# OpenStitching/stitching

Hardware: AMD Instinct MI355X
Metric: warped+blended Mpix/s (higher is better)
Workload: dtype u8/int16 (fixed-point remap, int32 pyramid sums, fp32 weights); 1 GPU; BASELINE config 2: 8 synthetic 4000x3000 frames, one ring; yaw step 38.9 deg = 0.58 hfov (42 % overlap; SURVEY 8(d) names 0.70 hfov); spherical warp + 5-band multiband blend, inputs resident in HBM; frames_per_gpu=8, panoramas_in_flight=2

## Files before the change

include/stitching_amd.h:

```cpp
#ifndef STITCHING_AMD_H
#define STITCHING_AMD_H

#include <stddef.h>
#include <stdint.h>

#ifdef __cplusplus
extern "C" {
#endif

#define STX_VERSION 100

#define STX_OK 0
#define STX_ERR_INVALID (-1)
#define STX_ERR_HIP (-2)
#define STX_ERR_OOM (-3)
#define STX_ERR_STATE (-4)
#define STX_ERR_UNSUPPORTED (-5)

#define STX_TRIG_EXACT 0
#define STX_TRIG_GLIBC 1
#define STX_TRIG_GLIBC_NOFMA 2
int stx_set_trig_mode(int mode);
int stx_get_trig_mode(void);

// ... 15 lines not shown
#define STX_WARP_CYLINDRICAL 2
#define STX_WARP_SPHERICAL 3
#define STX_WARP_FISHEYE 4
#define STX_WARP_STEREOGRAPHIC 5
#define STX_WARP_COMPRESSED_PLANE_A2B1 6
#define STX_WARP_COMPRESSED_PLANE_A15B1 7
#define STX_WARP_COMPRESSED_PLANE_PORTRAIT_A2B1 8
#define STX_WARP_COMPRESSED_PLANE_PORTRAIT_A15B1 9
#define STX_WARP_PANINI_A2B1 10
#define STX_WARP_PANINI_A15B1 11
#define STX_WARP_PANINI_PORTRAIT_A2B1 12
#define STX_WARP_PANINI_PORTRAIT_A15B1 13
#define STX_WARP_MERCATOR 14
#define STX_WARP_TRANSVERSE_MERCATOR 15
#define STX_WARP_TYPE_COUNT 16

#define STX_INTER_NEAREST 0
#define STX_INTER_LINEAR 1
#define STX_BORDER_CONSTANT 0
#define STX_BORDER_REFLECT 2

#define STX_BLEND_NO 0
#define STX_BLEND_FEATHER 1
#define STX_BLEND_MULTIBAND 2

#define STX_U8 0
#define STX_S16 1
#define STX_F32 2

typedef struct stx_ctx stx_ctx;
typedef struct stx_buf stx_buf;
typedef struct stx_blender stx_blender;
typedef struct stx_mb_weights stx_mb_weights;

int stx_version(void);
const char* stx_last_error(void);
int stx_device_count(int* out_n);
int stx_ctx_create(int device, stx_ctx** out);
int stx_ctx_destroy(stx_ctx* ctx);
int stx_ctx_sync(stx_ctx* ctx);

int stx_buf_from_host(stx_ctx* ctx, const void* host, size_t host_stride_bytes, int w, int h, int channels, int elem,
                      stx_buf** out);
int stx_buf_alloc(stx_ctx* ctx, int w, int h, int channels, int elem, stx_buf** out);
int stx_host_alloc(size_t bytes, void** out);
int stx_host_free(void* p);
int stx_buf_to_host(const stx_buf* buf, void* host, size_t host_stride_bytes);
int stx_buf_from_host_async(stx_ctx* ctx, const void* host, size_t host_stride_bytes, int w, int h, int channels, int elem,
                            stx_buf** out);
int stx_buf_to_host_async(const stx_buf* buf, void* host, size_t host_stride_bytes);
int stx_buf_view(const stx_buf* buf, int x, int y, int w, int h, stx_buf** out);
int stx_buf_info(const stx_buf* buf, int64_t info[6]);
int stx_buf_device_ptr(const stx_buf* buf, void** out);
int stx_buf_free(stx_buf* buf);

int stx_warp_roi(stx_ctx* ctx, int type, float scale, const float K[9], const float R[9], int w, int h,
                 int out_xywh[4]);
int stx_warp_rois(stx_ctx* ctx, int type, float scale, int n, const float* K9s, const float* R9s, const int* sizes_wh,
                  int* out_xywh);
int stx_warp(stx_ctx* ctx, int type, float scale, const float K[9], const float R[9], const stx_buf* src, int interp,
             int border, stx_buf** out, int out_tl[2]);
int stx_warp_image_and_mask(stx_ctx* ctx, int type, float scale, const float K[9], const float R[9],
                            const stx_buf* src, stx_buf** out_img, stx_buf** out_mask, int out_xywh[4]);
int stx_warp_batch(stx_ctx* ctx, int type, float scale, int n, const float* K9s, const float* R9s,
                   const stx_buf* const* srcs, stx_buf** out_imgs, stx_buf** out_masks, int* out_xywh);
int stx_warp_batch_rects(stx_ctx* ctx, int type, float scale, int n, const float* K9s, const float* R9s,
                         const stx_buf* const* srcs, const int* rects_xywh, stx_buf** out_imgs, stx_buf** out_masks);
int stx_warp_batch_gain(stx_ctx* ctx, int type, float scale, int n, const float* K9s, const float* R9s, const stx_buf* const* srcs,
                        const int* rects_xywh, const stx_buf* const* gain_maps_f32, const int* gain_flags, stx_buf** out_imgs,
                        stx_buf** out_masks, int* out_xywh);
int stx_warp_batch_with_rois(stx_ctx* ctx, int type, float scale, int n, const float* K9s, const float* R9s, const stx_buf* const* srcs,
                             const stx_buf* const* gain_maps_f32_or_null, const int* gain_flags_or_null, stx_buf** out_imgs,
                             stx_buf** out_masks, int* out_xywh);
int stx_warp_mask(stx_ctx* ctx, int type, float scale, const float K[9], const float R[9], int w, int h,
                  stx_buf** out_mask, int out_xywh[4]);

int stx_result_roi(int n, const int* corners_xy, const int* sizes_wh, int out_xywh[4]);
int stx_blend_create(stx_ctx* ctx, int kind, int num_bands, float sharpness, const int roi_xywh[4],
                     stx_blender** out);
int stx_blend_num_bands(const stx_blender* b, int* out_num_bands);
int stx_blend_feed(stx_blender* b, const stx_buf* img, const stx_buf* mask, int tlx, int tly);
int stx_blend_finish(stx_blender* b, stx_buf** out_pano_u8, stx_buf** out_mask_u8);
int stx_blend_finish_ex(stx_blender* b, stx_buf** out_pano_u8, stx_buf** out_mask_u8, stx_buf** out_pano_s16);
int stx_blend_destroy(stx_blender* b);
int stx_blend_keep_weights(stx_blender* b, stx_mb_weights** out);
int stx_blend_use_weights(stx_blender* b, stx_mb_weights* w, int* out_adopted);
int stx_mb_weights_free(stx_mb_weights* w);

int stx_gain_apply(stx_ctx* ctx, stx_buf* img_u8x3, const float gains_bgr[3]);
int stx_block_gain_apply(stx_ctx* ctx, stx_buf* img_u8x3, const stx_buf* gain_map_f32);
#define STX_GAIN_MAP_BOUNDED 1
int stx_block_gain_apply_batch(stx_ctx* ctx, int n, stx_buf* const* imgs_u8x3, const stx_buf* const* gain_maps_f32,
                               const int* full_wh_xy0, const int* flags);
#define STX_EXPOSURE_GAIN 1
#define STX_EXPOSURE_GAIN_BLOCKS 2
#define STX_EXPOSURE_CHANNELS 3
#define STX_EXPOSURE_CHANNELS_BLOCKS 4
int stx_exposure_feed(stx_ctx* ctx, int kind, int n, const stx_buf* const* imgs_u8x3, const stx_buf* const* masks_u8,
                      const int* corners_xy, int block_size, int nr_feeds, double* out_gains, long long* inout_count,
                      double out_info[4]);
int stx_exposure_stats(stx_ctx* ctx, int kind, int n, const stx_buf* const* imgs_u8x3, const stx_buf* const* masks_u8,
                       const int* corners_xy, int block_size, long long* inout_jobs, int* out_ab, long long* out_c,
                       double* out_sums);
// ... 108 lines not shown
```

include/stitching_amd_debug.h:

```cpp
#ifndef STITCHING_AMD_DEBUG_H
#define STITCHING_AMD_DEBUG_H

#include "stitching_amd.h"

#ifdef __cplusplus
extern "C" {
#endif

int stx_debug_warp_maps(stx_ctx* ctx, int type, float scale, const float K[9], const float R[9], int w, int h, int which,
                        const int rect_xywh[4], stx_buf** out_xmap_f32, stx_buf** out_ymap_f32, int out_xywh[4]);

int stx_debug_feather_dist_cap(void);

int stx_debug_blend_replayed(stx_ctx* ctx, int* out_launches);

#ifdef __cplusplus
}
#endif
#endif
```

stitching_amd/_lib.py:

```python
import ctypes as C
import os

from .stitching_error import StitchingError

_HERE = os.path.dirname(os.path.abspath(__file__))
LIB_PATH = os.environ.get("STITCHING_AMD_LIB") or os.path.join(_HERE, "libstitching_amd.so")

STX_OK = 0
WARP_PLANE, WARP_AFFINE, WARP_CYLINDRICAL, WARP_SPHERICAL = 0, 1, 2, 3
WARP_TYPE_IDS = {"plane": 0, "affine": 1, "cylindrical": 2, "spherical": 3, "fisheye": 4, "stereographic": 5,
                 "compressedPlaneA2B1": 6, "compressedPlaneA1.5B1": 7, "compressedPlanePortraitA2B1": 8,
                 "compressedPlanePortraitA1.5B1": 9, "paniniA2B1": 10, "paniniA1.5B1": 11, "paniniPortraitA2B1": 12,
                 "paniniPortraitA1.5B1": 13, "mercator": 14, "transverseMercator": 15}
INTER_NEAREST, INTER_LINEAR = 0, 1
BORDER_CONSTANT, BORDER_REFLECT = 0, 2
BLEND_NO, BLEND_FEATHER, BLEND_MULTIBAND = 0, 1, 2
U8, S16, F32 = 0, 1, 2
TRIG_MODES = {"exact": 0, "glibc": 1, "glibc-nofma": 2}
REMAP_MODES = {"q15": 0, "float": 1, "float-fma": 2}
PYRDOWN_MODES = {"scalar": 0, "simd-v": 1, "simd-hv": 3, "simd-v-fma": 5, "simd-hv-fma": 7}
GAIN_MAP_BOUNDED = 1
EXPOSURE_KINDS = {"gain": 1, "gain_blocks": 2, "channel": 3, "channel_blocks": 4}
EXPOSURE_SOLVERS = {"host": 0, "device": 1}
LU_NB, LU_MAX_N = 32, 16384
SEAM_KINDS = {"no": 0, "voronoi": 1}
COLOR_SEAM_MAX_LENGTH, COLOR_SEAM_MAX_CROSS = 16384, 4096
FEATURES_MAX_SIDE, FEATURES_MAX_LEVELS, FEATURES_MAX_FEATURES = 32767, 16, 65536
MATCH_MAX_FEATURES, MATCH_MAX_ITERS = 65536, 4096
RAY_MAX_CAMERAS, RAY_MAX_MATCHES = 1024, 131072
CONTRIB_U8_BINARY = 1
STRIP_MASK_BITS = 2

EXPORTS = (
    "stx_version stx_last_error stx_set_trig_mode stx_get_trig_mode stx_set_remap_mode stx_get_remap_mode stx_set_pyrdown_mode stx_get_pyrdown_mode stx_device_count stx_ctx_create stx_ctx_destroy stx_ctx_sync "
    "stx_host_alloc stx_host_free stx_buf_from_host stx_buf_from_host_async stx_buf_alloc stx_buf_to_host stx_buf_to_host_async stx_buf_view stx_buf_info stx_buf_device_ptr stx_buf_free "
    "stx_warp_roi stx_warp_rois stx_warp stx_warp_image_and_mask stx_warp_batch stx_warp_batch_rects stx_warp_batch_gain stx_warp_batch_with_rois stx_warp_mask "
    "stx_gain_apply stx_block_gain_apply stx_block_gain_apply_batch stx_resize_linear_exact stx_resize_linear_exact_batch stx_seam_mask_resize stx_seam_mask_resize_batch stx_seam_mask_resize_batch_sub stx_timelapse_frame stx_result_roi stx_blend_create stx_blend_num_bands stx_blend_feed stx_blend_finish stx_blend_finish_ex "
    "stx_blend_destroy stx_blend_keep_weights stx_blend_use_weights stx_mb_weights_free stx_blend_set_band stx_blend_feed_ex stx_blend_contrib_rect stx_blend_export_contrib stx_blend_export_contribs "
    "stx_blend_build stx_blend_feed_contrib stx_blend_feed_contrib_ex stx_buf_flags stx_strip_rect stx_view_rect stx_strip_pack stx_strip_pack_batch stx_strip_pack_batch_ex stx_strip_bytes stx_strip_unpack stx_blend_feed_strips stx_comm_unique_id stx_comm_create stx_comm_exchange stx_comm_exchange_begin stx_comm_exchange_end stx_comm_exchange_begin_on stx_comm_exchange_end_on stx_comm_info stx_comm_destroy stx_prof_enable stx_prof_reset stx_prof_count stx_prof_get stx_mark stx_mark_elapsed_ms "
    "stx_exposure_feed stx_exposure_stats stx_exposure_solve stx_set_exposure_solver stx_get_exposure_solver stx_exposure_feed_ex stx_exposure_solve_device stx_lu_solve_device stx_seam_find stx_seam_schedule stx_color_seam_find stx_crop_lir stx_features_detect stx_match_features stx_ray_problem_create stx_ray_problem_eval stx_ray_problem_free "
    "stx_debug_warp_maps stx_debug_feather_dist_cap stx_debug_blend_replayed"
).split()

_lib = None


def build_hint():
    return "build it with `make -C stitching_amd/csrc` or `python -c 'import __graft_entry__ as g; g.build()'`"


def lib():
    global _lib
    if _lib is not None:
        return _lib
    if not os.path.exists(LIB_PATH):
        raise ImportError(f"{LIB_PATH} is missing: the HIP back end is not built ({build_hint()}). "
                          "stitching_amd has no CPU fallback.")
    L = C.CDLL(LIB_PATH)
    vp, vpp = C.c_void_p, C.POINTER(C.c_void_p)
    fp, ip = C.POINTER(C.c_float), C.POINTER(C.c_int)
    L.stx_version.restype = C.c_int
    L.stx_last_error.restype = C.c_char_p
    L.stx_set_trig_mode.argtypes = [C.c_int]
    L.stx_get_trig_mode.restype = C.c_int
    L.stx_set_remap_mode.argtypes = [C.c_int]
    L.stx_get_remap_mode.restype = C.c_int
    L.stx_set_pyrdown_mode.argtypes = [C.c_int, C.c_int]
    L.stx_get_pyrdown_mode.argtypes = [C.POINTER(C.c_int)]
    L.stx_get_pyrdown_mode.restype = C.c_int
    L.stx_device_count.argtypes = [ip]
    L.stx_ctx_create.argtypes = [C.c_int, vpp]
    L.stx_ctx_destroy.argtypes = [vp]
    L.stx_ctx_sync.argtypes = [vp]
    L.stx_buf_from_host.argtypes = [vp, vp, C.c_size_t, C.c_int, C.c_int, C.c_int, C.c_int, vpp]
    L.stx_buf_from_host_async.argtypes = L.stx_buf_from_host.argtypes
    L.stx_buf_alloc.argtypes = [vp, C.c_int, C.c_int, C.c_int, C.c_int, vpp]
    L.stx_host_alloc.argtypes = [C.c_size_t, vpp]
    L.stx_host_free.argtypes = [vp]
    L.stx_buf_to_host.argtypes = [vp, vp, C.c_size_t]
    L.stx_buf_to_host_async.argtypes = [vp, vp, C.c_size_t]
    L.stx_buf_view.argtypes = [vp, C.c_int, C.c_int, C.c_int, C.c_int, vpp]
    L.stx_buf_info.argtypes = [vp, C.POINTER(C.c_int64)]
    L.stx_buf_device_ptr.argtypes = [vp, vpp]
    L.stx_buf_free.argtypes = [vp]
    L.stx_warp_roi.argtypes = [vp, C.c_int, C.c_float, fp, fp, C.c_int, C.c_int, ip]
    L.stx_warp_rois.argtypes = [vp, C.c_int, C.c_float, C.c_int, fp, fp, ip, ip]
    L.stx_warp.argtypes = [vp, C.c_int, C.c_float, fp, fp, vp, C.c_int, C.c_int, vpp, ip]
    L.stx_warp_image_and_mask.argtypes = [vp, C.c_int, C.c_float, fp, fp, vp, vpp, vpp, ip]
    L.stx_warp_batch.argtypes = [vp, C.c_int, C.c_float, C.c_int, fp, fp, vpp, vpp, vpp, ip]
    L.stx_warp_batch_rects.argtypes = [vp, C.c_int, C.c_float, C.c_int, fp, fp, vpp, ip, vpp, vpp]
    L.stx_warp_batch_gain.argtypes = [vp, C.c_int, C.c_float, C.c_int, fp, fp, vpp, ip, vpp, ip, vpp, vpp, ip]
    L.stx_warp_batch_with_rois.argtypes = [vp, C.c_int, C.c_float, C.c_int, fp, fp, vpp, vpp, ip, vpp, vpp, ip]
    L.stx_warp_mask.argtypes = [vp, C.c_int, C.c_float, fp, fp, C.c_int, C.c_int, vpp, ip]
    L.stx_gain_apply.argtypes = [vp, vp, fp]
    L.stx_block_gain_apply.argtypes = [vp, vp, vp]
    L.stx_block_gain_apply_batch.argtypes = [vp, C.c_int, vpp, vpp, ip, ip]
    L.stx_resize_linear_exact.argtypes = [vp, vp, C.c_int, C.c_int, vpp]
    L.stx_resize_linear_exact_batch.argtypes = [vp, C.c_int, vpp, ip, vpp]
    L.stx_seam_mask_resize.argtypes = [vp, vp, vp, vpp]
    L.stx_seam_mask_resize_batch.argtypes = [vp, C.c_int, vpp, vpp, vpp]
    L.stx_seam_mask_resize_batch_sub.argtypes = [vp, C.c_int, vpp, vpp, ip, vpp]
    L.stx_timelapse_frame.argtypes = [vp, vp, C.c_int, C.c_int, ip, vpp]
    L.stx_result_roi.argtypes = [C.c_int, ip, ip, ip]
    L.stx_blend_create.argtypes = [vp, C.c_int, C.c_int, C.c_float, ip, vpp]
    L.stx_blend_num_bands.argtypes = [vp, ip]
    L.stx_blend_feed.argtypes = [vp, vp, vp, C.c_int, C.c_int]
    L.stx_blend_finish.argtypes = [vp, vpp, vpp]
    L.stx_blend_finish_ex.argtypes = [vp, vpp, vpp, vpp]
    L.stx_blend_destroy.argtypes = [vp]
    L.stx_blend_keep_weights.argtypes = [vp, vpp]
    L.stx_blend_use_weights.argtypes = [vp, vp, ip]
    L.stx_mb_weights_free.argtypes = [vp]
    L.stx_blend_set_band.argtypes = [vp, C.c_int, C.c_int]
    L.stx_blend_feed_ex.argtypes = [vp, vp, vp, C.c_int, C.c_int, C.c_int]
    L.stx_blend_contrib_rect.argtypes = [vp, C.c_int, C.c_int, C.c_int, C.c_int, C.c_int, C.c_int, ip,
                                         C.POINTER(C.c_size_t)]
    L.stx_blend_export_contrib.argtypes = [vp, C.c_int, C.c_int, C.c_int, vpp, ip]
    L.stx_blend_export_contribs.argtypes = [vp, C.c_int, ip, ip, ip, vpp, ip]
    L.stx_blend_build.argtypes = [vp]
    L.stx_blend_feed_contrib.argtypes = [vp, C.c_int, ip, vp]
    L.stx_blend_feed_contrib_ex.argtypes = [vp, C.c_int, ip, vp, C.c_int]
    L.stx_buf_flags.argtypes = [vp, ip]
    L.stx_strip_rect.argtypes = [vp, C.c_int, C.c_int, C.c_int, C.c_int, C.c_int, C.c_int, ip, C.POINTER(C.c_size_t)]
    L.stx_view_rect.argtypes = [vp, C.c_int, C.c_int, C.c_int, C.c_int, C.c_int, C.c_int, C.c_int, C.c_int, ip]
    L.stx_strip_pack.argtypes = [vp, vp, vp, C.c_int, C.c_int, vpp]
    L.stx_strip_unpack.argtypes = [vp, C.c_int, C.c_int, C.c_int, vpp, vpp]
    L.stx_strip_pack_batch.argtypes = [vp, C.c_int, vpp, vpp, ip, ip, vpp]
    L.stx_strip_pack_batch_ex.argtypes = [vp, C.c_int, vpp, vpp, ip, ip, C.c_int, vpp]
    L.stx_strip_bytes.argtypes = [C.c_int, C.c_int, C.c_int, C.POINTER(C.c_size_t)]
    L.stx_blend_feed_strips.argtypes = [vp, C.c_int, vpp, ip, ip, ip, ip, ip, C.c_int]
    L.stx_comm_unique_id.argtypes = [C.POINTER(C.c_ubyte)]
    L.stx_comm_create.argtypes = [vp, C.c_int, C.c_int, C.POINTER(C.c_ubyte), vpp]
    L.stx_comm_exchange.argtypes = [vp, C.c_int, ip, ip, C.POINTER(C.c_void_p), C.POINTER(C.c_size_t)]
    L.stx_comm_exchange_begin.argtypes = [vp, C.c_int, ip, ip, C.POINTER(C.c_void_p), C.POINTER(C.c_size_t)]
    L.stx_comm_exchange_end.argtypes = [vp]
    L.stx_comm_exchange_begin_on.argtypes = [vp, vp, C.c_int, ip, ip, C.POINTER(C.c_void_p), C.POINTER(C.c_size_t)]
    L.stx_comm_exchange_end_on.argtypes = [vp, vp]
    L.stx_comm_info.argtypes = [vp, ip]
    L.stx_comm_destroy.argtypes = [vp]
    L.stx_prof_enable.argtypes = [vp, C.c_int]
    L.stx_prof_reset.argtypes = [vp]
    L.stx_prof_count.argtypes = [vp, ip]
    L.stx_prof_get.argtypes = [vp, C.c_int, C.c_char_p, C.c_int, C.POINTER(C.c_int64), C.POINTER(C.c_double),
                               C.POINTER(C.c_double)]
    L.stx_debug_blend_replayed.argtypes = [vp, ip]
    L.stx_debug_warp_maps.argtypes = [vp, C.c_int, C.c_float, fp, fp, C.c_int, C.c_int, C.c_int, ip, vpp, vpp, ip]
    llp, dp = C.POINTER(C.c_longlong), C.POINTER(C.c_double)
    L.stx_exposure_feed.argtypes = [vp, C.c_int, C.c_int, vpp, vpp, ip, C.c_int, C.c_int, dp, llp, dp]
    L.stx_exposure_stats.argtypes = [vp, C.c_int, C.c_int, vpp, vpp, ip, C.c_int, llp, ip, llp, dp]
    L.stx_exposure_solve.argtypes = [C.c_int, C.c_int, ip, dp, C.POINTER(C.c_ubyte), dp]
    L.stx_set_exposure_solver.argtypes = [C.c_int]
    L.stx_exposure_feed_ex.argtypes = [vp, C.c_int, C.c_int, vpp, vpp, ip, C.c_int, C.c_int, C.c_int, dp, llp, dp]
    L.stx_exposure_solve_device.argtypes = [vp, C.c_int, C.c_int, ip, dp, C.POINTER(C.c_ubyte), dp, dp]
    L.stx_lu_solve_device.argtypes = [vp, C.c_int, dp, dp, dp, dp]
    L.stx_seam_find.argtypes = [vp, C.c_int, C.c_int, ip, ip, vpp, vpp, dp]
    L.stx_seam_schedule.argtypes = [C.c_int, ip, ip, ip, ip, ip]
    L.stx_color_seam_find.argtypes = [vp, C.c_int, ip, ip, vpp, vpp, vpp, dp]
    L.stx_crop_lir.argtypes = [vp, vp, ip, ip, dp]
    L.stx_features_detect.argtypes = [vp, C.c_int, vpp, vpp, C.c_int, C.c_int, C.c_int, ip, ip, ip, ip, C.POINTER(C.c_byte), ip, ip, llp,
                                      C.POINTER(C.c_ubyte), dp]
    L.stx_match_features.argtypes = [vp, C.c_int, vpp, ip, vpp, ip, C.c_int, C.c_int, C.c_int, C.c_double, C.c_uint, ip, ip,
                                     C.POINTER(C.c_ubyte), ip, dp, dp]
    L.stx_ray_problem_create.argtypes = [vp, C.c_int, ip, llp, dp, vpp]
    L.stx_ray_problem_eval.argtypes = [vp, C.c_int, dp, dp, dp]
    L.stx_ray_problem_free.argtypes = [vp]
    L.stx_mark.argtypes = [vp, C.c_int]
    L.stx_mark_elapsed_ms.argtypes = [vp, C.c_int, C.c_int, C.POINTER(C.c_double)]
    for name in EXPORTS:
        if name not in ("stx_version", "stx_last_error"):
            getattr(L, name).restype = C.c_int
    _lib = L
    return L


def check(rc):
    if rc != STX_OK:
        msg = lib().stx_last_error()
        raise StitchingError(f"stitching_amd [{rc}]: {msg.decode(errors='replace') if msg else 'unknown error'}")
# ... 1 lines not shown
```

stitching_amd/csrc/stx_blend.hip:

```cpp
#include <cstring>

#include "stx_blend_kernels.h"
#include "stx_device_math.h"
#include "stx_internal.h"

using namespace stxd;

namespace {

constexpr float WEIGHT_EPS = 1e-5f;
constexpr float INV255 = 0.0039215688593685627f;
constexpr float INV256 = 0.00390625f;

template <bool S16>
STX_DEV void load_px0(const StxMbImage& im, int sx, int sy, int& b, int& g, int& r)
{
    if (S16) {
        const short* p = reinterpret_cast<const short*>(im.img0 + (long long)sy * im.img0_stride) + sx * 3;
        b = p[0]; g = p[1]; r = p[2];
    } else {
        const uint8_t* p = im.img0 + (long long)sy * im.img0_stride + sx * 3;
        b = p[0]; g = p[1]; r = p[2];
    }
}
// ... 661 lines not shown
            if (lv == 0) {
                if (im.img0_is_s16) hipLaunchKernelGGL(mb_down0_kernel<true>, grid64x4(ow, oh), dim3(256), 0, ctx->stream, im, pyr_mode, pyr_lanes);
                else hipLaunchKernelGGL(mb_down0_kernel<false>, grid64x4(ow, oh), dim3(256), 0, ctx->stream, im, pyr_mode, pyr_lanes);
            } else {
                hipLaunchKernelGGL(mb_down_kernel, grid64x4(ow, oh), dim3(256), 0, ctx->stream, im, lv, pyr_mode, pyr_lanes);
            }
        }
        STX_TRY(check_launch("mb_down"));
    }
    return STX_OK;
}

int stx_launch_mb_coarse(stx_ctx* ctx, const MbLevelK& K, double algo_bytes)
{
    if (K.x1 <= K.x0 || K.y1 <= K.y0) return STX_OK;
    if (K.level != K.num_bands - 2 || K.level < 1 || K.y0 != 0 || K.out_y0 != 0 || K.emit)
        return stx_fail(STX_ERR_INVALID, "mb_coarse: not the argument block of level B-2");
    StxProfScope prof(ctx, "mb_coarse", algo_bytes);
    MbCoarseK C;
    C.images = K.images; C.n_images = K.n_images; C.num_bands = K.num_bands;
    C.x0 = K.x0; C.x1 = K.x1; C.y1 = K.y1;
    C.out = K.out; C.out_stride = K.out_stride; C.out_plane = K.out_plane; C.out_x0 = K.out_x0;
    C.pw = K.pw; C.ph = K.ph;
    const dim3 grid((K.x1 - K.x0 + CO_TW - 1) / CO_TW, (K.y1 + CO_TH - 1) / CO_TH);
    hipLaunchKernelGGL(mb_coarse_kernel, grid, dim3(256), 0, ctx->stream, C);
    return check_launch("mb_coarse");
}

int stx_launch_mb_level(stx_ctx* ctx, const MbLevelK& K, double algo_bytes)
{
    if (K.x1 <= K.x0 || K.y1 <= K.y0) return STX_OK;
    StxProfScope prof(ctx, K.emit ? "mb_contrib" : (K.level == 0 ? "mb_level0" : "mb_level"), algo_bytes);
    if ((K.level > 0 || K.all_u8) && stx_fast_mb_level(ctx, K)) return STX_OK;
    const dim3 grid = grid64x4(K.x1 - K.x0, K.y1 - K.y0);
    if (K.level == 0) hipLaunchKernelGGL(mb_level_kernel<true>, grid, dim3(256), 0, ctx->stream, K);
    else hipLaunchKernelGGL(mb_level_kernel<false>, grid, dim3(256), 0, ctx->stream, K);
    return check_launch("mb_level");
}

int stx_launch_mb_emit_batch(stx_ctx* ctx, const MbLevelK* d_Ks, const MbLevelK* h_Ks, const int* classes, int n, double bytes)
{
    if (n <= 0) return STX_OK;
    StxProfScope prof(ctx, "mb_contrib", bytes);
    for (int start = 0; start < n;) {
        int end = start;
        while (end < n && classes[end] == classes[start]) end++;
        const int cls = classes[start], count = end - start;
        if (cls >= 0) {
            if (!stx_fast_mb_emit_launch(ctx, cls, d_Ks + start, h_Ks + start, count)) return check_launch("mb_contrib");
        } else {
            int gx = 1, gy = 1;
            for (int i = start; i < end; i++) {
                gx = std::max(gx, (h_Ks[i].x1 - h_Ks[i].x0 + 63) / 64);
                gy = std::max(gy, (h_Ks[i].y1 - h_Ks[i].y0 + 3) / 4);
            }
            const dim3 grid(gx, gy, count);
            if (cls == -1) hipLaunchKernelGGL(mb_level_multi_kernel<true>, grid, dim3(256), 0, ctx->stream, d_Ks + start);
            else hipLaunchKernelGGL(mb_level_multi_kernel<false>, grid, dim3(256), 0, ctx->stream, d_Ks + start);
        }
        start = end;
    }
    return check_launch("mb_contrib");
}

namespace {
STX_DEV uint32_t ld_u32_unaligned(const uint8_t* p)
// ... 1158 lines not shown
```

stitching_amd/csrc/stx_blend_fast.hip:

```cpp
#include <algorithm>
#include <cstdlib>

#include "stx_blend_kernels.h"
#include "stx_device_math.h"

using namespace stxd;

namespace {

constexpr int L0_WAVES = 5;
constexpr float WEIGHT_EPS = 1e-5f;
constexpr float INV255 = 0.0039215688593685627f;
constexpr float INV256 = 0.00390625f;

#define STX_GAS __attribute__((address_space(1)))
template <class T> STX_DEV const STX_GAS T* gp(const T* p) { return (const STX_GAS T*)p; }
template <class T> STX_DEV STX_GAS T* gp(T* p) { return (STX_GAS T*)p; }

STX_DEV bool xcd_tile(const StxTileMap& M, uint32_t b, int& tx, int& ty)
{
    if (M.plain) {
        const uint32_t wy = M.tiles_x == 1 ? b : __umulhi(b, M.magic_tx);
        tx = (int)(b - wy * (uint32_t)M.tiles_x);
        ty = (int)wy;
// ... 798 lines not shown
    int he[3][4], ho[3][4];
#pragma unroll
    for (int r = 0; r < 3; r++) {
        const T* p = plane + (long long)rr[r] * stride;
        int c[6];
        if (sizeof(T) == 2) {
            const v4u w = *reinterpret_cast<const v4u_a4*>(p + cx - 2);
            c[1] = s16lo(w.y); c[2] = s16hi(w.y); c[3] = s16lo(w.z); c[4] = s16hi(w.z);
            c[0] = s16hi(w.x);
            c[5] = s16lo(w.w);
        } else {
            const v3u w = *reinterpret_cast<const v3u_a4*>(p + cx - 4);
            c[0] = (int)(w.x >> 24);
            c[1] = (int)(w.y & 255u); c[2] = (int)((w.y >> 8) & 255u); c[3] = (int)((w.y >> 16) & 255u); c[4] = (int)(w.y >> 24);
            c[5] = (int)(w.z & 255u);
        }
        if (le) c[0] = c[2];
        if (re) c[5] = c[4];
#pragma unroll
        for (int j = 0; j < 4; j++) {
            he[r][j] = c[j] + 6 * c[j + 1] + c[j + 2];
            ho[r][j] = 4 * (c[j + 1] + c[j + 2]);
        }
    }
#pragma unroll
    for (int j = 0; j < 4; j++) {
        up[0][2 * j] = s6(he[0][j] + 6 * he[1][j] + he[2][j]);
        up[0][2 * j + 1] = s6(ho[0][j] + 6 * ho[1][j] + ho[2][j]);
        up[1][2 * j] = s6(4 * (he[1][j] + he[2][j]));
        up[1][2 * j + 1] = s6(4 * (ho[1][j] + ho[2][j]));
    }
}

template <bool L0>
STX_DEV void level_epilogue(const MbLevelK& P, int X0, int Y0, int (&acc)[2][8][3], float (&ws)[2][8])
{
    int v[2][8][3];
#pragma unroll
    for (int r = 0; r < 2; r++)
#pragma unroll
        for (int j = 0; j < 8; j++) {
            const float den = fadd(ws[r][j], WEIGHT_EPS);
            float q0, q1, q2;
            div3_shared(den, (float)(short)acc[r][j][0], (float)(short)acc[r][j][1], (float)(short)acc[r][j][2], q0, q1, q2);
            v[r][j][0] = trunc_small(q0);
            v[r][j][1] = trunc_small(q1);
            v[r][j][2] = trunc_small(q2);
        }
    if (P.up) {
#pragma unroll
        for (int c = 0; c < 3; c++) {
            int up[2][8];
            up_patch(P.up + c * P.up_plane - ((long long)P.up_y0 * P.up_stride + P.up_x0), P.up_stride, P.pw >> 1, P.ph >> 1,
                     X0 >> 1, Y0 >> 1, up);
#pragma unroll
            for (int r = 0; r < 2; r++)
#pragma unroll
                for (int j = 0; j < 8; j++) v[r][j][c] = sat_s16(up[r][j] + v[r][j][c]);
        }
    }
    if (!L0) {
#pragma unroll
        for (int r = 0; r < 2; r++)
#pragma unroll
            for (int c = 0; c < 3; c++) {
                uint4 o;
                o.x = pack16(v[r][0][c], v[r][1][c]);
                o.y = pack16(v[r][2][c], v[r][3][c]);
                o.z = pack16(v[r][4][c], v[r][5][c]);
                o.w = pack16(v[r][6][c], v[r][7][c]);
                if (Y0 + r < P.y1)
                    *reinterpret_cast<uint4*>(P.out + c * P.out_plane + (long long)(Y0 + r - P.out_y0) * P.out_stride + (X0 - P.out_x0)) = o;
            }
    } else {
#pragma unroll
        for (int r = 0; r < 2; r++) {
            const int y = Y0 + r;
            if (y >= P.y1) break;
            const int oy = y - P.pano_y0, ox = X0 - P.pano_x0;
            uint32_t ob[6] = {0, 0, 0, 0, 0, 0}, om[2] = {0, 0};
#pragma unroll
            for (int j = 0; j < 8; j++) {
                const bool keep = ws[r][j] > WEIGHT_EPS;
#pragma unroll
                for (int c = 0; c < 3; c++) {
                    if (!keep) v[r][j][c] = 0;
                    const uint32_t u = (uint32_t)min(abs(v[r][j][c]), 255);
                    const int bo = 3 * j + c;
                    ob[bo >> 2] |= u << (8 * (bo & 3));
                }
                om[j >> 2] |= (keep ? 255u : 0u) << (8 * (j & 3));
            }
            uint32_t* po = reinterpret_cast<uint32_t*>(P.pano + (long long)oy * P.pano_stride + (long long)ox * 3);
            *reinterpret_cast<uint2*>(po) = make_uint2(ob[0], ob[1]);
            *reinterpret_cast<uint2*>(po + 2) = make_uint2(ob[2], ob[3]);
            *reinterpret_cast<uint2*>(po + 4) = make_uint2(ob[4], ob[5]);
            *reinterpret_cast<uint2*>(P.pmask + (long long)oy * P.pmask_stride + ox) = make_uint2(om[0], om[1]);
            if (P.pano16) {
                uint32_t* p16 = reinterpret_cast<uint32_t*>(reinterpret_cast<uint8_t*>(P.pano16) + (long long)oy * P.pano16_stride +
                                                            (long long)ox * 6);
                uint32_t s[12];
#pragma unroll
                for (int j = 0; j < 8; j += 2) {
                    s[(j >> 1) * 3 + 0] = pack16(v[r][j][0], v[r][j][1]);
                    s[(j >> 1) * 3 + 1] = pack16(v[r][j][2], v[r][j + 1][0]);
                    s[(j >> 1) * 3 + 2] = pack16(v[r][j + 1][1], v[r][j + 1][2]);
                }
                *reinterpret_cast<uint4*>(p16) = make_uint4(s[0], s[1], s[2], s[3]);
                *reinterpret_cast<uint4*>(p16 + 4) = make_uint4(s[4], s[5], s[6], s[7]);
                *reinterpret_cast<uint4*>(p16 + 8) = make_uint4(s[8], s[9], s[10], s[11]);
            }
        }
    }
}

template <bool L0>
STX_DEV bool occ_hit_f(const uint8_t* occ, int fx, int fy, int fw, int fh, int lv, int tile_x, int Y0)
{
    const int sl = L0 ? 1 : lv;
    if (occ == nullptr) return true;
    const int lw = fw >> sl, lh = fh >> sl;
    const int fr = L0 ? (Y0 - fy) >> 1 : Y0 - (fy >> lv);
    int x0 = L0 ? (tile_x - fx) >> 1 : tile_x - (fx >> lv);
    int x1 = L0 ? (tile_x + 511 - fx) >> 1 : x0 + 511;
    x0 = max(x0, 0); x1 = min(x1, lw - 1);
    if (fr < 0 || fr >= lh || x0 > x1) return true;
    const int t0 = x0 >> 6, n = (x1 >> 6) - t0 + 1;
    const uint32_t* q = reinterpret_cast<const uint32_t*>(occ + (long long)(fr >> 1) * occ_pitch(lw) + (t0 & ~3));
    const uint32_t sh = (uint32_t)t0 & 3u;
    if (L0) {
// ... 14 lines not shown
}

template <bool L0, bool CONTRIB>
STX_DEV bool mb_tile_hit(const StxMbImage* images, int n_images, int lv, int tile_x, int Y0, int kk)
{
    const StxMbImage& im = images[min(kk, n_images - 1)];
    bool hit;
    if (L0) {
        const v4u f = *reinterpret_cast<const v4u_a4*>(&im.iw);
        const v4u ff = *reinterpret_cast<const v4u_a4*>(&im.fx);
        const uint8_t* const occp = im.occ[1];
        const int kind = CONTRIB ? im.kind : 0;
        int rx = (int)f.z, ry = (int)f.w, rw = (int)f.x, rh = (int)f.y;
        if (CONTRIB && kind == 1) { rx = (int)ff.x; ry = (int)ff.y; rw = (int)ff.z; rh = (int)ff.w; }
        hit = (kk < n_images) & (rx < tile_x + 512) & (rx + rw > tile_x) & (ry < Y0 + 2) & (ry + rh > Y0);
        if (hit) hit = occ_hit_f<true>(occp, (int)ff.x, (int)ff.y, (int)ff.z, (int)ff.w, 0, tile_x, Y0);
    } else {
        const v4u f = *reinterpret_cast<const v4u_a4*>(&im.fx);
        const uint8_t* const occp = im.occ[lv];
        const int rx = (int)f.x >> lv, ry = (int)f.y >> lv, rw = (int)f.z >> lv, rh = (int)f.w >> lv;
        hit = (kk < n_images) & (rx < tile_x + 512) & (rx + rw > tile_x) & (ry < Y0 + 2) & (ry + rh > Y0);
        if (hit) hit = occ_hit_f<false>(occp, (int)f.x, (int)f.y, (int)f.z, (int)f.w, lv, tile_x, Y0);
    }
    return hit;
}

typedef const unsigned long long __attribute__((address_space(4))) * StxCoverPtr;
STX_DEV unsigned long long mb_cover_word(const MbLevelK& P, int tile_tx, int Y0)
{
    const int idx = __builtin_amdgcn_readfirstlane(((Y0 - P.y0) / LV_TH) * P.tiles.tiles_x + tile_tx);
    return ((StxCoverPtr)P.cover)[idx];
}

template <bool WF>
STX_DEV void level0_epilogue_pk(const MbLevelK& P, int X0, int Y0, uint32_t (&acc)[2][3][4], uint32_t (&cnt)[2][4], const float (*ws)[8]);

template <bool L0, bool CONTRIB, bool EMIT, bool U8SRC>
STX_DEV void mb_level_fast_body(const MbLevelK& P)
{
    const int tid = threadIdx.x;
    const int lv = P.level;
    int tile_tx, tile_ty;
    if (!xcd_tile(P.tiles, blockIdx.x, tile_tx, tile_ty)) return;
    const int tile_x = P.x0 + tile_tx * 512, tile_y = P.y0 + tile_ty * LV_TH;
    const int X0 = tile_x + (tid & 63) * 8, Y0 = tile_y + __builtin_amdgcn_readfirstlane(tid >> 6) * 2;
    const bool active = X0 < P.x1 && Y0 < P.y1;

    int acc[2][8][3];
    float ws[2][8];
#pragma unroll
    for (int r = 0; r < 2; r++)
#pragma unroll
        for (int j = 0; j < 8; j++) {
            acc[r][j][0] = acc[r][j][1] = acc[r][j][2] = 0;
            ws[r][j] = 0.f;
        }
    constexpr bool PKACC = L0 && U8SRC && !CONTRIB && !EMIT;
    uint32_t accp[2][3][4], cntp[2][4];
    bool ws_live = false;
#pragma unroll
    for (int r = 0; r < 2; r++) {
#pragma unroll
        for (int c = 0; c < 3; c++) accp[r][c][0] = accp[r][c][1] = accp[r][c][2] = accp[r][c][3] = 0u;
        cntp[r][0] = cntp[r][1] = cntp[r][2] = cntp[r][3] = 0u;
    }

    for (int base = 0; base < P.n_images; base += 64) {
// ... 330 lines not shown
        HO[r][1] = pks(t.B1) + pks(t.A2);
    }
    if (unpk(__builtin_elementwise_min(worst, pk_splat(1000))) != unpk(worst)) return false;
#pragma unroll
    for (int k = 0; k < 2; k++) {
        up[0][k] = (HE[0][k] + HE[1][k] * pks_splat(6) + HE[2][k] + pks_splat(32)) >> pks_splat(6);
        up[0][2 + k] = (HO[0][k] + HO[1][k] * pks_splat(6) + HO[2][k] + pks_splat(8)) >> pks_splat(4);
        up[1][k] = (HE[1][k] + HE[2][k] + pks_splat(8)) >> pks_splat(4);
        up[1][2 + k] = (HO[1][k] + HO[2][k] + pks_splat(2)) >> pks_splat(2);
    }
    return true;
}
STX_DEV bool up_patch_pks(const STX_GAS short* __restrict__ plane, uint32_t stride, int ch, uint32_t boff, int cy, UpSel sel, pk16s up[2][4])
{
    v4u w[3];
    up_patch_pks_load(plane, stride, ch, boff, cy, w);
    return up_patch_pks_math(w, sel, up);
}

constexpr int pair_of(int j) { return (j & 1) ? 2 + (j >> 2) : (j >> 2); }
constexpr int half_of(int j) { return (j >> 1) & 1; }

template <int K>
STX_DEV uint32_t bgr_dword(const uint32_t (&U)[3][4])
{
    constexpr int b0 = 4 * K, b1 = b0 + 1, b2 = b0 + 2, b3 = b0 + 3;
    constexpr uint32_t s01 = (uint32_t)(2 * half_of(b0 / 3)) | ((uint32_t)(4 + 2 * half_of(b1 / 3)) << 8) | 0x0c0c0000u;
    constexpr uint32_t s23 = 0x00000c0cu | ((uint32_t)(2 * half_of(b2 / 3)) << 16) | ((uint32_t)(4 + 2 * half_of(b3 / 3)) << 24);
    const uint32_t lo = __builtin_amdgcn_perm(U[b1 % 3][pair_of(b1 / 3)], U[b0 % 3][pair_of(b0 / 3)], s01);
    const uint32_t hi = __builtin_amdgcn_perm(U[b3 % 3][pair_of(b3 / 3)], U[b2 % 3][pair_of(b2 / 3)], s23);
    return lo | hi;
}

template <bool WF>
STX_DEV void level0_epilogue_pk(const MbLevelK& P, int X0, int Y0, uint32_t (&acc)[2][3][4], uint32_t (&cnt)[2][4], const float (*ws)[8])
{
    uint32_t k_p1 = 0x00010001u, k_m1 = 0xffffffffu;
    asm("" : "+s"(k_p1), "+s"(k_m1));
    uint32_t v[2][3][4];
    const uint32_t anyc = (cnt[0][0] | cnt[0][1] | cnt[0][2] | cnt[0][3]) | (cnt[1][0] | cnt[1][1] | cnt[1][2] | cnt[1][3]);
    const uint32_t k11 = 0x00010001u;
    const uint32_t cnt3 = ((cnt[0][0] + k11) | (cnt[0][1] + k11) | (cnt[0][2] + k11) | (cnt[0][3] + k11)) |
                          ((cnt[1][0] + k11) | (cnt[1][1] + k11) | (cnt[1][2] + k11) | (cnt[1][3] + k11));
    if (!WF && (anyc & 0xfffefffeu) == 0u) {
#pragma unroll
        for (int r = 0; r < 2; r++)
#pragma unroll
            for (int c = 0; c < 3; c++)
#pragma unroll
                for (int q = 0; q < 4; q++) {
                    const pk16s a = pks(acc[r][c][q]);
                    v[r][c][q] = unpks(a - __builtin_elementwise_min(__builtin_elementwise_max(a, pks(k_m1)), pks(k_p1)));
                }
    } else if (!WF && (cnt3 & 0xfffcfffcu) == 0u) {
#pragma unroll
        for (int r = 0; r < 2; r++)
#pragma unroll
            for (int q = 0; q < 4; q++) {
                const pk16 h = pk(cnt[r][q]) >> pk_splat(1);
#pragma unroll
                for (int c = 0; c < 3; c++) {
                    const pk16s a0 = pks(acc[r][c][q]);
                    const pk16s a = a0 - __builtin_elementwise_min(__builtin_elementwise_max(a0, pks(k_m1)), pks(k_p1));
                    const pk16 neg = pk(unpks(a)) >> pk_splat(15);
                    v[r][c][q] = unpks(pks(unpk(pk(unpks(a)) + (neg & h))) >> pks(unpk(h)));
                }
            }
// ... 45 lines not shown
                    up[r][0] = pks(pack16(u32[r][0], u32[r][2]));
                    up[r][1] = pks(pack16(u32[r][4], u32[r][6]));
                    up[r][2] = pks(pack16(u32[r][1], u32[r][3]));
                    up[r][3] = pks(pack16(u32[r][5], u32[r][7]));
                }
            }
#pragma unroll
            for (int r = 0; r < 2; r++)
#pragma unroll
                for (int q = 0; q < 4; q++) v[r][c][q] = unpks(__builtin_elementwise_add_sat(up[r][q], pks(v[r][c][q])));
        }
    }
#pragma unroll
    for (int r = 0; r < 2; r++) {
        const int y = Y0 + r;
        if (y >= P.y1) break;
        const int oy = y - P.pano_y0, ox = X0 - P.pano_x0;
        uint32_t keep[4], U[3][4];
#pragma unroll
        for (int q = 0; q < 4; q++) keep[q] = unpk(pk_splat(0) - __builtin_elementwise_min(pk(cnt[r][q]), pk(k_p1)));
#pragma unroll
        for (int c = 0; c < 3; c++)
#pragma unroll
            for (int q = 0; q < 4; q++) {
                v[r][c][q] &= keep[q];
                const pk16s x = pks(v[r][c][q]);
                const pk16s ax = __builtin_elementwise_max(x, __builtin_elementwise_sub_sat(pks_splat(0), x));
                U[c][q] = unpks(__builtin_elementwise_min(ax, pks_splat(255)));
            }
        uint32_t* po = reinterpret_cast<uint32_t*>(P.pano + (long long)oy * P.pano_stride + (long long)ox * 3);
        *reinterpret_cast<uint2*>(po) = make_uint2(bgr_dword<0>(U), bgr_dword<1>(U));
        *reinterpret_cast<uint2*>(po + 2) = make_uint2(bgr_dword<2>(U), bgr_dword<3>(U));
        *reinterpret_cast<uint2*>(po + 4) = make_uint2(bgr_dword<4>(U), bgr_dword<5>(U));
        *reinterpret_cast<uint2*>(P.pmask + (long long)oy * P.pmask_stride + ox) =
            make_uint2(__builtin_amdgcn_perm(keep[2], keep[0], 0x06020400u), __builtin_amdgcn_perm(keep[3], keep[1], 0x06020400u));
        if (P.pano16) {
            uint32_t* p16 = reinterpret_cast<uint32_t*>(reinterpret_cast<uint8_t*>(P.pano16) + (long long)oy * P.pano16_stride + (long long)ox * 6);
            int w[8][3];
#pragma unroll
            for (int j = 0; j < 8; j++)
#pragma unroll
                for (int c = 0; c < 3; c++) w[j][c] = half_of(j) ? s16hi(v[r][c][pair_of(j)]) : s16lo(v[r][c][pair_of(j)]);
            uint32_t t[12];
#pragma unroll
            for (int j = 0; j < 8; j += 2) {
                t[(j >> 1) * 3 + 0] = pack16(w[j][0], w[j][1]);
                t[(j >> 1) * 3 + 1] = pack16(w[j][2], w[j + 1][0]);
                t[(j >> 1) * 3 + 2] = pack16(w[j + 1][1], w[j + 1][2]);
            }
            *reinterpret_cast<uint4*>(p16) = make_uint4(t[0], t[1], t[2], t[3]);
            *reinterpret_cast<uint4*>(p16 + 4) = make_uint4(t[4], t[5], t[6], t[7]);
            *reinterpret_cast<uint4*>(p16 + 8) = make_uint4(t[8], t[9], t[10], t[11]);
        }
    }
}

template <bool CONTRIB, bool DEFER = false, bool REPLAY = false>
__global__ __launch_bounds__(LV_THREADS) __attribute__((amdgpu_waves_per_eu(L0_WAVES, 8))) void mb_level0_pk_kernel(MbLevelK P)
{
    const int tid = threadIdx.x;
    int tile_tx, tile_ty;
    if (!xcd_tile(P.tiles, blockIdx.x, tile_tx, tile_ty)) return;
    const int tile_x = P.x0 + tile_tx * 512, tile_y = P.y0 + tile_ty * LV_TH;
    const int X0 = tile_x + (tid & 63) * 8, Y0 = tile_y + __builtin_amdgcn_readfirstlane(tid >> 6) * 2;
    const bool active = X0 < P.x1 && Y0 < P.y1;

    uint32_t acc[2][3][4];
    uint32_t cntb[2][2];
// ... 105 lines not shown
                        const pk16 L = pk(px[q]) - up[r][q];
                        acc[r][c][q] = unpk(L * pk(M[r][q]) + pk(acc[r][c][q]));
                    }
                }
            }
        }
    }
    if (!active) return;
    if (DEFER) {
        const bool mine = grey_seen != 0u;
        const unsigned long long dm = __ballot(mine);
        if (dm != 0ull) {
            const unsigned seg = (unsigned)tile_tx % (unsigned)STX_DEFER_SEGS;
            unsigned base_i = 0u;
            if ((unsigned)(tid & 63) == (unsigned)__builtin_ctzll(dm)) base_i = atomicAdd(P.defer_count + 32u * seg, (unsigned)__builtin_popcountll(dm));
            base_i = (unsigned)__builtin_amdgcn_readlane((int)base_i, (int)__builtin_ctzll(dm));
            if (mine) {
                const unsigned slot = base_i + (unsigned)__builtin_popcountll(dm & ((1ull << (tid & 63)) - 1ull));
                if (slot < P.defer_cap)
                    P.defer_list[(size_t)seg * P.defer_cap + slot] = (unsigned long long)(unsigned)X0 | ((unsigned long long)(unsigned)Y0 << 32);
                return;
            }
        }
    }

    uint32_t cnt[2][4];
#pragma unroll
    for (int r = 0; r < 2; r++) {
        cnt[r][0] = pair_u8<0, 2>(cntb[r]);
        cnt[r][1] = pair_u8<4, 6>(cntb[r]);
        cnt[r][2] = pair_u8<1, 3>(cntb[r]);
        cnt[r][3] = pair_u8<5, 7>(cntb[r]);
    }
    level0_epilogue_pk<false>(P, X0, Y0, acc, cnt, nullptr);
}


__global__ __launch_bounds__(256) void mb_level0_deferred_kernel(MbLevelK P)
{
    const unsigned wave = blockIdx.x * 4u + (unsigned)__builtin_amdgcn_readfirstlane((int)(threadIdx.x >> 6)), waves = gridDim.x * 4u;
    const unsigned lane = threadIdx.x & 63u;
    unsigned g0 = 0u;
    unsigned cnt_l[STX_DEFER_SEGS / 64];
#pragma unroll
    for (int j = 0; j < STX_DEFER_SEGS / 64; j++) {
        const unsigned sg = lane + 64u * (unsigned)j;
        cnt_l[j] = sg < (unsigned)P.defer_segs ? min(P.defer_count[32u * sg], P.defer_cap) : 0u;
    }
#pragma unroll
    for (int j = 0; j < STX_DEFER_SEGS / 64; j++)
    for (unsigned sl = 0; sl < 64u && 64u * (unsigned)j + sl < (unsigned)P.defer_segs; sl++) {
        const unsigned seg = 64u * (unsigned)j + sl;
        const unsigned n = (unsigned)__builtin_amdgcn_readlane((int)cnt_l[j], (int)sl), nb = (n + 63u) >> 6;
        for (unsigned g = g0 + (wave + waves - g0 % waves) % waves; g < g0 + nb; g += waves) {
            const unsigned i = (g - g0) * 64u + lane;
            const bool live = i < n;
            const unsigned long long e = live ? P.defer_list[(size_t)seg * P.defer_cap + i] : 0ull;
            const int X0 = (int)(unsigned)(e & 0xffffffffull), Y0 = (int)(unsigned)(e >> 32);
            int acc[2][8][3];
            float ws[2][8];
#pragma unroll
            for (int r = 0; r < 2; r++)
#pragma unroll
                for (int j = 0; j < 8; j++) {
                    acc[r][j][0] = acc[r][j][1] = acc[r][j][2] = 0;
                    ws[r][j] = 0.f;
                }
// ... 5 lines not shown
                if (!inside) continue;
                uint32_t vm0, vm1;
                {
                    const int lo = max(-lx0, 0), hi = min(im.iw - lx0, 8);
                    const uint32_t bits = ((1u << hi) - 1u) & ~((1u << lo) - 1u);
                    vm0 = (((bits & 15u) * 0x00204081u) & 0x01010101u) * 0xffu;
                    vm1 = (((bits >> 4) * 0x00204081u) & 0x01010101u) * 0xffu;
                }
                uint32_t pw_[2][6], mw[2][2];
#pragma unroll
                for (int r = 0; r < 2; r++) {
                    const int ly = ly0 + r;
                    const bool rin = (unsigned)ly < (unsigned)im.ih;
                    load_px8_u8(im, lx0, min(max(ly, 0), im.ih - 1), rin ? vm0 : 0u, rin ? vm1 : 0u, pw_[r], mw[r]);
                }
                int up[3][2][8];
#pragma unroll
                for (int c = 0; c < 3; c++)
                    up_patch(reinterpret_cast<const uint8_t*>(im.g[1]) + c * im.g_plane[1], im.g_stride[1], im.fw >> 1, im.fh >> 1,
                             (X0 - im.fx) >> 1, (Y0 - im.fy) >> 1, up[c]);
#pragma unroll
                for (int r = 0; r < 2; r++)
#pragma unroll
                    for (int j = 0; j < 8; j++) {
                        const float w = fmul((float)byte_of(mw[r], j), INV255);
#pragma unroll
                        for (int c = 0; c < 3; c++) {
                            const int L = sat_s16((int)byte_of(pw_[r], 3 * j + c) - up[c][r][j]);
                            acc[r][j][c] += trunc_small(fmul((float)L, w));
                        }
                        ws[r][j] = fadd(ws[r][j], w);
                    }
            }
            if (live) level_epilogue<true>(P, X0, Y0, acc, ws);
        }
        g0 += nb;
    }
}

STX_DEV uint32_t min3u(uint32_t a, uint32_t b, uint32_t c) { return min(min(a, b), c); }
STX_DEV uint32_t max3u(uint32_t a, uint32_t b, uint32_t c) { return max(max(a, b), c); }

constexpr int LVPK_WAVES = 3;
template <bool REPLAY>
__global__ __launch_bounds__(LV_THREADS) __attribute__((amdgpu_waves_per_eu(LVPK_WAVES, 8))) void mb_level_pk_kernel(MbLevelK P)
{
    const int tid = threadIdx.x;
    const int lv = P.level;
    int tile_tx, tile_ty;
    if (!xcd_tile(P.tiles, blockIdx.x, tile_tx, tile_ty)) return;
    const int tile_x = P.x0 + tile_tx * 512, tile_y = P.y0 + tile_ty * LV_TH;
    const int X0 = tile_x + (tid & 63) * 8, Y0 = tile_y + __builtin_amdgcn_readfirstlane(tid >> 6) * 2;
    const bool active = X0 < P.x1 && Y0 < P.y1;

    uint32_t acc[2][3][4];
    float ws[2][8];
#pragma unroll
    for (int r = 0; r < 2; r++) {
#pragma unroll
        for (int q = 0; q < 4; q++) acc[r][0][q] = acc[r][1][q] = acc[r][2][q] = 0;
#pragma unroll
        for (int j = 0; j < 8; j++) ws[r][j] = 0.f;
    }
    uint32_t ones = 0;
    uint32_t mixed = 0;

    for (int base = 0; base < (REPLAY ? 1 : P.n_images); base += 64) {
// ... 242 lines not shown
{
    if (K.num_bands - K.level < 3) return false;
    if ((K.x0 | K.y0 | K.out_x0 | K.out_y0 | K.pano_x0 | K.pano_y0) & 7) return false;
    if (K.up && ((K.up_x0 | K.up_y0) & 3)) return false;
    if (K.n_images > 255) return false;
    *KT = K;
    KT->tiles = stx_tile_map((K.x1 - K.x0 + 511) / 512, (K.y1 - K.y0 + LV_TH - 1) / LV_TH, LV_BAND);
    return true;
}

int stx_fast_mb_emit_class(const MbLevelK& K, MbLevelK* KT)
{
    if (!(K.level > 0 || K.all_u8) || !fast_level_ok(K, KT)) { *KT = K; return -1; }
    return K.level == 0 ? 0 : (K.all_u8 ? 1 : 2);
}

bool stx_fast_mb_emit_launch(stx_ctx* ctx, int cls, const MbLevelK* d_Ks, const MbLevelK* h_Ks, int count)
{
    unsigned gx = 1;
    for (int i = 0; i < count; i++) gx = std::max(gx, stx_tile_grid(h_Ks[i].tiles));
    const dim3 grid(gx, 1, (unsigned)count);
    if (cls == 0) hipLaunchKernelGGL((mb_emit_multi_kernel<true, false>), grid, dim3(LV_THREADS), 0, ctx->stream, d_Ks);
    else if (cls == 1) hipLaunchKernelGGL((mb_emit_multi_kernel<false, true>), grid, dim3(LV_THREADS), 0, ctx->stream, d_Ks);
    else hipLaunchKernelGGL((mb_emit_multi_kernel<false, false>), grid, dim3(LV_THREADS), 0, ctx->stream, d_Ks);
    return launched_ok();
}

static bool no_defer()
{
    static const bool off = getenv("STITCHING_AMD_NO_DEFER") != nullptr;
    return off;
}

bool stx_fast_mb_level(stx_ctx* ctx, const MbLevelK& K)
{
    MbLevelK KT;
    if (!fast_level_ok(K, &KT)) return false;
    dim3 grid(stx_tile_grid(KT.tiles), 1);
    hipStream_t st = ctx->stream;
    const bool replay = !K.emit && K.cover != nullptr && K.n_images <= 64 && !K.has_contrib;
    bool replayed = false;
    if (K.level == 0 && K.pk_ok && !K.emit && K.num_bands > 0) {
        static const unsigned pad_lds = getenv("STITCHING_AMD_L0_LDS") ? (unsigned)atoi(getenv("STITCHING_AMD_L0_LDS")) : 0u;
        if (K.has_contrib) hipLaunchKernelGGL(mb_level0_pk_kernel<true>, grid, dim3(LV_THREADS), pad_lds, st, KT);
        else if (replay) hipLaunchKernelGGL((mb_level0_pk_kernel<false, false, true>), grid, dim3(LV_THREADS), pad_lds, st, KT);
        else hipLaunchKernelGGL(mb_level0_pk_kernel<false>, grid, dim3(LV_THREADS), pad_lds, st, KT);
        replayed = replay && !K.has_contrib;
    } else if (K.level == 0 && K.all_u8 && !K.has_contrib && !K.emit && K.num_bands > 0 && !no_defer()) {
        const int segs = std::min(KT.tiles.tiles_x, STX_DEFER_SEGS);
        const size_t seg_cap = (size_t)((KT.tiles.tiles_x + STX_DEFER_SEGS - 1) / STX_DEFER_SEGS) * (size_t)KT.tiles.tiles_y * (unsigned)LV_THREADS;
        const size_t counters = (size_t)STX_DEFER_SEGS * 128;
        KT.defer_segs = segs;
        StxDevBlock q;
        if (stx_dev_alloc(ctx, counters + seg_cap * (size_t)segs * sizeof(unsigned long long), &q) != STX_OK) return false;
        KT.defer_count = reinterpret_cast<unsigned*>(q.get());
        KT.defer_list = reinterpret_cast<unsigned long long*>(reinterpret_cast<uint8_t*>(q.get()) + counters);
        KT.defer_cap = (unsigned)seg_cap;
        hipMemsetAsync(q.get(), 0, counters, st);
        if (replay) hipLaunchKernelGGL((mb_level0_pk_kernel<false, true, true>), grid, dim3(LV_THREADS), 0, st, KT);
        else hipLaunchKernelGGL((mb_level0_pk_kernel<false, true>), grid, dim3(LV_THREADS), 0, st, KT);
        replayed = replay;
        {
            StxProfScope prof2(ctx, "mb_level0_deferred", 0.0);
            hipLaunchKernelGGL(mb_level0_deferred_kernel, dim3(1024), dim3(256), 0, st, KT);
        }
        static const bool stats = getenv("STITCHING_AMD_DEFER_STATS") != nullptr;
        if (stats) {
            std::vector<unsigned> hc(counters / 4);
            hipStreamSynchronize(st);
            hipMemcpy(hc.data(), q.get(), counters, hipMemcpyDeviceToHost);
            unsigned long long tot = 0; unsigned mx = 0;
            for (int sgi = 0; sgi < segs; sgi++) { tot += hc[32 * sgi]; mx = std::max(mx, hc[32 * sgi]); }
            fprintf(stderr, "[stitching_amd] level-0 deferral: %llu of %llu patches queued (%d segments, fullest %u of %zu)\n", tot,
                    (unsigned long long)KT.tiles.tiles_x * KT.tiles.tiles_y * (unsigned long long)LV_THREADS, segs, mx, seg_cap);
        }
    } else if (K.emit) {
        if (K.level == 0) hipLaunchKernelGGL((mb_level_fast_kernel<true, false, true, false>), grid, dim3(LV_THREADS), 0, st, KT);
        else if (K.all_u8) hipLaunchKernelGGL((mb_level_fast_kernel<false, false, true, true>), grid, dim3(LV_THREADS), 0, st, KT);
        else hipLaunchKernelGGL((mb_level_fast_kernel<false, false, true, false>), grid, dim3(LV_THREADS), 0, st, KT);
    } else if (K.has_contrib) {
        if (K.level == 0) hipLaunchKernelGGL((mb_level_fast_kernel<true, true, false, false>), grid, dim3(LV_THREADS), 0, st, KT);
// ... 33 lines not shown
```

stitching_amd/csrc/stx_blend_host.cpp:

```cpp
#include <algorithm>
#include <climits>
#include <cmath>
#include <cstdlib>
#include <cstring>
#include <memory>

#include "stx_blend_kernels.h"
#include "stx_internal.h"

STX_EXPORT int stx_debug_feather_dist_cap(void) { return STX_FEATHER_DIST_CAP; }

STX_EXPORT int stx_result_roi(int n, const int* corners_xy, const int* sizes_wh, int out_xywh[4])
{
    if (n <= 0 || !corners_xy || !sizes_wh || !out_xywh) return stx_fail(STX_ERR_INVALID, "bad argument");
    int tlx = INT_MAX, tly = INT_MAX, brx = INT_MIN, bry = INT_MIN;
    for (int i = 0; i < n; i++) {
        tlx = std::min(tlx, corners_xy[2 * i]);
        tly = std::min(tly, corners_xy[2 * i + 1]);
        brx = std::max(brx, corners_xy[2 * i] + sizes_wh[2 * i]);
        bry = std::max(bry, corners_xy[2 * i + 1] + sizes_wh[2 * i + 1]);
    }
    out_xywh[0] = tlx; out_xywh[1] = tly; out_xywh[2] = brx - tlx; out_xywh[3] = bry - tly;
    return STX_OK;
}
// ... 121 lines not shown
    }
    L->bytes = off;
}

static void mb_insert_sorted(stx_blender* b, const StxMbImage& im, bool is_built)
{
    size_t pos = b->images.size();
    while (pos > 0 && b->images[pos - 1].order > im.order) pos--;
    b->images.insert(b->images.begin() + pos, im);
    b->built.insert(b->built.begin() + pos, is_built ? 1 : 0);
    b->d_all = nullptr;
}

static int mb_feed(stx_blender* b, const stx_buf* img, const stx_buf* mask, int tlx, int tly, int order)
{
    stx_ctx* ctx = b->ctx;
    const int nb = b->num_bands, w = img->w, h = img->h;
    StxMbImage im;
    memset(&im, 0, sizeof(im));
    im.kind = 0;
    im.order = order;
    mb_feed_rect(b, w, h, tlx, tly, &im.fx, &im.fy, &im.fw, &im.fh);
    im.img0 = img->ptr; im.img0_stride = (long long)img->stride; im.img0_is_s16 = img->elem == STX_S16;
    im.mask0 = mask->ptr; im.mask0_stride = (long long)mask->stride; im.mask_binary = mask->mask_binary;
    im.iw = w; im.ih = h;
    im.ix = tlx - b->rx; im.iy = tly - b->ry;
    im.left = im.ix - im.fx; im.top = im.iy - im.fy;
    im.g_u8 = img->elem == STX_U8 ? 1 : 0;
    static const bool w1_f32 = getenv("STITCHING_AMD_W1_F32") != nullptr;
    im.w1_f16 = (mask->mask_binary && !w1_f32) ? 1 : 0;
    for (int i = 1; i <= nb; i++) {
        const int lw = im.fw >> i, lh = im.fh >> i;
        const long long gs = (long long)align_up((size_t)lw, im.g_u8 ? 64 : 32), ws = (long long)align_up((size_t)lw, 16);
        void *g = nullptr, *wt = nullptr;
        STX_TRY(stx_dev_alloc(ctx, MB_FRONT_PAD + (size_t)gs * lh * 3 * (im.g_u8 ? 1 : sizeof(short)) + 64, &g));
        b->pyr_allocs.push_back(g);
        STX_TRY(stx_dev_alloc(ctx, (size_t)ws * lh * ((i == 1 && im.w1_f16) ? sizeof(uint16_t) : sizeof(float)), &wt));
        b->wt_allocs.push_back(wt);
        im.g[i] = (short*)((uint8_t*)g + MB_FRONT_PAD); im.g_stride[i] = gs; im.g_plane[i] = gs * lh;
        im.wt[i] = (float*)wt; im.wt_stride[i] = ws;
    }
    mb_insert_sorted(b, im, nb == 0);
    stx_buf_retain(const_cast<stx_buf*>(img));
    stx_buf_retain(const_cast<stx_buf*>(mask));
    b->held.push_back(const_cast<stx_buf*>(img));
    b->held.push_back(const_cast<stx_buf*>(mask));
    return STX_OK;
}

static int mb_upload(stx_blender* b, const StxMbImage* h, int n, StxMbImage** d_out)
{
    stx_ctx* ctx = b->ctx;
    void* d = nullptr;
    STX_TRY(stx_dev_alloc(ctx, sizeof(StxMbImage) * std::max(n, 1), &d));
    b->pyr_allocs.push_back(d);
    if (n > 0) STX_TRY(stx_stage_upload(ctx, d, h, sizeof(StxMbImage) * (size_t)n));
    *d_out = (StxMbImage*)d;
    return STX_OK;
}

static int mb_ensure_pyramids(stx_blender* b)
{
    std::vector<StxMbImage> todo;
    for (size_t i = 0; i < b->images.size(); i++)
        if (b->images[i].kind == 0 && !b->built[i]) todo.push_back(b->images[i]);
    if (todo.empty()) return STX_OK;
    static const bool occ_off = getenv("STITCHING_AMD_NO_OCC") != nullptr;
    const int pyr = b->pyr_mode;
    if (!b->adopted && todo.size() <= 65535 && !occ_off && (pyr & 255) == STX_PYRDOWN_SCALAR) {
        const int nl = b->num_bands + 1;
        std::vector<size_t> off(todo.size() * (size_t)nl, 0);
        size_t bytes = 0;
        for (size_t t = 0; t < todo.size(); t++) {
            if (todo[t].img0_is_s16) continue;
            for (int i = 1; i < nl; i++) {
                off[t * nl + i] = bytes;
                bytes += (size_t)((((todo[t].fh >> i) + 1) >> 1) + 1) * (size_t)(((((todo[t].fw >> i) + 63) >> 6) + 3) & ~3);
            }
        }
        if (bytes > 0) {
            void* arena = nullptr;
            STX_TRY(stx_dev_alloc(b->ctx, bytes + 16, &arena));
            b->wt_allocs.push_back(arena);
            size_t t = 0;
            for (size_t i = 0; i < b->images.size(); i++) {
                if (!(b->images[i].kind == 0 && !b->built[i])) continue;
                if (!todo[t].img0_is_s16)
                    for (int l = 1; l < nl; l++) todo[t].occ[l] = b->images[i].occ[l] = (uint8_t*)arena + off[t * nl + l];
                t++;
            }
        }
    }
    StxMbImage* d = nullptr;
    STX_TRY(mb_upload(b, todo.data(), (int)todo.size(), &d));
    b->d_all = todo.size() == b->images.size() && memcmp(todo.data(), b->images.data(), sizeof(StxMbImage) * todo.size()) == 0 ? d : nullptr;
    STX_TRY(stx_launch_mb_pyramids(b->ctx, d, todo.data(), (int)todo.size(), b->num_bands, pyr & 255, pyr >> 8, b->adopted == nullptr));
    for (size_t i = 0; i < b->images.size(); i++) b->built[i] = 1;
    return STX_OK;
}

static double mb_level_bytes(const stx_blender* b, const std::vector<StxMbImage>& imgs, int lv, int x0, int x1, bool emit,
                             bool with16)
{
    const int nb = b->num_bands;
    const int ph = lv == 0 ? b->fh : b->rh >> lv;
    double bytes = 0.0;
    for (const StxMbImage& im : imgs) {
        int rx = im.fx >> lv, rw = im.fw >> lv, ry = im.fy >> lv, rh = im.fh >> lv;
        if (lv == 0 && im.kind == 0) { rx = im.ix; rw = im.iw; ry = im.iy; rh = im.ih; }
        const double cols = std::max(0, std::min(rx + rw, x1) - std::max(rx, x0)), rows = std::min(ry + rh, ph) - ry;
        if (cols <= 0 || rows <= 0) continue;
        const double g3 = im.g_u8 ? 3.0 : 6.0;
        if (im.kind == 1) bytes += cols * rows * 10.0;
        else if (lv == 0) bytes += cols * rows * ((im.img0_is_s16 ? 6 : 3) + 1) + (nb > 0 ? cols * rows * g3 / 4.0 : 0.0);
        else bytes += cols * rows * (g3 + ((lv == 1 && im.w1_f16) ? 2.0 : 4.0)) + (lv < nb ? cols * rows * g3 / 4.0 : 0.0);
    }
    const double area = (double)(x1 - x0) * ph;
    if (emit) return bytes + area * 10.0;
    if (lv < nb) bytes += area * 6.0 / 4.0;
    bytes += lv == 0 ? area * (4 + (with16 ? 6 : 0)) : area * 6.0;
    return bytes;
}

STX_EXPORT int stx_blend_feed_ex(stx_blender* b, const stx_buf* img, const stx_buf* mask, int tlx, int tly, int order)
{
    if (!b || !img || !mask) return stx_fail(STX_ERR_INVALID, "null argument");
    if (b->finished) return stx_fail(STX_ERR_STATE, "feed after blend()");
// ... 48 lines not shown
    stx_buf_retain(const_cast<stx_buf*>(img));
    stx_buf_retain(const_cast<stx_buf*>(mask));
    b->held.push_back(const_cast<stx_buf*>(img));
    b->held.push_back(const_cast<stx_buf*>(mask));
    return STX_OK;
}

STX_EXPORT int stx_blend_feed(stx_blender* b, const stx_buf* img, const stx_buf* mask, int tlx, int tly)
{
    return stx_blend_feed_ex(b, img, mask, tlx, tly, -1);
}

static void mb_fill_common(const stx_blender* b, MbLevelK* K, const StxMbImage* d_images, int n, int lv)
{
    memset(K, 0, sizeof(*K));
    K->images = d_images; K->n_images = n; K->level = lv; K->num_bands = b->num_bands;
    K->pw = b->rw >> lv; K->ph = b->rh >> lv;
    K->all_u8 = 1;
}

static int mb_level_y1(const stx_blender* b, int lv) { return lv == 0 ? b->fh : b->rh >> lv; }

static const unsigned long long* mb_cover_for(const stx_mb_weights* w, const MbLevelK& K)
{
    if (!w || K.level < 0 || K.level > STX_MAX_BANDS || K.n_images > 64 || K.n_images != (int)w->images.size()) return nullptr;
    const stx_mb_weights::Cover& c = w->cover[K.level];
    int tx, ty, br;
    stx_fast_mb_cover_dims(K.x0, K.x1, K.y0, K.y1, &tx, &ty, &br);
    if (!c.table || c.x0 != K.x0 || c.x1 != K.x1 || c.y0 != K.y0 || c.y1 != K.y1 || c.tiles_x != tx || c.tiles_y != ty || c.band_rows != br)
        return nullptr;
    return c.table;
}

static int mb_finish(stx_blender* b, stx_buf* pano, stx_buf* pmask, stx_buf* pano16)
{
    stx_ctx* ctx = b->ctx;
    const int nb = b->num_bands, n = (int)b->images.size();
    STX_TRY(mb_ensure_pyramids(b));
    StxMbImage* d_images = b->d_all;
    if (!d_images) STX_TRY(mb_upload(b, b->images.data(), n, &d_images));
    b->d_gather = d_images;
    bool all_u8 = true, has_contrib = false, pk_ok = true;
    for (const StxMbImage& im : b->images) {
        if (im.kind == 0 && im.img0_is_s16) all_u8 = false;
        if (im.kind == 1) has_contrib = true;
        if ((im.kind == 0 && im.img0_is_s16) || !im.mask_binary) pk_ok = false;
    }
    int xb[STX_MAX_BANDS + 1], xe[STX_MAX_BANDS + 1];
    mb_level_regions(b, b->band_x0, b->band_x1, xb, xe);
    std::vector<short*> out(nb + 2, nullptr);
    std::vector<long long> ostride(nb + 2, 0), oplane(nb + 2, 0);
    static const bool no_fusion = getenv("STITCHING_AMD_NO_COARSE_FUSION") != nullptr;
    const bool fuse = nb >= 3 && !no_fusion;
    for (int lv = fuse ? nb - 2 : nb; lv >= 0; lv--) {
        MbLevelK K;
        mb_fill_common(b, &K, d_images, n, lv);
        K.all_u8 = all_u8 ? 1 : 0;
        K.has_contrib = has_contrib ? 1 : 0;
        K.pk_ok = pk_ok ? 1 : 0;
        K.x0 = xb[lv]; K.x1 = xe[lv]; K.y0 = 0; K.y1 = mb_level_y1(b, lv);
        if (b->adopted && !has_contrib) K.cover = mb_cover_for(b->adopted, K);
        if (lv < nb) {
            K.up = out[lv + 1]; K.up_stride = ostride[lv + 1]; K.up_plane = oplane[lv + 1];
            K.up_x0 = xb[lv + 1]; K.up_y0 = 0;
        }
        if (lv == 0) {
            K.pano = pano->ptr; K.pano_stride = (long long)pano->stride;
            K.pmask = pmask->ptr; K.pmask_stride = (long long)pmask->stride;
            if (pano16) { K.pano16 = (short*)pano16->ptr; K.pano16_stride = (long long)pano16->stride; }
            K.pano_x0 = b->band_x0; K.pano_y0 = 0;
        } else {
            const int w = xe[lv] - xb[lv], ph = b->rh >> lv;
            const long long st = (long long)align_up((size_t)std::max(w, 1), 32);
            void* p = nullptr;
            STX_TRY(stx_dev_alloc(ctx, MB_FRONT_PAD + (size_t)st * ph * 3 * sizeof(short), &p));
            b->pyr_allocs.push_back(p);
            out[lv] = (short*)((uint8_t*)p + MB_FRONT_PAD); ostride[lv] = st; oplane[lv] = st * ph;
            K.out = out[lv]; K.out_stride = st; K.out_plane = st * ph;
            K.out_x0 = xb[lv]; K.out_y0 = 0;
        }
        if (fuse && lv == nb - 2) {
            double bytes = mb_level_bytes(b, b->images, lv, K.x0, K.x1, false, false) - (double)(K.x1 - K.x0) * (b->rh >> lv) * 6.0 / 4.0;
            for (int l2 = nb - 1; l2 <= nb; l2++)
                bytes += mb_level_bytes(b, b->images, l2, xb[l2], xe[l2], false, false) - (double)(xe[l2] - xb[l2]) * (b->rh >> l2) * (l2 < nb ? 7.5 : 6.0);
            K.up = nullptr;
            STX_TRY(stx_launch_mb_coarse(ctx, K, bytes));
            continue;
        }
        STX_TRY(stx_launch_mb_level(ctx, K, mb_level_bytes(b, b->images, lv, K.x0, K.x1, false, pano16 != nullptr)));
    }
    return STX_OK;
}

void stx_mb_weights_release(stx_mb_weights* w)
{
    if (!w || --w->refs > 0) return;
    if (w->ctx) hipSetDevice(w->ctx->device);
    for (StxMbKept& k : w->images) stx_buf_release(k.mask);
    for (void* p : w->allocs) stx_dev_free(w->ctx, p);
    delete w;
}

static bool mb_weights_eligible(const stx_blender* b, bool built)
{
    if (b->kind != STX_BLEND_MULTIBAND || !b->ctx || b->num_bands < 1 || b->adopted) return false;
    if ((b->pyr_mode & 255) != STX_PYRDOWN_SCALAR || getenv("STITCHING_AMD_NO_OCC") != nullptr || b->images.size() > 65535) return false;
    for (const StxMbImage& im : b->images) {
        if (im.kind != 0 || im.img0_is_s16) return false;
        if (built && !im.occ[1]) return false;
    }
    return true;
}

static void mb_hand_over_weights(stx_blender* b)
{
    stx_mb_weights* w = b->keep;
    if (!w || b->images.empty() || !mb_weights_eligible(b, true)) return;
    w->num_bands = b->num_bands; w->pyr_mode = b->pyr_mode;
    w->rx = b->rx; w->ry = b->ry; w->rw = b->rw; w->rh = b->rh;
    for (const StxMbImage& im : b->images) {
        StxMbKept k;
        memset(&k, 0, sizeof(k));
        for (size_t h = 1; h < b->held.size(); h += 2)
            if (b->held[h]->ptr == im.mask0 && (long long)b->held[h]->stride == im.mask0_stride) k.mask = b->held[h];
        if (!k.mask) {
            for (StxMbKept& q : w->images) stx_buf_release(q.mask);
            w->images.clear();
            return;
        }
        stx_buf_retain(k.mask);
        k.mask0 = im.mask0; k.mask0_stride = im.mask0_stride; k.mask_binary = im.mask_binary; k.w1_f16 = im.w1_f16;
        k.iw = im.iw; k.ih = im.ih; k.ix = im.ix; k.iy = im.iy; k.fx = im.fx; k.fy = im.fy; k.fw = im.fw; k.fh = im.fh;
        k.left = im.left; k.top = im.top;
        for (int i = 1; i <= b->num_bands; i++) { k.wt[i] = im.wt[i]; k.wt_stride[i] = im.wt_stride[i]; k.occ[i] = im.occ[i]; }
        w->images.push_back(k);
    }
    w->allocs.swap(b->wt_allocs);
    if (b->images.size() > 64 || !b->d_gather) return;
    int xb[STX_MAX_BANDS + 1], xe[STX_MAX_BANDS + 1];
    mb_level_regions(b, b->band_x0, b->band_x1, xb, xe);
    for (int lv = 0; lv <= b->num_bands - 3; lv++) {
        stx_mb_weights::Cover c;
        c.x0 = xb[lv]; c.x1 = xe[lv]; c.y0 = 0; c.y1 = mb_level_y1(b, lv);
        if (c.x1 <= c.x0 || c.y1 <= c.y0) continue;
        stx_fast_mb_cover_dims(c.x0, c.x1, c.y0, c.y1, &c.tiles_x, &c.tiles_y, &c.band_rows);
        void* t = nullptr;
        if (stx_dev_alloc(b->ctx, sizeof(unsigned long long) * (size_t)c.tiles_x * (size_t)c.tiles_y, &t) != STX_OK) return;
        w->allocs.push_back(t);
        c.table = (unsigned long long*)t;
        if (!stx_fast_mb_cover(b->ctx, b->d_gather, (int)b->images.size(), lv, c.x0, c.x1, c.y0, c.y1, c.table)) return;
        w->cover[lv] = c;
    }
}

STX_EXPORT int stx_blend_keep_weights(stx_blender* b, stx_mb_weights** out)
{
    if (!b || !out) return stx_fail(STX_ERR_INVALID, "null argument");
    *out = nullptr;
    if (b->finished) return stx_fail(STX_ERR_STATE, "keep_weights after blend()");
    if (b->keep) return stx_fail(STX_ERR_STATE, "keep_weights was already called on this blender");
    if (b->images.empty() || !mb_weights_eligible(b, false)) return STX_OK;
    stx_mb_weights* w = new stx_mb_weights();
    w->ctx = b->ctx;
    w->refs = 2;
    b->keep = w;
    *out = w;
    return STX_OK;
}

STX_EXPORT int stx_blend_use_weights(stx_blender* b, stx_mb_weights* w, int* out_adopted)
{
    if (!b || !w || !out_adopted) return stx_fail(STX_ERR_INVALID, "null argument");
    *out_adopted = 0;
    if (b->finished) return stx_fail(STX_ERR_STATE, "use_weights after blend()");
    if (b->ctx != w->ctx) return stx_fail(STX_ERR_INVALID, "use_weights: the handle belongs to another context (no cross-stream use)");
    if (b->adopted || b->keep || w->images.empty() || w->images.size() != b->images.size() || !mb_weights_eligible(b, false)) return STX_OK;
    if (b->num_bands != w->num_bands || b->pyr_mode != w->pyr_mode || b->rx != w->rx || b->ry != w->ry || b->rw != w->rw || b->rh != w->rh)
        return STX_OK;
    for (size_t i = 0; i < b->images.size(); i++) {
        const StxMbImage& im = b->images[i];
        const StxMbKept& k = w->images[i];
        if (b->built[i]) return STX_OK;
        if (im.mask0 != k.mask0 || im.mask0_stride != k.mask0_stride || im.mask_binary != k.mask_binary || im.w1_f16 != k.w1_f16 ||
            im.iw != k.iw || im.ih != k.ih || im.ix != k.ix || im.iy != k.iy || im.fx != k.fx || im.fy != k.fy || im.fw != k.fw ||
            im.fh != k.fh || im.left != k.left || im.top != k.top)
            return STX_OK;
        for (int l = 1; l <= b->num_bands; l++)
            if (im.wt_stride[l] != k.wt_stride[l]) return STX_OK;
    }
    STX_TRY(stx_set_device(b->ctx));
    for (size_t i = 0; i < b->images.size(); i++)
        for (int l = 1; l <= b->num_bands; l++) { b->images[i].wt[l] = w->images[i].wt[l]; b->images[i].occ[l] = w->images[i].occ[l]; }
    for (void* p : b->wt_allocs) stx_dev_free(b->ctx, p);
    b->wt_allocs.clear();
    b->d_all = nullptr;
    w->refs++;
    b->adopted = w;
    *out_adopted = 1;
    return STX_OK;
}

STX_EXPORT int stx_debug_blend_replayed(stx_ctx* ctx, int* out_launches)
{
    if (!ctx || !out_launches) return stx_fail(STX_ERR_INVALID, "null argument");
    *out_launches = ctx->blend_replayed;
    return STX_OK;
}

STX_EXPORT int stx_mb_weights_free(stx_mb_weights* w)
{
    stx_mb_weights_release(w);
    return STX_OK;
}

STX_EXPORT int stx_blend_set_band(stx_blender* b, int x0, int x1)
{
    if (!b) return stx_fail(STX_ERR_INVALID, "null argument");
    if (b->kind != STX_BLEND_MULTIBAND) return stx_fail(STX_ERR_UNSUPPORTED, "bands exist for the multi-band blender only");
    if (b->finished) return stx_fail(STX_ERR_STATE, "set_band after blend()");
    const int al = (1 << b->num_bands) - 1;
    if (x0 < 0 || x1 > b->fw || x1 <= x0 || (x0 & al) || ((x1 & al) && x1 != b->fw) || (x0 & 7))
        return stx_fail(STX_ERR_INVALID, "band [%d,%d) must lie in [0,%d) with edges on multiples of max(8, 2^bands)", x0, x1, b->fw);
    b->band_x0 = x0; b->band_x1 = x1;
    return STX_OK;
}

STX_EXPORT int stx_blend_contrib_rect(const stx_blender* b, int img_w, int img_h, int tlx, int tly, int band_x0, int band_x1,
                                      int out_rect_xywh[4], size_t* out_bytes)
{
    if (!b || !out_rect_xywh) return stx_fail(STX_ERR_INVALID, "null argument");
    if (b->kind != STX_BLEND_MULTIBAND) return stx_fail(STX_ERR_UNSUPPORTED, "multi-band blender only");
    int fx, fy, fw, fh, sx0, sx1;
    mb_feed_rect(b, img_w, img_h, tlx, tly, &fx, &fy, &fw, &fh);
    if (!mb_contrib_range(b, fx, fw, band_x0, band_x1, &sx0, &sx1)) {
        out_rect_xywh[0] = out_rect_xywh[1] = out_rect_xywh[2] = out_rect_xywh[3] = 0;
        if (out_bytes) *out_bytes = 0;
        return STX_OK;
    }
// ... 4 lines not shown
        *out_bytes = L.bytes;
    }
    return STX_OK;
}

STX_EXPORT int stx_blend_export_contrib(stx_blender* b, int order, int band_x0, int band_x1, stx_buf** out_packed,
                                        int out_rect_xywh[4])
{
    return stx_blend_export_contribs(b, 1, &order, &band_x0, &band_x1, out_packed, out_rect_xywh);
}

STX_EXPORT int stx_blend_export_contribs(stx_blender* b, int n, const int* orders, const int* band_x0s, const int* band_x1s,
                                         stx_buf** out_packed, int* out_rects_xywh)
{
    if (!b || n < 0 || (n > 0 && (!orders || !band_x0s || !band_x1s || !out_packed || !out_rects_xywh)))
        return stx_fail(STX_ERR_INVALID, "null argument");
    if (b->kind != STX_BLEND_MULTIBAND) return stx_fail(STX_ERR_UNSUPPORTED, "multi-band blender only");
    if (b->finished) return stx_fail(STX_ERR_STATE, "export after blend()");
    if (!b->ctx) return stx_fail(STX_ERR_STATE, "geometry-only blender (created without a context)");
    if (n == 0) return STX_OK;
    STX_TRY(stx_set_device(b->ctx));
    const int nb = b->num_bands;
    std::vector<StxMbImage> srcs(n);
    std::vector<int> sx0(n), sx1(n);
    for (int i = 0; i < n; i++) {
        const StxMbImage* src = nullptr;
        for (const StxMbImage& im : b->images) if (im.kind == 0 && im.order == orders[i]) src = &im;
        if (!src) return stx_fail(STX_ERR_INVALID, "no fed image with order %d", orders[i]);
        if (!mb_contrib_range(b, src->fx, src->fw, band_x0s[i], band_x1s[i], &sx0[i], &sx1[i]))
            return stx_fail(STX_ERR_INVALID, "image %d does not reach the columns [%d,%d)", orders[i], band_x0s[i], band_x1s[i]);
        srcs[i] = *src;
    }
    STX_TRY(mb_ensure_pyramids(b));
    std::vector<StxBufRef> packed(n);
    std::vector<ContribLayout> Ls(n);
    for (int i = 0; i < n; i++) {
        mb_contrib_layout(nb, sx1[i] - sx0[i], srcs[i].fh, &Ls[i]);
        STX_TRY(stx_buf_new(b->ctx, (int)std::min<size_t>(Ls[i].bytes, 1u << 30), (int)((Ls[i].bytes + (1u << 30) - 1) >> 30), 1, STX_U8,
                            &packed[i]));
        if (packed[i]->stride * (size_t)packed[i]->h < Ls[i].bytes) return stx_fail(STX_ERR_OOM, "contribution too large");
    }
    StxMbImage* d_srcs = nullptr;
    STX_TRY(mb_upload(b, srcs.data(), n, &d_srcs));
    struct Item { int cls; MbLevelK K; };
    std::vector<Item> items;
    double bytes = 0.0;
    for (int i = 0; i < n; i++) {
        const StxMbImage& one = srcs[i];
        const int sh = one.fh;
        std::vector<StxMbImage> single(1, one);
        for (int lv = 0; lv <= nb; lv++) {
            MbLevelK K;
            mb_fill_common(b, &K, d_srcs + i, 1, lv);
            K.all_u8 = one.img0_is_s16 ? 0 : 1;
            K.x0 = sx0[i] >> lv; K.x1 = sx1[i] >> lv; K.y0 = one.fy >> lv; K.y1 = (one.fy + sh) >> lv;
            K.emit = 1;
            K.out = (short*)(packed[i]->ptr + Ls[i].g_off[lv]); K.out_stride = Ls[i].g_stride[lv];
            K.out_plane = Ls[i].g_stride[lv] * std::max(sh >> lv, 1);
            K.out_x0 = K.x0; K.out_y0 = K.y0;
            K.out_w = (float*)(packed[i]->ptr + Ls[i].w_off[lv]); K.out_w_stride = Ls[i].w_stride[lv];
            if (K.x1 <= K.x0 || K.y1 <= K.y0) continue;
            Item it;
            it.cls = stx_fast_mb_emit_class(K, &it.K);
            if (it.cls < 0) it.cls = lv == 0 ? -1 : -2;
            items.push_back(it);
            bytes += mb_level_bytes(b, single, lv, K.x0, K.x1, true, false);
// ... 83 lines not shown
}

static int no_finish(stx_blender* b, stx_buf* pano, stx_buf* pmask, stx_buf* p16)
{
    stx_ctx* ctx = b->ctx;
    const int n = (int)b->no_images.size();
    void* d_tab = nullptr;
    STX_TRY(stx_dev_alloc(ctx, sizeof(NoImg) * std::max(n, 1), &d_tab));
    b->pyr_allocs.push_back(d_tab);
    bool all_binary = true;
    double bytes = 4.0 * pano->w * pano->h + (p16 ? 6.0 * pano->w * pano->h : 0.0);
    for (const NoImg& im : b->no_images) {
        all_binary = all_binary && im.mask_binary;
        bytes += (double)im.w * im.h;
    }
    bytes += 3.0 * pano->w * pano->h;
    if (n > 0) STX_TRY(stx_stage_upload(ctx, d_tab, b->no_images.data(), sizeof(NoImg) * (size_t)n));
    NoGatherK K;
    K.imgs = (const NoImg*)d_tab; K.n = n; K.all_binary = all_binary ? 1 : 0;
    K.w = pano->w; K.h = pano->h;
    K.pano = pano->ptr; K.pano_stride = (long long)pano->stride; K.pmask = pmask->ptr; K.pmask_stride = (long long)pmask->stride;
    K.pano16 = p16 ? (short*)p16->ptr : nullptr; K.pano16_stride = p16 ? (long long)p16->stride : 0;
    return stx_launch_no_gather(ctx, K, bytes);
}

STX_EXPORT int stx_blend_finish_ex(stx_blender* b, stx_buf** out_pano_u8, stx_buf** out_mask_u8, stx_buf** out_pano_s16)
{
    if (!b) return stx_fail(STX_ERR_INVALID, "null argument");
    if (b->finished) return stx_fail(STX_ERR_STATE, "blend() was already called on this blender");
    if (!b->ctx) return stx_fail(STX_ERR_STATE, "geometry-only blender (created without a context)");
    STX_TRY(stx_set_device(b->ctx));
    stx_ctx* ctx = b->ctx;
    ctx->blend_replayed = 0;
    const int ow = b->kind == STX_BLEND_MULTIBAND ? b->band_x1 - b->band_x0 : b->rw, oh = b->kind == STX_BLEND_MULTIBAND ? b->fh : b->rh;
    StxBufRef p16, pmask, pano;
    const int rc = [&]() {
        STX_TRY(stx_buf_new(ctx, ow, oh, 3, STX_U8, &pano));
        STX_TRY(stx_buf_new(ctx, ow, oh, 1, STX_U8, &pmask));
        if (out_pano_s16) STX_TRY(stx_buf_new(ctx, ow, oh, 3, STX_S16, &p16));
        if (b->kind == STX_BLEND_MULTIBAND) return mb_finish(b, pano.get(), pmask.get(), p16.get());
        if (b->kind == STX_BLEND_NO) return no_finish(b, pano.get(), pmask.get(), p16.get());
        return feather_finish(b, pano.get(), pmask.get(), p16.get());
    }();
    if (rc == STX_OK) mb_hand_over_weights(b);
    b->finished = true;
    blender_release(b);
    STX_TRY(rc);
    if (out_pano_u8) *out_pano_u8 = pano.release();
    if (out_mask_u8) *out_mask_u8 = pmask.release();
    if (out_pano_s16) *out_pano_s16 = p16.release();
    return STX_OK;
}

STX_EXPORT int stx_blend_finish(stx_blender* b, stx_buf** out_pano_u8, stx_buf** out_mask_u8)
{
    return stx_blend_finish_ex(b, out_pano_u8, out_mask_u8, nullptr);
}

STX_EXPORT int stx_blend_destroy(stx_blender* b)
{
    if (!b) return STX_OK;
    if (b->ctx) {
        hipSetDevice(b->ctx->device);
        blender_release(b);
    }
    delete b;
    return STX_OK;
}
```

stitching_amd/csrc/stx_blend_kernels.h:

```cpp
#pragma once
#include "stx_internal.h"

struct StxTileMap {
    int tiles_x, tiles_y, band_rows, band_tiles;
    unsigned magic_tx, magic_band;
    int plain;
};
inline StxTileMap stx_tile_map(int tiles_x, int tiles_y, int band_rows)
{
    StxTileMap m;
    m.tiles_x = tiles_x; m.tiles_y = tiles_y; m.band_rows = band_rows; m.band_tiles = band_rows * tiles_x;
    m.magic_tx = (unsigned)((1ull << 32) / (unsigned)tiles_x) + 1u;
    m.magic_band = (unsigned)((1ull << 32) / (unsigned)m.band_tiles) + 1u;
    m.plain = 0;
    return m;
}
inline unsigned stx_tile_grid(const StxTileMap& m)
{
    if (m.plain) return (unsigned)(m.tiles_x * m.tiles_y);
    const int bands = (m.tiles_y + m.band_rows - 1) / m.band_rows;
    return 8u * (unsigned)(((bands + 7) / 8) * m.band_tiles);
}

constexpr int STX_DEFER_SEGS = 256;
struct MbLevelK {
    const StxMbImage* images;
    int n_images, level, num_bands, pw, ph;
    int x0, x1, y0, y1;
    short* out; long long out_stride, out_plane; int out_x0, out_y0;
    const short* up; long long up_stride, up_plane; int up_x0, up_y0;
    int emit; union { float* out_w; const unsigned long long* cover; }; long long out_w_stride;
    uint8_t* pano; long long pano_stride;
    uint8_t* pmask; long long pmask_stride;
    short* pano16; long long pano16_stride;
    int pano_x0, pano_y0;
    int has_contrib;
    int all_u8;
    StxTileMap tiles;
    int pk_ok;
    int defer_segs;
    unsigned long long* defer_list; unsigned* defer_count; unsigned defer_cap;
};

bool stx_fast_mb_down_batch(stx_ctx* ctx, const StxMbImage* d_images, const StxMbImage* h_images, int n, int level, bool weights);
bool stx_fast_mb_level(stx_ctx* ctx, const MbLevelK& K);
void stx_fast_mb_cover_dims(int x0, int x1, int y0, int y1, int* tiles_x, int* tiles_y, int* band_rows);
bool stx_fast_mb_cover(stx_ctx* ctx, const StxMbImage* d_images, int n, int level, int x0, int x1, int y0, int y1, unsigned long long* cover);

int stx_fast_mb_emit_class(const MbLevelK& K, MbLevelK* KT);
bool stx_fast_mb_emit_launch(stx_ctx* ctx, int cls, const MbLevelK* d_Ks, const MbLevelK* h_Ks, int count);
int stx_launch_mb_emit_batch(stx_ctx* ctx, const MbLevelK* d_Ks, const MbLevelK* h_Ks, const int* classes, int n, double bytes);
```

stitching_amd/csrc/stx_context_host.cpp:

```cpp
#include <algorithm>
#include <cstring>

#include "stx_internal.h"

static thread_local char g_err[512] = "";

void stx_set_error(const char* fmt, ...)
{
    va_list ap;
    va_start(ap, fmt);
    vsnprintf(g_err, sizeof(g_err), fmt, ap);
    va_end(ap);
}

int stx_fail(int code, const char* fmt, ...)
{
    va_list ap;
    va_start(ap, fmt);
    vsnprintf(g_err, sizeof(g_err), fmt, ap);
    va_end(ap);
    return code;
}

STX_EXPORT const char* stx_last_error(void) { return g_err; }
// ... 62 lines not shown
    if (!ctx) return STX_OK;
    hipSetDevice(ctx->device);
    if (ctx->stream) hipStreamSynchronize(ctx->stream);
    if (ctx->aux_stream) hipStreamSynchronize(ctx->aux_stream);
    for (auto& kv : ctx->block_size) hipFree(kv.first);
    for (auto& p : ctx->prof_pending) { hipEventDestroy(p.start); hipEventDestroy(p.stop); }
    for (auto e : ctx->event_pool) hipEventDestroy(e);
    for (auto e : ctx->marks) if (e) hipEventDestroy(e);
    if (ctx->pinned) hipHostFree(ctx->pinned);
    if (ctx->stage) hipHostFree(ctx->stage);
    for (hipEvent_t e : ctx->stage_ev) if (e) hipEventDestroy(e);
    if (ctx->aux_scratch) hipFree(ctx->aux_scratch);
    if (ctx->aux_stream) hipStreamDestroy(ctx->aux_stream);
    if (ctx->stream) hipStreamDestroy(ctx->stream);
    delete ctx;
    return STX_OK;
}

static size_t bucket_of(size_t bytes)
{
    if (bytes < 256) return 256;
    if (bytes >= (1u << 20)) return (bytes + (1u << 20) - 1) & ~(size_t)((1u << 20) - 1);
    size_t b = 256;
    while (b < bytes) b <<= 1;
    return b;
}

int stx_dev_alloc(stx_ctx* ctx, size_t bytes, void** out)
{
    size_t b = bucket_of(bytes + 64);
    std::lock_guard<std::mutex> lock(ctx->alloc_mutex);
    auto it = ctx->free_blocks.find(b);
    if (it != ctx->free_blocks.end() && !it->second.empty()) {
        *out = it->second.back();
        it->second.pop_back();
        return STX_OK;
    }
    void* p = nullptr;
    hipError_t e = hipMalloc(&p, b);
    if (e != hipSuccess) {
        hipStreamSynchronize(ctx->stream);
        for (auto& kv : ctx->free_blocks) {
            for (void* q : kv.second) { ctx->bytes_allocated -= ctx->block_size[q]; ctx->block_size.erase(q); hipFree(q); }
            kv.second.clear();
        }
        e = hipMalloc(&p, b);
        if (e != hipSuccess) return stx_fail(STX_ERR_OOM, "hipMalloc(%zu) failed: %s", b, hipGetErrorString(e));
    }
    ctx->block_size[p] = b;
    ctx->bytes_allocated += b;
    *out = p;
    return STX_OK;
}

void stx_dev_free(stx_ctx* ctx, void* p)
{
    if (!p) return;
    std::lock_guard<std::mutex> lock(ctx->alloc_mutex);
    auto it = ctx->block_size.find(p);
    if (it == ctx->block_size.end()) return;
    ctx->free_blocks[it->second].push_back(p);
}

int stx_stage_upload(stx_ctx* ctx, void* d, const void* h, size_t bytes)
{
    if (bytes == 0) return STX_OK;
    const size_t seg = ctx->stage_bytes / STX_STAGE_SEGS;
    if (bytes > seg) {
// ... 156 lines not shown
```

stitching_amd/csrc/stx_internal.h:

```cpp
#pragma once
#include <hip/hip_runtime.h>

#include <atomic>
#include <cstdarg>
#include <cstddef>
#include <cstdint>
#include <cstdio>
#include <map>
#include <memory>
#include <mutex>
#include <string>
#include <vector>

#include "../../include/stitching_amd.h"
#include "../../include/stitching_amd_debug.h"

#define STX_EXPORT extern "C" __attribute__((visibility("default")))
#define STX_MAX_BANDS 16

void stx_set_error(const char* fmt, ...);
int stx_fail(int code, const char* fmt, ...);

#define STX_HIP(call)                                                                                      \
    do {                                                                                                   \
// ... 16 lines not shown
    double algo_bytes = 0.0;
};

struct StxPendingEvent {
    hipEvent_t start, stop;
    int entry;
};

struct stx_ctx {
    int device = 0;
    hipStream_t stream = nullptr;
    hipStream_t aux_stream = nullptr;
    void* aux_scratch = nullptr;
    std::mutex alloc_mutex;
    std::map<size_t, std::vector<void*>> free_blocks;
    std::map<void*, size_t> block_size;
    size_t bytes_allocated = 0;
    void* pinned = nullptr;
    size_t pinned_bytes = 0;
    uint32_t roi_seq = 0;
    uint8_t* stage = nullptr;
    size_t stage_bytes = 0, stage_off = 0;
    hipEvent_t stage_ev[4] = {};
    bool stage_ev_set[4] = {};
    int stage_seg = 0;
    bool prof_on = false;
    std::vector<StxProfEntry> prof;
    std::map<std::string, int> prof_index;
    std::vector<StxPendingEvent> prof_pending;
    std::vector<hipEvent_t> event_pool;
    hipEvent_t marks[16] = {};
    double* exp_sqrt = nullptr;
    int blend_replayed = 0;
};

#define STX_STAGE_SEGS 4
int stx_dev_alloc(stx_ctx* ctx, size_t bytes, void** out);
int stx_stage_upload(stx_ctx* ctx, void* d, const void* h, size_t bytes);
void stx_dev_free(stx_ctx* ctx, void* p);
int stx_set_device(stx_ctx* ctx);
struct StxDevFree { stx_ctx* ctx; void operator()(void* p) const { stx_dev_free(ctx, p); } };
using StxDevBlock = std::unique_ptr<void, StxDevFree>;
inline int stx_dev_alloc(stx_ctx* ctx, size_t bytes, StxDevBlock* out)
{
    void* p = nullptr;
    STX_TRY(stx_dev_alloc(ctx, bytes, &p));
    *out = StxDevBlock(p, StxDevFree{ctx});
    return STX_OK;
}
int upload_small(stx_ctx* ctx, const void* h, size_t bytes, StxDevBlock* d_out);
size_t align_up(size_t v, size_t a);

struct StxProfScope {
    stx_ctx* ctx;
    int pending = -1;
    hipStream_t stream;
    bool attached;
    StxProfScope(stx_ctx* c, const char* name, double algo_bytes, hipStream_t on = nullptr, bool attach = false);
    ~StxProfScope();
    hipEvent_t start() const;
    hipEvent_t stop() const;
};

struct stx_buf {
    stx_ctx* ctx = nullptr;
    void* base = nullptr;
// ... 25 lines not shown
    for (const StxBufRef& b : v) p.push_back(b.get());
    return p;
}

int trig_mode_now();
int remap_mode_now();
int pyrdown_now();
int exposure_solver_now();

enum { STX_F_PLANE = 0, STX_F_CYLINDRICAL, STX_F_SPHERICAL, STX_F_FISHEYE, STX_F_STEREOGRAPHIC, STX_F_CRECT,
       STX_F_CRECT_PORTRAIT, STX_F_PANINI, STX_F_PANINI_PORTRAIT, STX_F_MERCATOR, STX_F_TRANSVERSE_MERCATOR };
struct StxProjector {
    int type;
    int family;
    float a, b;
    float scale;
    float k[9], rinv[9], r_kinv[9], k_rinv[9], t[3];
    int trig;
    int remap;
};
int stx_make_projector(int type, float scale, const float* K, const float* R, StxProjector* out);

struct StxWarpLaunch {
    StxProjector proj;
    int tlx, tly, dw, dh;
    const uint8_t* src; int sw, sh; size_t sstride; int src_channels;
    uint8_t* dimg; size_t dimg_stride;
    uint8_t* dmask; size_t dmask_stride;
    int nearest_src;
    int debug_maps = 0;
    const float* gain_H = nullptr; long long gain_hstride = 0; const void* gain_yt = nullptr; int gain_gh = 0;
};
bool stx_warp_fast_eligible(const StxWarpLaunch& L);
int stx_launch_warp(stx_ctx* ctx, const StxWarpLaunch& L);
int stx_launch_warp_batch(stx_ctx* ctx, const StxWarpLaunch* Ls, int n);
int stx_launch_roi_minmax(stx_ctx* ctx, int n, const StxProjector* projs, const int* sizes_wh, float* out_minmax4);

struct StxMbImage {
    int kind; int order;
    const uint8_t* img0; long long img0_stride; int img0_is_s16;
    const uint8_t* mask0; long long mask0_stride; int mask_binary;
    int iw, ih;
    int ix, iy;
    int fx, fy, fw, fh;
    int left, top;
    int g_u8;
    short* g[STX_MAX_BANDS + 1]; long long g_stride[STX_MAX_BANDS + 1]; long long g_plane[STX_MAX_BANDS + 1];
    float* wt[STX_MAX_BANDS + 1]; long long wt_stride[STX_MAX_BANDS + 1];
    int w1_f16;
    uint8_t* occ[STX_MAX_BANDS + 1];
};
static_assert(offsetof(StxMbImage, ih) == offsetof(StxMbImage, iw) + 4 && offsetof(StxMbImage, ix) == offsetof(StxMbImage, iw) + 8 &&
                  offsetof(StxMbImage, iy) == offsetof(StxMbImage, iw) + 12 && offsetof(StxMbImage, iw) % 4 == 0,
              "StxMbImage: iw, ih, ix, iy must be four adjacent ints");
static_assert(offsetof(StxMbImage, fy) == offsetof(StxMbImage, fx) + 4 && offsetof(StxMbImage, fw) == offsetof(StxMbImage, fx) + 8 &&
                  offsetof(StxMbImage, fh) == offsetof(StxMbImage, fx) + 12 && offsetof(StxMbImage, fx) % 4 == 0,
              "StxMbImage: fx, fy, fw, fh must be four adjacent ints");
int stx_launch_mb_pyramids(stx_ctx* ctx, const StxMbImage* d_images, const StxMbImage* h_images, int n, int num_bands, int pyr_mode,
                           int pyr_lanes, bool weights);
struct MbLevelK;
int stx_launch_mb_level(stx_ctx* ctx, const MbLevelK& K, double algo_bytes);
int stx_launch_mb_coarse(stx_ctx* ctx, const MbLevelK& K_level_Bm2, double algo_bytes);

int stx_launch_gain_apply(stx_ctx* ctx, stx_buf* img, const float g[3]);
int block_gain_check(stx_ctx* ctx, const stx_buf* img, const stx_buf* gain_map);
int stx_launch_block_gain(stx_ctx* ctx, stx_buf* img, const stx_buf* gmap, const int* d_xt, const int* d_yt);
int stx_launch_block_gain_batch(stx_ctx* ctx, int n, stx_buf* const* imgs, const stx_buf* const* gmaps, const int* full_wh_xy0,
                                float* const* Hs, void* const* yts, const int* fast);
// ... 89 lines not shown
    uint16_t* dist; long long dstride;
    int* first; int* last; unsigned long long* zbits; int n_chunks;
};
struct FeatherGatherK {
    const FeatherImg* imgs; int n; int w, h; float sharpness;
    uint8_t* pano; long long pano_stride; uint8_t* pmask; long long pmask_stride; short* pano16; long long pano16_stride;
};
int stx_launch_feather_weights(stx_ctx* ctx, const FeatherImg* d_imgs, const FeatherImg* h_imgs, int n);
int stx_launch_feather_gather(stx_ctx* ctx, const FeatherGatherK& K, double algo_bytes);

struct NoImg { const uint8_t* img; long long istride; const uint8_t* mask; long long mstride; int is_s16; int x, y, w, h; int mask_binary; };
struct NoGatherK {
    const NoImg* imgs; int n; int all_binary;
    int w, h;
    uint8_t* pano; long long pano_stride; uint8_t* pmask; long long pmask_stride; short* pano16; long long pano16_stride;
};
int stx_launch_no_gather(stx_ctx* ctx, const NoGatherK& K, double algo_bytes);

struct stx_blender {
    stx_ctx* ctx = nullptr;
    int kind = 0, num_bands = 0;
    float sharpness = 0.02f;
    int rx = 0, ry = 0, rw = 0, rh = 0;
    int fw = 0, fh = 0;
    bool finished = false;
    std::vector<StxMbImage> images;
    std::vector<char> built;
    std::vector<stx_buf*> held;
    std::vector<void*> pyr_allocs;
    std::vector<void*> wt_allocs;
    stx_mb_weights* keep = nullptr;
    stx_mb_weights* adopted = nullptr;
    StxMbImage* d_all = nullptr;
    StxMbImage* d_gather = nullptr;
    int band_x0 = 0, band_x1 = 0;
    int next_order = 0;
    int pyr_mode = 0;
    std::vector<NoImg> no_images;
    std::vector<FeatherImg> feather_images;
};
struct StxMbKept {
    stx_buf* mask;
    const uint8_t* mask0; long long mask0_stride; int mask_binary, w1_f16;
    int iw, ih, ix, iy, fx, fy, fw, fh, left, top;
    float* wt[STX_MAX_BANDS + 1]; long long wt_stride[STX_MAX_BANDS + 1];
    uint8_t* occ[STX_MAX_BANDS + 1];
};
struct stx_mb_weights {
    stx_ctx* ctx = nullptr;
    std::atomic<int> refs{1};
    int num_bands = 0, pyr_mode = 0;
    int rx = 0, ry = 0, rw = 0, rh = 0;
    std::vector<StxMbKept> images;
    std::vector<void*> allocs;
    struct Cover { int x0, x1, y0, y1, tiles_x, tiles_y, band_rows; unsigned long long* table; };
    Cover cover[STX_MAX_BANDS + 1] = {};
};
void stx_mb_weights_release(stx_mb_weights* w);
void mb_feed_rect(const stx_blender* b, int w, int h, int tlx, int tly, int* fx, int* fy, int* fw, int* fh);
bool mb_contrib_range(const stx_blender* b, int fx, int fw, int bx0, int bx1, int* sx0, int* sx1);
```

stitching_amd/csrc/stx_warp.hip:

```cpp
#include <algorithm>
#include <chrono>
#include <cmath>
#include <cstdlib>
#include <cstring>
#include <thread>

#include <hip/hip_ext.h>

#include "stx_device_math.h"
#include "stx_internal.h"

using namespace stxd;

namespace {

constexpr int WARP_TW = 256;
constexpr int WARP_TH = 4;
constexpr int WARP_IT = 1;
constexpr int WARP_FTH = WARP_TH * WARP_IT;
constexpr int WARP_WAVES = 1;
constexpr int WARP_FW = 64 * WARP_WAVES;
constexpr int WARP_BAND = 4;
constexpr float PI_F = 3.14159274101257324f;

// ... 927 lines not shown
    for (int o = 32; o > 0; o >>= 1) {
        float a = __shfl_xor(mnu, o), b = __shfl_xor(mnv, o), c = __shfl_xor(mxu, o), d = __shfl_xor(mxv, o);
        if (a < mnu) mnu = a;
        if (b < mnv) mnv = b;
        if (c > mxu) mxu = c;
        if (d > mxv) mxv = d;
    }
    __shared__ float s_part[4][4];
    if ((threadIdx.x & 63) == 0) {
        const int wv = threadIdx.x >> 6;
        s_part[wv][0] = mnu; s_part[wv][1] = mnv; s_part[wv][2] = mxu; s_part[wv][3] = mxv;
    }
    __syncthreads();
    if (threadIdx.x == 0) {
        for (int wv = 1; wv < 4; wv++) {
            if (s_part[wv][0] < mnu) mnu = s_part[wv][0];
            if (s_part[wv][1] < mnv) mnv = s_part[wv][1];
            if (s_part[wv][2] > mxu) mxu = s_part[wv][2];
            if (s_part[wv][3] > mxv) mxv = s_part[wv][3];
        }
        const size_t blk = (size_t)blockIdx.y * gridDim.x + blockIdx.x;
        float* o = out + 4 * blk;
        o[0] = mnu; o[1] = mnv; o[2] = mxu; o[3] = mxv;
        __hip_atomic_store(stamps + blk, seq, __ATOMIC_RELEASE, __HIP_MEMORY_SCOPE_SYSTEM);
    }
}

bool fast_ok(const WarpK& K)
{
    return !K.msrc && K.sw <= 32767 && K.sh <= 32767 && K.sw >= 2 && K.sh >= 2 && (long long)K.sstride * K.sh < (1ll << 31);
}

template <int TYPE>
int launch_typed(stx_ctx* ctx, const WarpK* Ks, int n, bool img, bool mask, const char* prof_name, const double* algo_bytes, int dbg)
{
    hipStream_t s = ctx->stream;
    size_t total = 0;
    for (int i = 0; i < n; i++) total += (((size_t)Ks[i].dw + 3) & ~(size_t)3) + 3 * (((size_t)Ks[i].dh + 3) & ~(size_t)3) + 32;
    StxDevBlock tab;
    STX_TRY(stx_dev_alloc(ctx, total * sizeof(float2), &tab));
    float2* cursor = (float2*)tab.get();
    for (int base = 0, m = 0; base < n; base += m) {
        const int rm = Ks[base].src ? Ks[base].remap : STX_REMAP_Q15;
        const bool gain = Ks[base].g_H != nullptr;
        for (m = 1; m < WARP_BATCH && base + m < n && (Ks[base + m].src ? Ks[base + m].remap : STX_REMAP_Q15) == rm && (Ks[base + m].g_H != nullptr) == gain; m++) {}
        WarpBatchK B;
        memset(&B, 0, sizeof(B));
        int max_tab = 0, gx = 0, gy = 0;
        bool fast = true;
        double tab_bytes = 0.0, bytes = 0.0;
        for (int i = 0; i < m; i++) {
            const WarpK& K = Ks[base + i];
            B.k[i] = K;
            B.k[i].band_rows = WARP_BAND;
            B.k[i].tiles_x = (K.dw + WARP_FW - 1) / WARP_FW;
            B.k[i].tiles_y = (K.dh + WARP_FTH - 1) / WARP_FTH;
            B.k[i].band_tiles = B.k[i].band_rows * B.k[i].tiles_x;
            B.k[i].magic_tx = (uint32_t)((1ull << 32) / (uint32_t)B.k[i].tiles_x) + 1u;
            B.k[i].magic_band = (uint32_t)((1ull << 32) / (uint32_t)B.k[i].band_tiles) + 1u;
            B.colT[i] = cursor;
            cursor += ((size_t)K.dw + 3) & ~(size_t)3;
            cursor = reinterpret_cast<float2*>(((uintptr_t)cursor + 63) & ~(uintptr_t)63);
            B.rowT[i] = reinterpret_cast<float4*>(cursor);
            cursor += 3 * (((size_t)K.dh + 3) & ~(size_t)3);
            max_tab = std::max(max_tab, K.dw + ((K.dh + 3) & ~3));
            gx = std::max(gx, (K.dw + WARP_TW - 1) / WARP_TW);
            gy = std::max(gy, (K.dh + WARP_TH - 1) / WARP_TH);
            fast = fast && fast_ok(K) && dbg != 2;
            if (gain && (!fast_ok(K) || dbg))
                return stx_fail(STX_ERR_UNSUPPORTED, "a fused gain needs the tuned warp kernel (image %d does not qualify)", base + i);
            tab_bytes += (double)K.dw * sizeof(float2) + (double)K.dh * 5 * sizeof(float);
            bytes += algo_bytes[base + i];
        }
        {
            StxProfScope prof(ctx, "warp_tables", tab_bytes);
            hipLaunchKernelGGL((warp_tables_kernel<TYPE>), dim3((max_tab + 255) / 256, m), dim3(256), 0, s, B);
        }
        if (fast) {
            StxProfScope prof(ctx, prof_name, bytes, nullptr, true);
            unsigned long long wgs = 0, wg_max = 0;
            for (int i = 0; i < WARP_BATCH; i++) B.first_wg[i] = 0xffffffffu;
            for (int i = 0; i < m; i++) {
                const int tx = (B.k[i].dw + WARP_FW - 1) / WARP_FW, ty = (B.k[i].dh + WARP_FTH - 1) / WARP_FTH;
                const int wb = B.k[i].band_rows, bands = (ty + wb - 1) / wb;
                const unsigned long long own = 8ull * (unsigned long long)(((bands + 7) / 8) * wb) * (unsigned long long)tx;
                B.first_wg[i] = (uint32_t)wgs;
                wgs += own;
                wg_max = std::max(wg_max, own);
            }
            if (wgs >= (1ull << 31)) return stx_fail(STX_ERR_UNSUPPORTED, "warp batch of %llu tiles exceeds the grid", wgs);
            const bool flat = !dbg && (double)wgs < 0.95 * (double)(wg_max * (unsigned long long)m);
            const dim3 gf(flat ? (unsigned)wgs : (unsigned)wg_max, 1, flat ? 1 : m);
            static const unsigned pad_lds = getenv("STITCHING_AMD_WARP_LDS") ? (unsigned)atoi(getenv("STITCHING_AMD_WARP_LDS")) : 0u;
#define STX_FAST_LAUNCH_K(...)                                                                                                    \
    do {                                                                                                                          \
        if (prof.start()) hipExtLaunchKernelGGL((__VA_ARGS__), gf, dim3(WARP_FW), pad_lds, s, prof.start(), prof.stop(), 0, B);     \
        else hipLaunchKernelGGL((__VA_ARGS__), gf, dim3(WARP_FW), pad_lds, s, B);                                                   \
    } while (0)
#define STX_FAST_LAUNCH_G(I, M, R, G)                                                    \
    do {                                                                                 \
        if (flat) STX_FAST_LAUNCH_K(warp_fast_kernel<TYPE, I, M, false, R, G, true>);     \
        else STX_FAST_LAUNCH_K(warp_fast_kernel<TYPE, I, M, false, R, G, false>);         \
    } while (0)
#define STX_FAST_LAUNCH(I, M, R)                              \
    do {                                                      \
        if (gain) STX_FAST_LAUNCH_G(I, M, R, true);           \
        else STX_FAST_LAUNCH_G(I, M, R, false);               \
    } while (0)
#define STX_FAST_LAUNCH_RM(I, M)                                             \
    do {                                                                     \
        if (rm == STX_REMAP_FLOAT) STX_FAST_LAUNCH(I, M, STX_REMAP_FLOAT);   \
        else if (rm == STX_REMAP_FLOAT_FMA) STX_FAST_LAUNCH(I, M, STX_REMAP_FLOAT_FMA); \
        else STX_FAST_LAUNCH(I, M, STX_REMAP_Q15);                           \
    } while (0)
            if (dbg) STX_FAST_LAUNCH_K(warp_fast_kernel<TYPE, false, false, true>);
            else if (img && mask) STX_FAST_LAUNCH_RM(true, true);
            else if (img) STX_FAST_LAUNCH_RM(true, false);
            else STX_FAST_LAUNCH_G(false, true, STX_REMAP_Q15, false);
#undef STX_FAST_LAUNCH_RM
#undef STX_FAST_LAUNCH
#undef STX_FAST_LAUNCH_G
#undef STX_FAST_LAUNCH_K
        } else {
            for (int i = 0; i < m; i++) {
                StxProfScope prof(ctx, prof_name, algo_bytes[base + i]);
                const WarpK& K = B.k[i];
                const dim3 grid((K.dw + WARP_TW - 1) / WARP_TW, (K.dh + WARP_TH - 1) / WARP_TH);
                if (dbg) hipLaunchKernelGGL((warp_kernel<TYPE, false, false, true>), grid, dim3(256), 0, s, K, B.colT[i], B.rowT[i]);
                else if (img && mask) hipLaunchKernelGGL((warp_kernel<TYPE, true, true>), grid, dim3(256), 0, s, K, B.colT[i], B.rowT[i]);
                else if (img) hipLaunchKernelGGL((warp_kernel<TYPE, true, false>), grid, dim3(256), 0, s, K, B.colT[i], B.rowT[i]);
                else hipLaunchKernelGGL((warp_kernel<TYPE, false, true>), grid, dim3(256), 0, s, K, B.colT[i], B.rowT[i]);
            }
        }
    }
    tab.reset();
    hipError_t e = hipGetLastError();
    if (e != hipSuccess) return stx_fail(STX_ERR_HIP, "warp kernel launch failed: %s", hipGetErrorString(e));
    return STX_OK;
}

template <int G>
void launch_general_group(stx_ctx* ctx, const WarpK& K, bool img, bool mask, int dbg)
{
    const dim3 grid((K.dw + WARP_TW - 1) / WARP_TW, (K.dh + GEN_TH - 1) / GEN_TH);
    if (dbg) hipLaunchKernelGGL((warp_general_kernel<G, false, false, true>), grid, dim3(256), 0, ctx->stream, K);
    else if (img && mask) hipLaunchKernelGGL((warp_general_kernel<G, true, true>), grid, dim3(256), 0, ctx->stream, K);
    else if (img) hipLaunchKernelGGL((warp_general_kernel<G, true, false>), grid, dim3(256), 0, ctx->stream, K);
    else hipLaunchKernelGGL((warp_general_kernel<G, false, true>), grid, dim3(256), 0, ctx->stream, K);
}

int launch_general(stx_ctx* ctx, const WarpK* Ks, int n, bool img, bool mask, const char* prof_name, const double* algo_bytes, int dbg)
{
    for (int i = 0; i < n; i++)
        if (Ks[i].g_H) return stx_fail(STX_ERR_UNSUPPORTED, "a fused gain needs the tuned warp kernel (per-pixel projector families have none)");
    for (int i = 0; i < n; i++) {
        StxProfScope prof(ctx, prof_name, algo_bytes[i]);
        const WarpK& K = Ks[i];
        switch (K.family) {
        case STX_F_FISHEYE:
        case STX_F_STEREOGRAPHIC: launch_general_group<GEN_FISH>(ctx, K, img, mask, dbg); break;
        case STX_F_CRECT:
        case STX_F_CRECT_PORTRAIT: launch_general_group<GEN_CRECT>(ctx, K, img, mask, dbg); break;
        case STX_F_PANINI:
        case STX_F_PANINI_PORTRAIT: launch_general_group<GEN_PANINI>(ctx, K, img, mask, dbg); break;
        case STX_F_TRANSVERSE_MERCATOR: launch_general_group<GEN_TMERC>(ctx, K, img, mask, dbg); break;
        default: return stx_fail(STX_ERR_INVALID, "no per-pixel kernel for projector family %d", K.family);
        }
    }
    hipError_t e = hipGetLastError();
    if (e != hipSuccess) return stx_fail(STX_ERR_HIP, "warp kernel launch failed: %s", hipGetErrorString(e));
// ... 28 lines not shown
    K.inv_x = 1.0f / (float)K.per_x; K.inv_y = 1.0f / (float)K.per_y;
    K.bias_x = 32 * L.sw + K.per_x * (((1 << 20) + K.per_x - 1) / K.per_x);
    K.bias_y = 32 * L.sh + K.per_y * (((1 << 20) + K.per_y - 1) / K.per_y);
    K.ux_zlo = RND_U0 + (uint32_t)zx_lo; K.ux_zhi = RND_U0 + (uint32_t)zx_hi;
    K.uy_zlo = RND_U0 + (uint32_t)zy_lo; K.uy_zhi = RND_U0 + (uint32_t)zy_hi;
    K.mx32_hi = 32.f * (((L.sw - 1) & 1) ? (float)(L.sw - 0.5) : std::nextafterf((float)(L.sw - 0.5), 3.0e38f));
    K.my32_hi = 32.f * (((L.sh - 1) & 1) ? (float)(L.sh - 0.5) : std::nextafterf((float)(L.sh - 0.5), 3.0e38f));
    {
        bool ok = std::isfinite(K.scale) && std::fabs(K.scale) > 1e-30f;
        for (int i = 0; i < 9; i++) ok = ok && std::isfinite(K.kr[i]);
        for (int i = 0; i < 3; i++) ok = ok && std::isfinite(K.t[i]);
        const double sc = std::fabs((double)K.scale);
        const double umax = std::max(std::fabs((double)L.tlx), std::fabs((double)L.tlx + L.dw)) / std::max(sc, 1e-30);
        const double vmax = std::max(std::fabs((double)L.tly), std::fabs((double)L.tly + L.dh)) / std::max(sc, 1e-30);
        double bx = 1.0001, by = 1.0001, bz = 1.0001;
        if (L.proj.family == STX_F_SPHERICAL || L.proj.family == STX_F_MERCATOR) ok = ok && umax < 5e5 && vmax < 5e5;
        else if (L.proj.family == STX_F_CYLINDRICAL) { ok = ok && umax < 5e5; by = vmax * 1.0001; }
        else { bx = (umax + std::fabs((double)K.t[0])) * 1.0001; by = (vmax + std::fabs((double)K.t[1])) * 1.0001; bz = (1.0 + std::fabs((double)K.t[2])) * 1.0001; }
        for (int r = 0; r < 2; r++)
            ok = ok && std::fabs((double)K.kr[3 * r]) * bx + std::fabs((double)K.kr[3 * r + 1]) * by + std::fabs((double)K.kr[3 * r + 2]) * bz <= 0x1p59;
        K.num_ok = ok ? 1 : 0;
    }
    {
        volatile float omt = 1.f - K.t[2];
        volatile float c2 = K.kr[2] * omt, c5 = K.kr[5] * omt, c8 = K.kr[8] * omt;
        K.c2 = c2; K.c5 = c5; K.c8 = c8;
    }
    K.z_one = K.num_ok && L.proj.family == STX_F_PLANE && K.kr[6] == 0.f && K.kr[7] == 0.f && K.c8 == 1.0f ? 1 : 0;
    *bytes = (img ? 3.0 * L.sw * L.sh + 3.0 * L.dw * L.dh : 0.0) + (mask ? 1.0 * L.dw * L.dh : 0.0);
}

}

int stx_launch_warp_batch(stx_ctx* ctx, const StxWarpLaunch* Ls, int n)
{
    if (n <= 0) return STX_OK;
    std::vector<WarpK> Ks(n);
    std::vector<double> bytes(n);
    for (int i = 0; i < n; i++) fill_warpk(Ls[i], &Ks[i], &bytes[i]);
    const bool img = Ls[0].dimg != nullptr, mask = Ls[0].dmask != nullptr;
    const int dbg = Ls[0].debug_maps;
    const char* name = dbg ? "warp_debug_maps" : (img ? (mask ? "warp_img_mask" : "warp_img") : "warp_mask");
    switch (Ls[0].proj.family) {
    case STX_F_PLANE: return launch_typed<STX_WARP_PLANE>(ctx, Ks.data(), n, img, mask, name, bytes.data(), dbg);
    case STX_F_CYLINDRICAL: return launch_typed<STX_WARP_CYLINDRICAL>(ctx, Ks.data(), n, img, mask, name, bytes.data(), dbg);
    case STX_F_SPHERICAL:
    case STX_F_MERCATOR:
        return launch_typed<STX_WARP_SPHERICAL>(ctx, Ks.data(), n, img, mask, name, bytes.data(), dbg);
    default: return launch_general(ctx, Ks.data(), n, img, mask, name, bytes.data(), dbg);
    }
}

int stx_launch_warp(stx_ctx* ctx, const StxWarpLaunch& L) { return stx_launch_warp_batch(ctx, &L, 1); }

bool stx_warp_fast_eligible(const StxWarpLaunch& L)
{
    if (L.proj.family != STX_F_PLANE && L.proj.family != STX_F_CYLINDRICAL && L.proj.family != STX_F_SPHERICAL && L.proj.family != STX_F_MERCATOR) return false;
    WarpK K;
    double bytes;
    fill_warpk(L, &K, &bytes);
    return fast_ok(K) && !L.debug_maps && L.dimg != nullptr;
}

int stx_launch_roi_minmax(stx_ctx* ctx, int n, const StxProjector* projs, const int* sizes_wh, float* out_minmax4)
{
    const bool full = n > 0 && projs[0].family > STX_F_SPHERICAL;
    const int BX = full ? 256 : 32;
    const size_t stamp_off = ctx->pinned_bytes / 4 * 3;
    const int cap = (int)(stamp_off / (16 * BX));
    static const bool no_spin = getenv("STITCHING_AMD_ROI_NO_SPIN") != nullptr;
    for (int start = 0; start < n; start += cap) {
        const int cnt = std::min(cap, n - start);
        float* dout = (float*)ctx->pinned;
        uint32_t* stamps = (uint32_t*)((uint8_t*)ctx->pinned + stamp_off);
        uint32_t seq = ++ctx->roi_seq;
        if (seq == 0) seq = ++ctx->roi_seq;
        for (int base = 0; base < cnt; base += ROI_BATCH) {
            const int m = std::min(ROI_BATCH, cnt - base);
            RoiBatchK B;
            memset(&B, 0, sizeof(B));
            for (int i = 0; i < m; i++) {
// ... 57 lines not shown
```

stitching_amd/csrc/stx_warp_host.cpp:

```cpp
#include <algorithm>
#include <array>
#include <climits>
#include <cmath>
#include <cstdlib>
#include <cstring>
#include <limits>

#include "stx_internal.h"

static void inv3x3_f32(const float* m, float* o)
{
    auto M = [&](int i, int j) { return (double)m[i * 3 + j]; };
    double d = m[0] * (M(1, 1) * M(2, 2) - M(1, 2) * M(2, 1)) - m[1] * (M(1, 0) * M(2, 2) - M(1, 2) * M(2, 0)) +
               m[2] * (M(1, 0) * M(2, 1) - M(1, 1) * M(2, 0));
    if (d == 0.) {
        for (int i = 0; i < 9; i++) o[i] = 0.f;
        return;
    }
    d = 1. / d;
    o[0] = (float)((M(1, 1) * M(2, 2) - M(1, 2) * M(2, 1)) * d);
    o[1] = (float)((M(0, 2) * M(2, 1) - M(0, 1) * M(2, 2)) * d);
    o[2] = (float)((M(0, 1) * M(1, 2) - M(0, 2) * M(1, 1)) * d);
    o[3] = (float)((M(1, 2) * M(2, 0) - M(1, 0) * M(2, 2)) * d);
    o[4] = (float)((M(0, 0) * M(2, 2) - M(0, 2) * M(2, 0)) * d);
    o[5] = (float)((M(0, 2) * M(1, 0) - M(0, 0) * M(1, 2)) * d);
    o[6] = (float)((M(1, 0) * M(2, 1) - M(1, 1) * M(2, 0)) * d);
    o[7] = (float)((M(0, 1) * M(2, 0) - M(0, 0) * M(2, 1)) * d);
    o[8] = (float)((M(0, 0) * M(1, 1) - M(0, 1) * M(1, 0)) * d);
}

static void mul3x3_f32(const float* a, const float* b, float* d)
{
    for (int i = 0; i < 3; i++)
        for (int j = 0; j < 3; j++) {
            float t = a[i * 3] * b[j];
            t = t + a[i * 3 + 1] * b[3 + j];
            t = t + a[i * 3 + 2] * b[6 + j];
            d[i * 3 + j] = t;
        }
// ... 240 lines not shown
    }
    STX_TRY(stx_launch_warp(ctx, L));
    if (bm) bm->mask_binary = 1;
    if (out_img) *out_img = bi.release();
    if (out_mask) *out_mask = bm.release();
    if (out_xywh) memcpy(out_xywh, roi, 16);
    return STX_OK;
}

STX_EXPORT int stx_warp(stx_ctx* ctx, int type, float scale, const float K[9], const float R[9], const stx_buf* src,
                        int interp, int border, stx_buf** out, int out_tl[2])
{
    if (!ctx || !src || !out) return stx_fail(STX_ERR_INVALID, "null argument");
    STX_TRY(stx_set_device(ctx));
    if (src->elem != STX_U8) return stx_fail(STX_ERR_INVALID, "warp source must be 8-bit");
    int roi[4];
    if (interp == STX_INTER_LINEAR && border == STX_BORDER_REFLECT) {
        if (src->c != 3) return stx_fail(STX_ERR_UNSUPPORTED, "INTER_LINEAR warp needs a 3-channel u8 image");
        STX_TRY(warp_impl(ctx, type, scale, K, R, src, src->w, src->h, true, false, false, out, nullptr, roi));
    } else if (interp == STX_INTER_NEAREST && border == STX_BORDER_CONSTANT) {
        if (src->c != 1) return stx_fail(STX_ERR_UNSUPPORTED, "INTER_NEAREST warp needs a 1-channel u8 mask");
        STX_TRY(warp_impl(ctx, type, scale, K, R, src, src->w, src->h, true, false, true, out, nullptr, roi));
    } else {
        return stx_fail(STX_ERR_UNSUPPORTED,
                        "only (INTER_LINEAR, BORDER_REFLECT) and (INTER_NEAREST, BORDER_CONSTANT) are on the path "
                        "(stitching/warper.py:49-50,65-66)");
    }
    if (out_tl) { out_tl[0] = roi[0]; out_tl[1] = roi[1]; }
    return STX_OK;
}

static int warp_batch_impl(stx_ctx* ctx, int type, float scale, int n, const float* K9s, const float* R9s,
                           const stx_buf* const* srcs, const int* rects, stx_buf** out_imgs, stx_buf** out_masks, int* out_xywh,
                           const stx_buf* const* gains = nullptr, const int* gflags = nullptr, bool fresh_rois = false)
{
    if (!ctx || !K9s || !R9s || !srcs || n < 0) return stx_fail(STX_ERR_INVALID, "bad argument");
    if (!out_imgs && !out_masks) return stx_fail(STX_ERR_INVALID, "nothing requested");
    if (n == 0) return STX_OK;
    STX_TRY(stx_set_device(ctx));
    std::vector<StxProjector> ps(n);
    std::vector<int> rois(4 * (size_t)n), sizes(2 * (size_t)n);
    for (int i = 0; i < n; i++) {
        if (!srcs[i] || srcs[i]->elem != STX_U8 || srcs[i]->c != 3) return stx_fail(STX_ERR_INVALID, "warp source %d must be u8x3", i);
        if (srcs[i]->ctx->device != ctx->device) return stx_fail(STX_ERR_INVALID, "warp source %d lives on another device", i);
        STX_TRY(stx_make_projector(type, scale, K9s + 9 * i, R9s + 9 * i, &ps[i]));
        sizes[2 * i] = srcs[i]->w;
        sizes[2 * i + 1] = srcs[i]->h;
    }
    if (!g_roi_cache) g_roi_cache = new std::map<RoiKey, std::array<int, 4>>();
    std::vector<int> miss;
    const bool need_rois = !rects || gains;
    for (int i = 0; i < n && need_rois; i++) {
        if (fresh_rois) { miss.push_back(i); continue; }
        auto it = g_roi_cache->find(make_key(type, scale, K9s + 9 * i, R9s + 9 * i, sizes[2 * i], sizes[2 * i + 1]));
        if (it != g_roi_cache->end()) memcpy(&rois[4 * i], it->second.data(), 16);
        else miss.push_back(i);
    }
    if (!miss.empty()) {
        const int m = (int)miss.size();
        std::vector<StxProjector> mp(m);
        std::vector<int> msz(2 * (size_t)m), mroi(4 * (size_t)m);
        for (int j = 0; j < m; j++) { mp[j] = ps[miss[j]]; msz[2 * j] = sizes[2 * miss[j]]; msz[2 * j + 1] = sizes[2 * miss[j] + 1]; }
        STX_TRY(rois_impl(ctx, m, mp.data(), msz.data(), mroi.data()));
        if (g_roi_cache->size() > 8192) g_roi_cache->clear();
        for (int j = 0; j < m; j++) {
            const int i = miss[j];
            memcpy(&rois[4 * i], &mroi[4 * j], 16);
// ... 33 lines not shown
    }
    std::vector<int> sub;
    StxDevBlock gscratch;
    bool fused = false;
    if (gains) {
        for (int i = 0; i < n; i++) {
            sub.push_back(full_rois[4 * i + 2]); sub.push_back(full_rois[4 * i + 3]);
            sub.push_back(rois[4 * i] - full_rois[4 * i]); sub.push_back(rois[4 * i + 1] - full_rois[4 * i + 1]);
        }
        static const bool no_fuse = getenv("STITCHING_AMD_NO_GAIN_FUSION") != nullptr;
        fused = !no_fuse;
        for (int i = 0; i < n && fused; i++)
            fused = gains[i]->c == 1 && gflags && (gflags[i] & STX_GAIN_MAP_BOUNDED) && stx_warp_fast_eligible(Ls[i]) &&
                    (size_t)gains[i]->h * (size_t)Ls[i].dw < ((size_t)16 << 20);
        if (fused) {
            std::vector<size_t> offH(n), offY(n);
            size_t bytes = 0;
            for (int i = 0; i < n; i++) {
                offH[i] = bytes; bytes += align_up((size_t)gains[i]->h * ((Ls[i].dw + 3) & ~3) * sizeof(float), 256);
                offY[i] = bytes; bytes += align_up((size_t)Ls[i].dh * 8, 256);
            }
            STX_TRY(stx_dev_alloc(ctx, bytes, &gscratch));
            std::vector<float*> Hs(n);
            std::vector<void*> yts(n);
            std::vector<int> wh(2 * (size_t)n);
            for (int i = 0; i < n; i++) {
                Hs[i] = (float*)((uint8_t*)gscratch.get() + offH[i]); yts[i] = (uint8_t*)gscratch.get() + offY[i];
                wh[2 * i] = Ls[i].dw; wh[2 * i + 1] = Ls[i].dh;
                Ls[i].gain_H = Hs[i]; Ls[i].gain_hstride = (Ls[i].dw + 3) & ~3; Ls[i].gain_yt = yts[i]; Ls[i].gain_gh = gains[i]->h;
            }
            STX_TRY(stx_launch_gain_rows(ctx, n, wh.data(), gains, sub.data(), Hs.data(), yts.data()));
        }
    }
    STX_TRY(stx_launch_warp_batch(ctx, Ls.data(), n));
    gscratch.reset();
    if (gains && !fused) STX_TRY(stx_block_gain_apply_batch(ctx, n, stx_buf_ptrs(bi).data(), gains, sub.data(), gflags));
    for (int i = 0; i < n; i++) {
        if (bm[i]) bm[i]->mask_binary = 1;
        if (out_imgs) out_imgs[i] = bi[i].release();
        if (out_masks) out_masks[i] = bm[i].release();
    }
    if (out_xywh) memcpy(out_xywh, rois.data(), sizeof(int) * 4 * (size_t)n);
    return STX_OK;
}

STX_EXPORT int stx_warp_batch(stx_ctx* ctx, int type, float scale, int n, const float* K9s, const float* R9s,
                              const stx_buf* const* srcs, stx_buf** out_imgs, stx_buf** out_masks, int* out_xywh)
{
    return warp_batch_impl(ctx, type, scale, n, K9s, R9s, srcs, nullptr, out_imgs, out_masks, out_xywh);
}

STX_EXPORT int stx_warp_batch_rects(stx_ctx* ctx, int type, float scale, int n, const float* K9s, const float* R9s,
                                    const stx_buf* const* srcs, const int* rects_xywh, stx_buf** out_imgs, stx_buf** out_masks)
{
    if (!rects_xywh) return stx_fail(STX_ERR_INVALID, "null argument");
    return warp_batch_impl(ctx, type, scale, n, K9s, R9s, srcs, rects_xywh, out_imgs, out_masks, nullptr);
}

STX_EXPORT int stx_warp_batch_gain(stx_ctx* ctx, int type, float scale, int n, const float* K9s, const float* R9s, const stx_buf* const* srcs,
                                   const int* rects_xywh_or_null, const stx_buf* const* gain_maps, const int* gain_flags, stx_buf** out_imgs,
                                   stx_buf** out_masks, int* out_xywh_or_null)
{
    if (!gain_maps || !out_imgs) return stx_fail(STX_ERR_INVALID, "null argument");
    return warp_batch_impl(ctx, type, scale, n, K9s, R9s, srcs, rects_xywh_or_null, out_imgs, out_masks, rects_xywh_or_null ? nullptr : out_xywh_or_null,
                           gain_maps, gain_flags);
}

STX_EXPORT int stx_warp_batch_with_rois(stx_ctx* ctx, int type, float scale, int n, const float* K9s, const float* R9s,
                                        const stx_buf* const* srcs, const stx_buf* const* gain_maps_or_null, const int* gain_flags_or_null,
                                        stx_buf** out_imgs, stx_buf** out_masks, int* out_xywh)
{
    if (!out_xywh) return stx_fail(STX_ERR_INVALID, "null argument");
    if (gain_maps_or_null && !out_imgs) return stx_fail(STX_ERR_INVALID, "gains without images");
    return warp_batch_impl(ctx, type, scale, n, K9s, R9s, srcs, nullptr, out_imgs, out_masks, out_xywh, gain_maps_or_null, gain_flags_or_null, true);
}

STX_EXPORT int stx_warp_image_and_mask(stx_ctx* ctx, int type, float scale, const float K[9], const float R[9],
                                       const stx_buf* src, stx_buf** out_img, stx_buf** out_mask, int out_xywh[4])
{
    if (!ctx || !src) return stx_fail(STX_ERR_INVALID, "null argument");
    if (!out_img && !out_mask) return stx_fail(STX_ERR_INVALID, "nothing requested");
    STX_TRY(stx_set_device(ctx));
    if (src->elem != STX_U8 || src->c != 3) return stx_fail(STX_ERR_INVALID, "warp source must be u8x3");
    return warp_impl(ctx, type, scale, K, R, src, src->w, src->h, out_img != nullptr, out_mask != nullptr, false,
                     out_img, out_mask, out_xywh);
}

STX_EXPORT int stx_warp_mask(stx_ctx* ctx, int type, float scale, const float K[9], const float R[9], int w, int h,
                             stx_buf** out_mask, int out_xywh[4])
{
    if (!ctx || !out_mask) return stx_fail(STX_ERR_INVALID, "null argument");
    if (w <= 0 || h <= 0) return stx_fail(STX_ERR_INVALID, "image size %dx%d", w, h);
    STX_TRY(stx_set_device(ctx));
    return warp_impl(ctx, type, scale, K, R, nullptr, w, h, false, true, false, nullptr, out_mask, out_xywh);
}

STX_EXPORT int stx_debug_warp_maps(stx_ctx* ctx, int type, float scale, const float K[9], const float R[9], int w, int h, int which,
                                   const int rect_xywh[4], stx_buf** out_xmap, stx_buf** out_ymap, int out_xywh[4])
// ... 30 lines not shown
```

stitching_amd/pipeline.py:

```python
import ctypes as C

import numpy as np

from . import _lib, config
from .blender import Blender
from .cropper import Cropper
from .device import as_device, get_context
from .exposure_error_compensator import ExposureErrorCompensator
from .images import Images
from .seam_estimation import SeamEstimator
from .seam_finder import DEVICE_SEAM_FINDERS, SeamFinder
from .stitching_error import StitchingError
from .synthetic import blend_strength_for_bands
from .warper import Warper


def mask_box(mask):
    m2 = mask.reshape(mask.shape[0], mask.shape[1], -1).any(axis=2)
    nx, ny = np.flatnonzero(m2.any(axis=0)), np.flatnonzero(m2.any(axis=1))
    if not nx.size:
        return None
    return (int(nx[0]), int(nx[-1]) + 1, int(mask.shape[1]), int(ny[0]), int(ny[-1]) + 1, int(mask.shape[0]))


def view_rects(handle, corners, sizes, boxes, min_gain=0.9):
    B = handle.num_bands()
    if B <= 0:
        return None
    roi = Blender.result_roi(corners, sizes)
    align, reach = max(8, 1 << B), 2 << B

    def band(lo, hi, size, msize, origin):
        if msize != size:
            lo = int(np.floor((lo - 2 + 0.5) * size / msize - 0.5)) - 1
            hi = int(np.ceil((hi + 2 + 0.5) * size / msize - 0.5)) + 1
        lo, hi = max(lo, 0), min(hi, size)
        return max(((origin + lo - reach) // align) * align, 0), -((-(origin + hi + reach)) // align) * align

    out = []
    for (cx, cy), (w, h), box in zip(corners, sizes, boxes):
        if box is None:
            out.append(None)
            continue
        bx0, bx1 = band(box[0], box[1], w, box[2], cx - roi[0])
        by0, by1 = band(box[3], box[4], h, box[5], cy - roi[1])
        r = (C.c_int * 4)()
        _lib.check(_lib.lib().stx_view_rect(handle._h, int(w), int(h), int(cx), int(cy), int(bx0), int(bx1), int(by0), int(by1), r))
        x0, x1, y0, y1 = (int(v) for v in r)
        if x1 <= x0 or y1 <= y0:
            out.append(None)
            continue
        if x1 - x0 > min_gain * w:
            x0, x1 = 0, w
        if y1 - y0 > min_gain * h:
            y0, y1 = 0, h
        out.append((x0, x1, y0, y1) if (x1 - x0) * (y1 - y0) < w * h else None)
    return None if all(o is None for o in out) else out


def clip_rectangle(rect, width, height):
    x0, x1, _ = slice(rect.x, rect.x2).indices(int(width))
    y0, y1, _ = slice(rect.y, rect.y2).indices(int(height))
    return x0, max(x1, x0), y0, max(y1, y0)


def _split_cropper(cropper, crop_aspect):
    if isinstance(cropper, (tuple, list)):
        cropper, crop_aspect = cropper
    if cropper is not None and not cropper.do_crop:
        cropper = None
    if cropper is not None and not getattr(cropper, "intersection_rectangles", None):
        raise StitchingError("the cropper is not prepared: Cropper.prepare(imgs, masks, corners, sizes) on the low-resolution warps comes first")
    return cropper, crop_aspect


class _RigGeometry:

    __slots__ = ("key", "rects", "prep_corners", "prep_sizes", "feed_corners", "feed_masks", "blend_strength", "crop", "gain_in_warp",
                 "gain_corners", "gain_sub", "weights", "blender")

    def __init__(self):
        self.key = self.weights = self.crop = self.gain_corners = self.gain_sub = None
        self.blender = None
        self.gain_in_warp = True


def rig_key(cam_bytes, camera_aspect, warper_type, scale, sizes, blender_type, num_bands, blend_strength, modes, cropper, crop_aspect):
    crop = None
    if cropper is not None:
        crop = (tuple(tuple(int(v) for v in r) for r in cropper.intersection_rectangles), float(crop_aspect))
    return (cam_bytes, float(camera_aspect), str(warper_type), None if scale is None else float(scale), tuple((int(w), int(h)) for w, h in sizes),
            str(blender_type), None if num_bands is None else int(num_bands), float(blend_strength) if num_bands is None else None,
            tuple(modes), crop)


def masks_belong_to_job(feed_masks, seam_masks):
    given = feed_masks if feed_masks is not None else seam_masks
    return given is None or all(isinstance(m, np.ndarray) for m in given)


class StitchJob:

    def __init__(self, frames, cameras, warper_type="spherical", blender_type="multiband", num_bands=None,
                 blend_strength=Blender.DEFAULT_BLEND_STRENGTH, ctx=None, async_upload=False, feed_masks=None, seam_masks=None,
                 crop_to_masks=True, compensator=None, cropper=None, crop_aspect=1, camera_aspect=1, reuse_geometry=True):
        cropper, crop_aspect = _split_cropper(cropper, crop_aspect)
        if len(frames) != len(cameras) or not frames:
            raise StitchingError("need one camera per frame and at least one frame")
        self.ctx = ctx or get_context()
        self.frames = [as_device(f, self.ctx, wait=not async_upload) for f in frames]
        self.cameras = list(cameras)
        self.sizes = [(f.width, f.height) for f in self.frames]
        self.warper = Warper(warper_type, ctx=self.ctx)
        self.warper.set_scale(self.cameras)
        self.blender_type = blender_type
# ... 21 lines not shown
    def source_pixels(self):
        return sum(w * h for w, h in self.sizes)

    def plan(self):
        self._adopt(*self.warper.warp_rois(self.sizes, self.cameras, self.camera_aspect, camera_arrays=self._cam_arrays))
        return self.corners, self.warped_sizes

    def _adopt(self, corners, warped_sizes):
        self.corners, self.warped_sizes = corners, warped_sizes
        if any(w <= 0 or h <= 0 for w, h in self.warped_sizes):
            raise StitchingError(f"degenerate warp roi {self.warped_sizes}: the {self.warper.warper_type!r} projection cannot "
                                 "represent these cameras")
        if self.num_bands is not None:
            roi = Blender.result_roi(self.corners, self.warped_sizes)
            self.blend_strength = blend_strength_for_bands(self.num_bands, roi[2], roi[3])

    def _crop_rects(self, handle, corners, sizes):
        key = (tuple(corners), tuple(sizes), self.blend_strength)
        if self._crop_cache is None or self._crop_cache[0] != key:
            self._crop_cache = (key, view_rects(handle, corners, sizes, self._mask_cols))
        return self._crop_cache[1]

    def set_frames(self, frames):
        frames = list(frames)
        got = [Images.get_image_size(f) for f in frames]
        if got != [tuple(z) for z in self.sizes]:
            raise StitchingError(f"the job was made for frames of sizes {self.sizes}, got {got}: same rig, same sizes")
        self.frames = [as_device(f, self.ctx) for f in frames]

    def release_geometry(self):
        g, self._geometry = self._geometry, None
        if g is not None and g.weights is not None:
            g.weights.free()

    def geometry_key(self):
        modes = (config.trig_mode(), config.remap_mode()) + tuple(config.pyrdown_mode())
        return rig_key(self._cam_bytes, self.camera_aspect, self.warper.warper_type, self.warper.scale, self.sizes, self.blender_type,
                       self.num_bands, self.blend_strength, modes, self.cropper, self.crop_aspect)

    def run(self, frames=None):
        if frames is not None:
            self.set_frames(frames)
        prev = config.device_resident()
        config.set_device_resident(True)
        try:
            key = self.geometry_key() if self.reuse_geometry else None
            g = self._geometry
            if g is not None and g.key != key:
                self.release_geometry()
                g = None
            self.last_reused, self.last_weights_adopted = g is not None, False
            if g is None:
                g, imgs = self._geometry_pass()
                g.key = key
            else:
                imgs, _, _ = self.warper.warp_images_and_masks(self.frames, self.cameras, self.camera_aspect, rects=g.rects,
                                                               compensator=self.compensator if g.gain_in_warp else None,
                                                               camera_arrays=self._cam_arrays, masks=False)
                if self.compensator is not None and not g.gain_in_warp:
                    imgs = self.compensator.apply_all(g.gain_corners, imgs, None, sub=g.gain_sub, ctx=self.ctx)
            self.last_crop = g.crop
            blender, g.blender = g.blender, None
            if blender is None:
                blender = Blender(self.blender_type, g.blend_strength, ctx=self.ctx)
                blender.prepare(g.prep_corners, g.prep_sizes)
            for img, mask, corner in zip(imgs, g.feed_masks, g.feed_corners):
                blender.feed(img, mask, corner)
            self.last_num_bands = blender.blender.num_bands()
            if key is not None and blender.blender.kind == _lib.BLEND_MULTIBAND:
                if not self.last_reused:
                    g.weights = blender.blender.keep_weights()
                elif g.weights is not None:
                    self.last_weights_adopted = blender.blender.use_weights(g.weights)
            pano, pmask = blender.blend()
            if key is not None:
                self._geometry = g
        finally:
            config.set_device_resident(prev)
        return pano, pmask

    def _geometry_pass(self):
        g = _RigGeometry()
        if self.cropper is not None:
            return self._geometry_pass_cropped(g)
        warped = None
        if self._mask_cols is None:
            warped = self.warper.warp_images_and_masks(self.frames, self.cameras, self.camera_aspect, compensator=self.compensator,
                                                       with_rois=True, camera_arrays=self._cam_arrays)
            self._adopt([r[0:2] for r in warped[2]], [r[2:4] for r in warped[2]])
        else:
            self.plan()
        g.blender = Blender(self.blender_type, self.blend_strength, ctx=self.ctx)
        g.blender.prepare(self.corners, self.warped_sizes)
        crop = None
        if self._mask_cols is not None and g.blender.blender.kind == _lib.BLEND_MULTIBAND:
            crop = self._crop_rects(g.blender.blender, self.corners, self.warped_sizes)
        if crop is not None:
            box = [c if c is not None else (0, w, 0, h) for c, (w, h) in zip(crop, self.warped_sizes)]
            rects = [(cx + x0, cy + y0, x1 - x0, y1 - y0) for (x0, x1, y0, y1), (cx, cy) in zip(box, self.corners)]
            imgs, masks, rois = self.warper.warp_images_and_masks(self.frames, self.cameras, self.camera_aspect, rects=rects,
                                                                  compensator=self.compensator, camera_arrays=self._cam_arrays)
            if self.feed_masks is not None:
                masks = [m[y0:y1, x0:x1] for m, (x0, x1, y0, y1) in zip(self.feed_masks, box)]
            else:
                masks = SeamFinder.resize_all(self.seam_masks, masks,
                                              sub=[(w, h, x0, y0) for (x0, x1, y0, y1), (w, h) in zip(box, self.warped_sizes)])
            corners = [(r[0], r[1]) for r in rects]
        else:
            imgs, masks, rois = warped or self.warper.warp_images_and_masks(self.frames, self.cameras, self.camera_aspect,
                                                                            compensator=self.compensator, camera_arrays=self._cam_arrays)
            if self.feed_masks is not None:
                masks = self.feed_masks
            elif self.seam_masks is not None:
                masks = SeamFinder.resize_all(self.seam_masks, masks)
            corners = self.corners
            for roi, corner in zip(rois, self.corners):
                if roi[0:2] != tuple(corner):
                    raise StitchingError("warp roi changed between plan() and run()")
            rects = [(cx, cy, w, h) for (cx, cy), (w, h) in zip(self.corners, self.warped_sizes)]
        g.rects, g.crop = [tuple(int(v) for v in r) for r in rects], crop
        g.prep_corners, g.prep_sizes, g.blend_strength = list(self.corners), list(self.warped_sizes), self.blend_strength
        g.feed_corners, g.feed_masks = list(corners), list(masks)
        return g, imgs

    def _geometry_pass_cropped(self, g):
        self.plan()
        cuts = [clip_rectangle(r.times(self.crop_aspect), w, h) for r, (w, h) in zip(self.cropper.intersection_rectangles, self.warped_sizes)]
        cut_sizes = [(x1 - x0, y1 - y0) for x0, x1, y0, y1 in cuts]
        if any(w <= 0 or h <= 0 for w, h in cut_sizes):
            raise StitchingError(f"the cropper leaves nothing of a warped image (sizes {cut_sizes}): it was prepared for another panorama")
        corners, sizes = self.cropper.crop_rois(self.corners, self.warped_sizes, self.crop_aspect)
        corners, sizes = [tuple(c) for c in corners], [tuple(z) for z in sizes]
        roi = Blender.result_roi(corners, sizes)
        if self.num_bands is not None:
# ... 210 lines not shown
```

stitching_amd/warper.py:

```python
import ctypes as C
from statistics import median

import numpy as np

from . import _lib, config
from .device import DeviceImage, as_device, get_context
from .stitching_error import StitchingError

_TYPE_IDS = _lib.WARP_TYPE_IDS


def _mat33(m, what):
    a = np.asarray(m)
    if a.shape != (3, 3) or a.dtype != np.float32:
        raise StitchingError(f"{what} must be a 3x3 float32 matrix, got shape {a.shape} dtype {a.dtype}")
    return np.ascontiguousarray(a)


def _fp(a):
    return a.ctypes.data_as(C.POINTER(C.c_float))


class Warper:

    WARP_TYPE_CHOICES = (
        "spherical",
        "plane",
        "affine",
        "cylindrical",
        "fisheye",
        "stereographic",
        "compressedPlaneA2B1",
        "compressedPlaneA1.5B1",
        "compressedPlanePortraitA2B1",
        "compressedPlanePortraitA1.5B1",
        "paniniA2B1",
        "paniniA1.5B1",
        "paniniPortraitA2B1",
        "paniniPortraitA1.5B1",
        "mercator",
        "transverseMercator",
    )
    SUPPORTED_WARP_TYPES = tuple(_TYPE_IDS)

    DEFAULT_WARP_TYPE = "spherical"

    def __init__(self, warper_type=DEFAULT_WARP_TYPE, ctx=None):
        self.warper_type = warper_type
        self.scale = None
        self.ctx = ctx

    def _ctx(self):
        return self.ctx or get_context()
# ... 48 lines not shown
        _lib.check(ctx._lib.stx_warp_rois(ctx.handle, self._type_id(), self._scale(aspect), n, _fp(Ks), _fp(Rs),
                                          wh.ctypes.data_as(C.POINTER(C.c_int)),
                                          out.ctypes.data_as(C.POINTER(C.c_int))))
        for roi in out:
            roi = tuple(int(v) for v in roi)
            roi_corners.append(roi[0:2])
            roi_sizes.append(roi[2:4])
        return roi_corners, roi_sizes

    def warp_roi(self, size, camera, aspect=1):
        ctx = self._ctx()
        K, R = self._K_R(camera, aspect)
        roi = (C.c_int * 4)()
        _lib.check(ctx._lib.stx_warp_roi(ctx.handle, self._type_id(), self._scale(aspect), _fp(K), _fp(R),
                                         int(size[0]), int(size[1]), roi))
        return tuple(int(v) for v in roi)

    @staticmethod
    def get_K(camera, aspect=1):
        K = np.array(camera.K(), dtype=np.float32)
        for r, c in ((0, 0), (0, 2), (1, 1), (1, 2)):
            K[r, c] *= aspect
        return K

    def warp_image_and_mask(self, img, camera, aspect=1):
        ctx = self._ctx()
        src = self._source(img, ctx)
        K, R = self._K_R(camera, aspect)
        oi, om, roi = C.c_void_p(), C.c_void_p(), (C.c_int * 4)()
        _lib.check(ctx._lib.stx_warp_image_and_mask(ctx.handle, self._type_id(), self._scale(aspect), _fp(K), _fp(R),
                                                    src._h, C.byref(oi), C.byref(om), roi))
        return (self._result(DeviceImage(ctx, oi)), self._result(DeviceImage(ctx, om)), tuple(int(v) for v in roi))

    def warp_images_and_masks(self, imgs, cameras, aspect=1, rects=None, compensator=None, with_rois=False, camera_arrays=None, masks=True):
        ctx = self._ctx()
        srcs = [self._source(img, ctx) for img in imgs]
        cameras = list(cameras)
        n = min(len(srcs), len(cameras))
        if n == 0:
            return [], [], []
        Ks, Rs = camera_arrays if camera_arrays is not None else self.camera_arrays(cameras[:n], aspect)
        h_src = (C.c_void_p * n)(*[s._h for s in srcs[:n]])
        h_img, h_mask = (C.c_void_p * n)(), (C.c_void_p * n)()
        if not masks:
            if rects is None:
                raise StitchingError("masks=False needs rects: the rectangles of the call that made the masks")
            h_mask = None
        rois = np.zeros((n, 4), np.int32)
        blocks = compensator is not None and compensator.compensator_type in ("gain_blocks", "channel_blocks")
        if blocks and compensator.gains is None:
            raise StitchingError("ExposureErrorCompensator.set_gains(gains) must be called before apply")
        if with_rois and rects is None:
            ga = fl = None
            if blocks:
                gm = [compensator._gain_map(i, ctx) for i in range(n)]
                ga, fl = (C.c_void_p * n)(*[g[0]._h for g in gm]), (C.c_int * n)(*[g[1] for g in gm])
                compensator = None
            _lib.check(ctx._lib.stx_warp_batch_with_rois(ctx.handle, self._type_id(), self._scale(aspect), n, _fp(Ks), _fp(Rs), h_src, ga, fl,
                                                         h_img, h_mask, rois.ctypes.data_as(C.POINTER(C.c_int))))
        elif blocks:
            gm = [compensator._gain_map(i, ctx) for i in range(n)]
            ga, fl = (C.c_void_p * n)(*[g[0]._h for g in gm]), (C.c_int * n)(*[g[1] for g in gm])
            rp = None
            if rects is not None:
                rois = np.ascontiguousarray(np.asarray(rects, np.int32).reshape(n, 4))
                rp = rois.ctypes.data_as(C.POINTER(C.c_int))
            _lib.check(ctx._lib.stx_warp_batch_gain(ctx.handle, self._type_id(), self._scale(aspect), n, _fp(Ks), _fp(Rs), h_src, rp, ga, fl,
                                                    h_img, h_mask, None if rects is not None else rois.ctypes.data_as(C.POINTER(C.c_int))))
            compensator = None
        elif rects is not None:
            rois = np.ascontiguousarray(np.asarray(rects, np.int32).reshape(n, 4))
            _lib.check(ctx._lib.stx_warp_batch_rects(ctx.handle, self._type_id(), self._scale(aspect), n, _fp(Ks), _fp(Rs), h_src,
                                                     rois.ctypes.data_as(C.POINTER(C.c_int)), h_img, h_mask))
        else:
            _lib.check(ctx._lib.stx_warp_batch(ctx.handle, self._type_id(), self._scale(aspect), n, _fp(Ks), _fp(Rs), h_src,
                                               h_img, h_mask, rois.ctypes.data_as(C.POINTER(C.c_int))))
        d_imgs = [DeviceImage(ctx, C.c_void_p(h_img[i])) for i in range(n)]
        if compensator is not None:
            prev = config.device_resident()
            config.set_device_resident(True)
            try:
                d_imgs = compensator.apply_all([tuple(int(v) for v in r[:2]) for r in rois], d_imgs, None, ctx=ctx)
            finally:
                config.set_device_resident(prev)
        imgs_out = [self._result(d) for d in d_imgs]
        masks_out = None if h_mask is None else [self._result(DeviceImage(ctx, C.c_void_p(h_mask[i]))) for i in range(n)]
        return imgs_out, masks_out, [tuple(int(v) for v in r) for r in rois]

    @staticmethod
    def _source(img, ctx):
        src = as_device(img, ctx)
        if src.channels != 3 or src.dtype != np.uint8:
            raise StitchingError(f"warp_image expects a HxWx3 uint8 image, got {src.shape} {src.dtype}")
        return src

    def _type_id(self):
        if self.warper_type not in Warper.WARP_TYPE_CHOICES:
            raise StitchingError(f"unknown warper type {self.warper_type!r}")
        if self.warper_type not in _TYPE_IDS:
            raise StitchingError(f"warper type {self.warper_type!r} is not implemented by the MI355X back end "
                                 f"(implemented: {', '.join(_TYPE_IDS)})")
        return _TYPE_IDS[self.warper_type]

    def _scale(self, aspect):
        if self.scale is None:
            raise StitchingError("Warper.set_scale(cameras) must be called before warping")
# ... 9 lines not shown
```

Measured before the change: 204,400 Mpix/s.

## Keep warp tables across frames, cache blend tables, skip unused mask stores

Adds kept warp-table handles, so repeated panoramas with the same geometry can reuse the per-batch warp setup tables instead of rebuilding them. It also keeps the multiband image descriptor table resident under an LRU keyed on its contents, defers weight-pyramid allocation until the pyramids are built, and lets the replaying level-0 kernels skip the panorama-mask store when no mask is requested. The aim is to cut per-frame host launches, uploads and write bandwidth. In exchange it adds cache-invalidation risk and a new hard failure when the level-0 replay path cannot run without a mask.

```diff
diff --git a/include/stitching_amd.h b/include/stitching_amd.h
--- a/include/stitching_amd.h
+++ b/include/stitching_amd.h
@@ -71,6 +71,7 @@
 typedef struct stx_buf stx_buf;
 typedef struct stx_blender stx_blender;
 typedef struct stx_mb_weights stx_mb_weights;
+typedef struct stx_warp_tables stx_warp_tables;
 
 int stx_version(void);
 const char* stx_last_error(void);
@@ -108,6 +109,15 @@
 int stx_warp_batch_gain(stx_ctx* ctx, int type, float scale, int n, const float* K9s, const float* R9s, const stx_buf* const* srcs,
                         const int* rects_xywh, const stx_buf* const* gain_maps_f32, const int* gain_flags, stx_buf** out_imgs,
                         stx_buf** out_masks, int* out_xywh);
+int stx_warp_batch_rects_kept(stx_ctx* ctx, int type, float scale, int n, const float* K9s, const float* R9s, const stx_buf* const* srcs,
+                              const int* rects_xywh, stx_buf** out_imgs, stx_buf** out_masks, stx_warp_tables** tables);
+int stx_warp_batch_gain_kept(stx_ctx* ctx, int type, float scale, int n, const float* K9s, const float* R9s, const stx_buf* const* srcs,
+                             const int* rects_xywh, const stx_buf* const* gain_maps_f32, const int* gain_flags, stx_buf** out_imgs,
+                             stx_buf** out_masks, stx_warp_tables** tables);
+int stx_warp_batch_with_rois_kept(stx_ctx* ctx, int type, float scale, int n, const float* K9s, const float* R9s, const stx_buf* const* srcs,
+                                  const stx_buf* const* gain_maps_f32_or_null, const int* gain_flags_or_null, stx_buf** out_imgs,
+                                  stx_buf** out_masks, int* out_xywh, stx_warp_tables** tables);
+int stx_warp_tables_free(stx_warp_tables* t);
 int stx_warp_batch_with_rois(stx_ctx* ctx, int type, float scale, int n, const float* K9s, const float* R9s, const stx_buf* const* srcs,
                              const stx_buf* const* gain_maps_f32_or_null, const int* gain_flags_or_null, stx_buf** out_imgs,
                              stx_buf** out_masks, int* out_xywh);
diff --git a/include/stitching_amd_debug.h b/include/stitching_amd_debug.h
--- a/include/stitching_amd_debug.h
+++ b/include/stitching_amd_debug.h
@@ -14,6 +14,12 @@
 
 int stx_debug_blend_replayed(stx_ctx* ctx, int* out_launches);
 
+int stx_debug_warp_table_launches(stx_ctx* ctx, int* out_launches);
+
+int stx_debug_blend_uploads(stx_ctx* ctx, int* out_uploads);
+
+int stx_debug_blend_mask_stored(stx_ctx* ctx, int* out_stored);
+
 #ifdef __cplusplus
 }
 #endif
diff --git a/stitching_amd/_lib.py b/stitching_amd/_lib.py
--- a/stitching_amd/_lib.py
+++ b/stitching_amd/_lib.py
@@ -34,12 +34,12 @@
 EXPORTS = (
     "stx_version stx_last_error stx_set_trig_mode stx_get_trig_mode stx_set_remap_mode stx_get_remap_mode stx_set_pyrdown_mode stx_get_pyrdown_mode stx_device_count stx_ctx_create stx_ctx_destroy stx_ctx_sync "
     "stx_host_alloc stx_host_free stx_buf_from_host stx_buf_from_host_async stx_buf_alloc stx_buf_to_host stx_buf_to_host_async stx_buf_view stx_buf_info stx_buf_device_ptr stx_buf_free "
-    "stx_warp_roi stx_warp_rois stx_warp stx_warp_image_and_mask stx_warp_batch stx_warp_batch_rects stx_warp_batch_gain stx_warp_batch_with_rois stx_warp_mask "
+    "stx_warp_roi stx_warp_rois stx_warp stx_warp_image_and_mask stx_warp_batch stx_warp_batch_rects stx_warp_batch_gain stx_warp_batch_rects_kept stx_warp_batch_gain_kept stx_warp_tables_free stx_warp_batch_with_rois stx_warp_batch_with_rois_kept stx_warp_mask "
     "stx_gain_apply stx_block_gain_apply stx_block_gain_apply_batch stx_resize_linear_exact stx_resize_linear_exact_batch stx_seam_mask_resize stx_seam_mask_resize_batch stx_seam_mask_resize_batch_sub stx_timelapse_frame stx_result_roi stx_blend_create stx_blend_num_bands stx_blend_feed stx_blend_finish stx_blend_finish_ex "
     "stx_blend_destroy stx_blend_keep_weights stx_blend_use_weights stx_mb_weights_free stx_blend_set_band stx_blend_feed_ex stx_blend_contrib_rect stx_blend_export_contrib stx_blend_export_contribs "
     "stx_blend_build stx_blend_feed_contrib stx_blend_feed_contrib_ex stx_buf_flags stx_strip_rect stx_view_rect stx_strip_pack stx_strip_pack_batch stx_strip_pack_batch_ex stx_strip_bytes stx_strip_unpack stx_blend_feed_strips stx_comm_unique_id stx_comm_create stx_comm_exchange stx_comm_exchange_begin stx_comm_exchange_end stx_comm_exchange_begin_on stx_comm_exchange_end_on stx_comm_info stx_comm_destroy stx_prof_enable stx_prof_reset stx_prof_count stx_prof_get stx_mark stx_mark_elapsed_ms "
     "stx_exposure_feed stx_exposure_stats stx_exposure_solve stx_set_exposure_solver stx_get_exposure_solver stx_exposure_feed_ex stx_exposure_solve_device stx_lu_solve_device stx_seam_find stx_seam_schedule stx_color_seam_find stx_crop_lir stx_features_detect stx_match_features stx_ray_problem_create stx_ray_problem_eval stx_ray_problem_free "
-    "stx_debug_warp_maps stx_debug_feather_dist_cap stx_debug_blend_replayed"
+    "stx_debug_warp_maps stx_debug_feather_dist_cap stx_debug_blend_replayed stx_debug_warp_table_launches stx_debug_blend_uploads stx_debug_blend_mask_stored"
 ).split()
 
 _lib = None
@@ -90,6 +90,10 @@
     L.stx_warp_batch.argtypes = [vp, C.c_int, C.c_float, C.c_int, fp, fp, vpp, vpp, vpp, ip]
     L.stx_warp_batch_rects.argtypes = [vp, C.c_int, C.c_float, C.c_int, fp, fp, vpp, ip, vpp, vpp]
     L.stx_warp_batch_gain.argtypes = [vp, C.c_int, C.c_float, C.c_int, fp, fp, vpp, ip, vpp, ip, vpp, vpp, ip]
+    L.stx_warp_batch_rects_kept.argtypes = [vp, C.c_int, C.c_float, C.c_int, fp, fp, vpp, ip, vpp, vpp, vpp]
+    L.stx_warp_batch_gain_kept.argtypes = [vp, C.c_int, C.c_float, C.c_int, fp, fp, vpp, ip, vpp, ip, vpp, vpp, vpp]
+    L.stx_warp_tables_free.argtypes = [vp]
+    L.stx_warp_batch_with_rois_kept.argtypes = [vp, C.c_int, C.c_float, C.c_int, fp, fp, vpp, vpp, ip, vpp, vpp, ip, vpp]
     L.stx_warp_batch_with_rois.argtypes = [vp, C.c_int, C.c_float, C.c_int, fp, fp, vpp, vpp, ip, vpp, vpp, ip]
     L.stx_warp_mask.argtypes = [vp, C.c_int, C.c_float, fp, fp, C.c_int, C.c_int, vpp, ip]
     L.stx_gain_apply.argtypes = [vp, vp, fp]
@@ -144,6 +148,9 @@
     L.stx_prof_get.argtypes = [vp, C.c_int, C.c_char_p, C.c_int, C.POINTER(C.c_int64), C.POINTER(C.c_double),
                                C.POINTER(C.c_double)]
     L.stx_debug_blend_replayed.argtypes = [vp, ip]
+    L.stx_debug_warp_table_launches.argtypes = [vp, ip]
+    L.stx_debug_blend_uploads.argtypes = [vp, ip]
+    L.stx_debug_blend_mask_stored.argtypes = [vp, ip]
     L.stx_debug_warp_maps.argtypes = [vp, C.c_int, C.c_float, fp, fp, C.c_int, C.c_int, C.c_int, ip, vpp, vpp, ip]
     llp, dp = C.POINTER(C.c_longlong), C.POINTER(C.c_double)
     L.stx_exposure_feed.argtypes = [vp, C.c_int, C.c_int, vpp, vpp, ip, C.c_int, C.c_int, dp, llp, dp]
diff --git a/stitching_amd/csrc/stx_blend.hip b/stitching_amd/csrc/stx_blend.hip
--- a/stitching_amd/csrc/stx_blend.hip
+++ b/stitching_amd/csrc/stx_blend.hip
@@ -717,6 +717,7 @@
     if (K.x1 <= K.x0 || K.y1 <= K.y0) return STX_OK;
     StxProfScope prof(ctx, K.emit ? "mb_contrib" : (K.level == 0 ? "mb_level0" : "mb_level"), algo_bytes);
     if ((K.level > 0 || K.all_u8) && stx_fast_mb_level(ctx, K)) return STX_OK;
+    if (K.level == 0 && !K.emit && !K.pmask) return stx_fail(STX_ERR_HIP, "multi-band level 0: the replaying gather could not be launched");
     const dim3 grid = grid64x4(K.x1 - K.x0, K.y1 - K.y0);
     if (K.level == 0) hipLaunchKernelGGL(mb_level_kernel<true>, grid, dim3(256), 0, ctx->stream, K);
     else hipLaunchKernelGGL(mb_level_kernel<false>, grid, dim3(256), 0, ctx->stream, K);
diff --git a/stitching_amd/csrc/stx_blend_fast.hip b/stitching_amd/csrc/stx_blend_fast.hip
--- a/stitching_amd/csrc/stx_blend_fast.hip
+++ b/stitching_amd/csrc/stx_blend_fast.hip
@@ -854,7 +854,7 @@
     }
 }
 
-template <bool L0>
+template <bool L0, bool MASK_OPT = false>
 STX_DEV void level_epilogue(const MbLevelK& P, int X0, int Y0, int (&acc)[2][8][3], float (&ws)[2][8])
 {
     int v[2][8][3];
@@ -917,7 +917,7 @@
             *reinterpret_cast<uint2*>(po) = make_uint2(ob[0], ob[1]);
             *reinterpret_cast<uint2*>(po + 2) = make_uint2(ob[2], ob[3]);
             *reinterpret_cast<uint2*>(po + 4) = make_uint2(ob[4], ob[5]);
-            *reinterpret_cast<uint2*>(P.pmask + (long long)oy * P.pmask_stride + ox) = make_uint2(om[0], om[1]);
+            if (!MASK_OPT || P.pmask) *reinterpret_cast<uint2*>(P.pmask + (long long)oy * P.pmask_stride + ox) = make_uint2(om[0], om[1]);
             if (P.pano16) {
                 uint32_t* p16 = reinterpret_cast<uint32_t*>(reinterpret_cast<uint8_t*>(P.pano16) + (long long)oy * P.pano16_stride +
                                                             (long long)ox * 6);
@@ -998,7 +998,7 @@
     return ((StxCoverPtr)P.cover)[idx];
 }
 
-template <bool WF>
+template <bool WF, bool MASK_OPT = false>
 STX_DEV void level0_epilogue_pk(const MbLevelK& P, int X0, int Y0, uint32_t (&acc)[2][3][4], uint32_t (&cnt)[2][4], const float (*ws)[8]);
 
 template <bool L0, bool CONTRIB, bool EMIT, bool U8SRC>
@@ -1395,7 +1395,7 @@
     return lo | hi;
 }
 
-template <bool WF>
+template <bool WF, bool MASK_OPT>
 STX_DEV void level0_epilogue_pk(const MbLevelK& P, int X0, int Y0, uint32_t (&acc)[2][3][4], uint32_t (&cnt)[2][4], const float (*ws)[8])
 {
     uint32_t k_p1 = 0x00010001u, k_m1 = 0xffffffffu;
@@ -1507,8 +1507,9 @@
         *reinterpret_cast<uint2*>(po) = make_uint2(bgr_dword<0>(U), bgr_dword<1>(U));
         *reinterpret_cast<uint2*>(po + 2) = make_uint2(bgr_dword<2>(U), bgr_dword<3>(U));
         *reinterpret_cast<uint2*>(po + 4) = make_uint2(bgr_dword<4>(U), bgr_dword<5>(U));
-        *reinterpret_cast<uint2*>(P.pmask + (long long)oy * P.pmask_stride + ox) =
-            make_uint2(__builtin_amdgcn_perm(keep[2], keep[0], 0x06020400u), __builtin_amdgcn_perm(keep[3], keep[1], 0x06020400u));
+        if (!MASK_OPT || P.pmask)
+            *reinterpret_cast<uint2*>(P.pmask + (long long)oy * P.pmask_stride + ox) =
+                make_uint2(__builtin_amdgcn_perm(keep[2], keep[0], 0x06020400u), __builtin_amdgcn_perm(keep[3], keep[1], 0x06020400u));
         if (P.pano16) {
             uint32_t* p16 = reinterpret_cast<uint32_t*>(reinterpret_cast<uint8_t*>(P.pano16) + (long long)oy * P.pano16_stride + (long long)ox * 6);
             int w[8][3];
@@ -1680,7 +1681,7 @@
         cnt[r][2] = pair_u8<1, 3>(cntb[r]);
         cnt[r][3] = pair_u8<5, 7>(cntb[r]);
     }
-    level0_epilogue_pk<false>(P, X0, Y0, acc, cnt, nullptr);
+    level0_epilogue_pk<false, REPLAY>(P, X0, Y0, acc, cnt, nullptr);
 }
 
 
@@ -1752,7 +1753,7 @@
                         ws[r][j] = fadd(ws[r][j], w);
                     }
             }
-            if (live) level_epilogue<true>(P, X0, Y0, acc, ws);
+            if (live) level_epilogue<true, true>(P, X0, Y0, acc, ws);
         }
         g0 += nb;
     }
@@ -2061,21 +2062,38 @@
     return off;
 }
 
+static bool mb_replays(const MbLevelK& K) { return !K.emit && K.cover != nullptr && K.n_images <= 64 && !K.has_contrib; }
+enum MbL0Path { L0_OTHER, L0_PK, L0_DEFER };
+static MbL0Path mb_level0_path(const MbLevelK& K)
+{
+    if (K.level != 0 || K.emit || K.num_bands <= 0) return L0_OTHER;
+    if (K.pk_ok) return L0_PK;
+    return K.all_u8 && !K.has_contrib && !no_defer() ? L0_DEFER : L0_OTHER;
+}
+
+bool stx_fast_mb_level0_skips_mask(const MbLevelK& K)
+{
+    MbLevelK KT;
+    return K.all_u8 && fast_level_ok(K, &KT) && mb_replays(K) && mb_level0_path(K) != L0_OTHER;
+}
+
 bool stx_fast_mb_level(stx_ctx* ctx, const MbLevelK& K)
 {
     MbLevelK KT;
     if (!fast_level_ok(K, &KT)) return false;
+    if (K.level == 0 && !K.emit && !K.pmask && !stx_fast_mb_level0_skips_mask(K)) return false;
     dim3 grid(stx_tile_grid(KT.tiles), 1);
     hipStream_t st = ctx->stream;
-    const bool replay = !K.emit && K.cover != nullptr && K.n_images <= 64 && !K.has_contrib;
+    const bool replay = mb_replays(K);
+    const MbL0Path l0 = mb_level0_path(K);
     bool replayed = false;
-    if (K.level == 0 && K.pk_ok && !K.emit && K.num_bands > 0) {
+    if (l0 == L0_PK) {
         static const unsigned pad_lds = getenv("STITCHING_AMD_L0_LDS") ? (unsigned)atoi(getenv("STITCHING_AMD_L0_LDS")) : 0u;
         if (K.has_contrib) hipLaunchKernelGGL(mb_level0_pk_kernel<true>, grid, dim3(LV_THREADS), pad_lds, st, KT);
         else if (replay) hipLaunchKernelGGL((mb_level0_pk_kernel<false, false, true>), grid, dim3(LV_THREADS), pad_lds, st, KT);
         else hipLaunchKernelGGL(mb_level0_pk_kernel<false>, grid, dim3(LV_THREADS), pad_lds, st, KT);
         replayed = replay && !K.has_contrib;
-    } else if (K.level == 0 && K.all_u8 && !K.has_contrib && !K.emit && K.num_bands > 0 && !no_defer()) {
+    } else if (l0 == L0_DEFER) {
         const int segs = std::min(KT.tiles.tiles_x, STX_DEFER_SEGS);
         const size_t seg_cap = (size_t)((KT.tiles.tiles_x + STX_DEFER_SEGS - 1) / STX_DEFER_SEGS) * (size_t)KT.tiles.tiles_y * (unsigned)LV_THREADS;
         const size_t counters = (size_t)STX_DEFER_SEGS * 128;
diff --git a/stitching_amd/csrc/stx_blend_host.cpp b/stitching_amd/csrc/stx_blend_host.cpp
--- a/stitching_amd/csrc/stx_blend_host.cpp
+++ b/stitching_amd/csrc/stx_blend_host.cpp
@@ -177,13 +177,11 @@
     for (int i = 1; i <= nb; i++) {
         const int lw = im.fw >> i, lh = im.fh >> i;
         const long long gs = (long long)align_up((size_t)lw, im.g_u8 ? 64 : 32), ws = (long long)align_up((size_t)lw, 16);
-        void *g = nullptr, *wt = nullptr;
+        void* g = nullptr;
         STX_TRY(stx_dev_alloc(ctx, MB_FRONT_PAD + (size_t)gs * lh * 3 * (im.g_u8 ? 1 : sizeof(short)) + 64, &g));
         b->pyr_allocs.push_back(g);
-        STX_TRY(stx_dev_alloc(ctx, (size_t)ws * lh * ((i == 1 && im.w1_f16) ? sizeof(uint16_t) : sizeof(float)), &wt));
-        b->wt_allocs.push_back(wt);
         im.g[i] = (short*)((uint8_t*)g + MB_FRONT_PAD); im.g_stride[i] = gs; im.g_plane[i] = gs * lh;
-        im.wt[i] = (float*)wt; im.wt_stride[i] = ws;
+        im.wt[i] = nullptr; im.wt_stride[i] = ws;
     }
     mb_insert_sorted(b, im, nb == 0);
     stx_buf_retain(const_cast<stx_buf*>(img));
@@ -200,12 +198,53 @@
     STX_TRY(stx_dev_alloc(ctx, sizeof(StxMbImage) * std::max(n, 1), &d));
     b->pyr_allocs.push_back(d);
     if (n > 0) STX_TRY(stx_stage_upload(ctx, d, h, sizeof(StxMbImage) * (size_t)n));
+    ctx->blend_uploads++;
     *d_out = (StxMbImage*)d;
     return STX_OK;
 }
 
+static int mb_resident_table(stx_blender* b, stx_mb_weights* w, const StxMbImage* h, int n, StxMbImage** d_out)
+{
+    stx_ctx* ctx = b->ctx;
+    const size_t bytes = sizeof(StxMbImage) * (size_t)n;
+    stx_mb_weights::Resident* lru = &w->resident[0];
+    for (stx_mb_weights::Resident& r : w->resident) {
+        if (r.d && r.shadow.size() == (size_t)n && memcmp(r.shadow.data(), h, bytes) == 0) {
+            r.used = ++w->resident_clock;
+            *d_out = r.d;
+            return STX_OK;
+        }
+        if (r.used < lru->used) lru = &r;
+    }
+    if (!lru->d) {
+        void* d = nullptr;
+        STX_TRY(stx_dev_alloc(ctx, bytes, &d));
+        w->allocs.push_back(d);
+        lru->d = (StxMbImage*)d;
+    }
+    lru->shadow.clear();
+    STX_TRY(stx_stage_upload(ctx, lru->d, h, bytes));
+    ctx->blend_uploads++;
+    lru->shadow.assign(h, h + n);
+    lru->used = ++w->resident_clock;
+    *d_out = lru->d;
+    return STX_OK;
+}
+
 static int mb_ensure_pyramids(stx_blender* b)
 {
+    for (size_t i = 0; i < b->images.size(); i++) {
+        StxMbImage& im = b->images[i];
+        if (im.kind != 0 || b->built[i]) continue;
+        for (int l = 1; l <= b->num_bands; l++) {
+            if (im.wt[l]) continue;
+            void* wt = nullptr;
+            STX_TRY(stx_dev_alloc(b->ctx, (size_t)im.wt_stride[l] * (im.fh >> l) * ((l == 1 && im.w1_f16) ? sizeof(uint16_t) : sizeof(float)), &wt));
+            b->wt_allocs.push_back(wt);
+            im.wt[l] = (float*)wt;
+            b->d_all = nullptr;
+        }
+    }
     std::vector<StxMbImage> todo;
     for (size_t i = 0; i < b->images.size(); i++)
         if (b->images[i].kind == 0 && !b->built[i]) todo.push_back(b->images[i]);
@@ -237,7 +276,9 @@
         }
     }
     StxMbImage* d = nullptr;
-    STX_TRY(mb_upload(b, todo.data(), (int)todo.size(), &d));
+    b->d_all_resident = b->adopted && todo.size() == b->images.size() && todo.size() == b->adopted->images.size();
+    if (b->d_all_resident) STX_TRY(mb_resident_table(b, b->adopted, todo.data(), (int)todo.size(), &d));
+    else STX_TRY(mb_upload(b, todo.data(), (int)todo.size(), &d));
     b->d_all = todo.size() == b->images.size() && memcmp(todo.data(), b->images.data(), sizeof(StxMbImage) * todo.size()) == 0 ? d : nullptr;
     STX_TRY(stx_launch_mb_pyramids(b->ctx, d, todo.data(), (int)todo.size(), b->num_bands, pyr & 255, pyr >> 8, b->adopted == nullptr));
     for (size_t i = 0; i < b->images.size(); i++) b->built[i] = 1;
@@ -352,12 +393,13 @@
     return c.table;
 }
 
-static int mb_finish(stx_blender* b, stx_buf* pano, stx_buf* pmask, stx_buf* pano16)
+static int mb_finish(stx_blender* b, stx_buf* pano, StxBufRef* pmask, stx_buf* pano16)
 {
     stx_ctx* ctx = b->ctx;
     const int nb = b->num_bands, n = (int)b->images.size();
     STX_TRY(mb_ensure_pyramids(b));
     StxMbImage* d_images = b->d_all;
+    if (d_images && b->d_all_resident) STX_TRY(mb_resident_table(b, b->adopted, b->images.data(), n, &d_images));
     if (!d_images) STX_TRY(mb_upload(b, b->images.data(), n, &d_images));
     b->d_gather = d_images;
     bool all_u8 = true, has_contrib = false, pk_ok = true;
@@ -386,9 +428,19 @@
         }
         if (lv == 0) {
             K.pano = pano->ptr; K.pano_stride = (long long)pano->stride;
-            K.pmask = pmask->ptr; K.pmask_stride = (long long)pmask->stride;
             if (pano16) { K.pano16 = (short*)pano16->ptr; K.pano16_stride = (long long)pano16->stride; }
             K.pano_x0 = b->band_x0; K.pano_y0 = 0;
+            const stx_mb_weights* w = b->adopted;
+            K.pmask = nullptr;
+            if (w && w->pmask && K.cover && w->pmask_x0 == b->band_x0 && w->pmask_x1 == b->band_x1 && w->pmask_h == b->fh &&
+                w->pmask->w == pano->w && w->pmask->h == pano->h && stx_fast_mb_level0_skips_mask(K)) {
+                stx_buf_retain(w->pmask);
+                pmask->reset(w->pmask);
+            } else {
+                STX_TRY(stx_buf_new(ctx, pano->w, pano->h, 1, STX_U8, pmask));
+                K.pmask = (*pmask)->ptr; K.pmask_stride = (long long)(*pmask)->stride;
+            }
+            ctx->blend_mask_stored = K.pmask ? 1 : 0;
         } else {
             const int w = xe[lv] - xb[lv], ph = b->rh >> lv;
             const long long st = (long long)align_up((size_t)std::max(w, 1), 32);
@@ -417,6 +469,7 @@
     if (!w || --w->refs > 0) return;
     if (w->ctx) hipSetDevice(w->ctx->device);
     for (StxMbKept& k : w->images) stx_buf_release(k.mask);
+    if (w->pmask) stx_buf_release(w->pmask);
     for (void* p : w->allocs) stx_dev_free(w->ctx, p);
     delete w;
 }
@@ -432,7 +485,7 @@
     return true;
 }
 
-static void mb_hand_over_weights(stx_blender* b)
+static void mb_hand_over_weights(stx_blender* b, stx_buf* pmask)
 {
     stx_mb_weights* w = b->keep;
     if (!w || b->images.empty() || !mb_weights_eligible(b, true)) return;
@@ -456,6 +509,15 @@
         w->images.push_back(k);
     }
     w->allocs.swap(b->wt_allocs);
+    for (stx_mb_weights::Resident& r : w->resident) {
+        void* d = nullptr;
+        if (stx_dev_alloc(b->ctx, sizeof(StxMbImage) * b->images.size(), &d) != STX_OK) break;
+        w->allocs.push_back(d);
+        r.d = (StxMbImage*)d;
+    }
+    stx_buf_retain(pmask);
+    w->pmask = pmask;
+    w->pmask_x0 = b->band_x0; w->pmask_x1 = b->band_x1; w->pmask_h = b->fh;
     if (b->images.size() > 64 || !b->d_gather) return;
     int xb[STX_MAX_BANDS + 1], xe[STX_MAX_BANDS + 1];
     mb_level_regions(b, b->band_x0, b->band_x1, xb, xe);
@@ -511,8 +573,6 @@
     STX_TRY(stx_set_device(b->ctx));
     for (size_t i = 0; i < b->images.size(); i++)
         for (int l = 1; l <= b->num_bands; l++) { b->images[i].wt[l] = w->images[i].wt[l]; b->images[i].occ[l] = w->images[i].occ[l]; }
-    for (void* p : b->wt_allocs) stx_dev_free(b->ctx, p);
-    b->wt_allocs.clear();
     b->d_all = nullptr;
     w->refs++;
     b->adopted = w;
@@ -524,6 +584,20 @@
 {
     if (!ctx || !out_launches) return stx_fail(STX_ERR_INVALID, "null argument");
     *out_launches = ctx->blend_replayed;
+    return STX_OK;
+}
+
+STX_EXPORT int stx_debug_blend_mask_stored(stx_ctx* ctx, int* out_stored)
+{
+    if (!ctx || !out_stored) return stx_fail(STX_ERR_INVALID, "null argument");
+    *out_stored = ctx->blend_mask_stored;
+    return STX_OK;
+}
+
+STX_EXPORT int stx_debug_blend_uploads(stx_ctx* ctx, int* out_uploads)
+{
+    if (!ctx || !out_uploads) return stx_fail(STX_ERR_INVALID, "null argument");
+    *out_uploads = ctx->blend_uploads;
     return STX_OK;
 }
 
@@ -594,6 +668,10 @@
         srcs[i] = *src;
     }
     STX_TRY(mb_ensure_pyramids(b));
+    for (int i = 0; i < n; i++)
+        for (const StxMbImage& im : b->images)
+            if (im.kind == 0 && im.order == orders[i])
+                for (int l = 1; l <= nb; l++) srcs[i].wt[l] = im.wt[l];
     std::vector<StxBufRef> packed(n);
     std::vector<ContribLayout> Ls(n);
     for (int i = 0; i < n; i++) {
@@ -743,17 +821,19 @@
     STX_TRY(stx_set_device(b->ctx));
     stx_ctx* ctx = b->ctx;
     ctx->blend_replayed = 0;
+    ctx->blend_uploads = 0;
+    ctx->blend_mask_stored = 0;
     const int ow = b->kind == STX_BLEND_MULTIBAND ? b->band_x1 - b->band_x0 : b->rw, oh = b->kind == STX_BLEND_MULTIBAND ? b->fh : b->rh;
     StxBufRef p16, pmask, pano;
     const int rc = [&]() {
         STX_TRY(stx_buf_new(ctx, ow, oh, 3, STX_U8, &pano));
-        STX_TRY(stx_buf_new(ctx, ow, oh, 1, STX_U8, &pmask));
+        if (b->kind != STX_BLEND_MULTIBAND) STX_TRY(stx_buf_new(ctx, ow, oh, 1, STX_U8, &pmask));
         if (out_pano_s16) STX_TRY(stx_buf_new(ctx, ow, oh, 3, STX_S16, &p16));
-        if (b->kind == STX_BLEND_MULTIBAND) return mb_finish(b, pano.get(), pmask.get(), p16.get());
+        if (b->kind == STX_BLEND_MULTIBAND) return mb_finish(b, pano.get(), &pmask, p16.get());
         if (b->kind == STX_BLEND_NO) return no_finish(b, pano.get(), pmask.get(), p16.get());
         return feather_finish(b, pano.get(), pmask.get(), p16.get());
     }();
-    if (rc == STX_OK) mb_hand_over_weights(b);
+    if (rc == STX_OK && b->kind == STX_BLEND_MULTIBAND) mb_hand_over_weights(b, pmask.get());
     b->finished = true;
     blender_release(b);
     STX_TRY(rc);
diff --git a/stitching_amd/csrc/stx_blend_kernels.h b/stitching_amd/csrc/stx_blend_kernels.h
--- a/stitching_amd/csrc/stx_blend_kernels.h
+++ b/stitching_amd/csrc/stx_blend_kernels.h
@@ -44,6 +44,7 @@
 
 bool stx_fast_mb_down_batch(stx_ctx* ctx, const StxMbImage* d_images, const StxMbImage* h_images, int n, int level, bool weights);
 bool stx_fast_mb_level(stx_ctx* ctx, const MbLevelK& K);
+bool stx_fast_mb_level0_skips_mask(const MbLevelK& K);
 void stx_fast_mb_cover_dims(int x0, int x1, int y0, int y1, int* tiles_x, int* tiles_y, int* band_rows);
 bool stx_fast_mb_cover(stx_ctx* ctx, const StxMbImage* d_images, int n, int level, int x0, int x1, int y0, int y1, unsigned long long* cover);
 
diff --git a/stitching_amd/csrc/stx_context_host.cpp b/stitching_amd/csrc/stx_context_host.cpp
--- a/stitching_amd/csrc/stx_context_host.cpp
+++ b/stitching_amd/csrc/stx_context_host.cpp
@@ -118,8 +118,13 @@
     std::lock_guard<std::mutex> lock(ctx->alloc_mutex);
     auto it = ctx->free_blocks.find(b);
     if (it != ctx->free_blocks.end() && !it->second.empty()) {
-        *out = it->second.back();
-        it->second.pop_back();
+        std::vector<void*>& v = it->second;
+        size_t lo = 0;
+        for (size_t i = 1; i < v.size(); i++)
+            if (v[i] < v[lo]) lo = i;
+        *out = v[lo];
+        v[lo] = v.back();
+        v.pop_back();
         return STX_OK;
     }
     void* p = nullptr;
diff --git a/stitching_amd/csrc/stx_internal.h b/stitching_amd/csrc/stx_internal.h
--- a/stitching_amd/csrc/stx_internal.h
+++ b/stitching_amd/csrc/stx_internal.h
@@ -72,6 +72,9 @@
     hipEvent_t marks[16] = {};
     double* exp_sqrt = nullptr;
     int blend_replayed = 0;
+    int warp_table_launches = 0;
+    int blend_uploads = 0;
+    int blend_mask_stored = 0;
 };
 
 #define STX_STAGE_SEGS 4
@@ -163,8 +166,16 @@
     const float* gain_H = nullptr; long long gain_hstride = 0; const void* gain_yt = nullptr; int gain_gh = 0;
 };
 bool stx_warp_fast_eligible(const StxWarpLaunch& L);
+struct StxWarpTabRec { int family, dw, dh, tlx, tly, trig; float scale, t0, t1, kr1, kr4, kr7; };
+struct stx_warp_tables {
+    stx_ctx* ctx = nullptr;
+    int type = -1;
+    std::vector<StxWarpTabRec> rec;
+    void* block = nullptr;
+    size_t floats2 = 0;
+};
 int stx_launch_warp(stx_ctx* ctx, const StxWarpLaunch& L);
-int stx_launch_warp_batch(stx_ctx* ctx, const StxWarpLaunch* Ls, int n);
+int stx_launch_warp_batch(stx_ctx* ctx, const StxWarpLaunch* Ls, int n, stx_warp_tables* kept = nullptr);
 int stx_launch_roi_minmax(stx_ctx* ctx, int n, const StxProjector* projs, const int* sizes_wh, float* out_minmax4);
 
 struct StxMbImage {
@@ -320,6 +331,7 @@
     stx_mb_weights* keep = nullptr;
     stx_mb_weights* adopted = nullptr;
     StxMbImage* d_all = nullptr;
+    bool d_all_resident = false;
     StxMbImage* d_gather = nullptr;
     int band_x0 = 0, band_x1 = 0;
     int next_order = 0;
@@ -343,6 +355,12 @@
     std::vector<void*> allocs;
     struct Cover { int x0, x1, y0, y1, tiles_x, tiles_y, band_rows; unsigned long long* table; };
     Cover cover[STX_MAX_BANDS + 1] = {};
+    struct Resident { StxMbImage* d = nullptr; std::vector<StxMbImage> shadow; unsigned long long used = 0; };
+    static constexpr int kResidentSlots = 4;
+    Resident resident[kResidentSlots];
+    unsigned long long resident_clock = 0;
+    stx_buf* pmask = nullptr;
+    int pmask_x0 = 0, pmask_x1 = 0, pmask_h = 0;
 };
 void stx_mb_weights_release(stx_mb_weights* w);
 void mb_feed_rect(const stx_blender* b, int w, int h, int tlx, int tly, int* fx, int* fy, int* fw, int* fh);
diff --git a/stitching_amd/csrc/stx_warp.hip b/stitching_amd/csrc/stx_warp.hip
--- a/stitching_amd/csrc/stx_warp.hip
+++ b/stitching_amd/csrc/stx_warp.hip
@@ -983,14 +983,41 @@
 }
 
 template <int TYPE>
-int launch_typed(stx_ctx* ctx, const WarpK* Ks, int n, bool img, bool mask, const char* prof_name, const double* algo_bytes, int dbg)
+int launch_typed(stx_ctx* ctx, const WarpK* Ks, int n, bool img, bool mask, const char* prof_name, const double* algo_bytes, int dbg,
+                 stx_warp_tables* kept)
 {
     hipStream_t s = ctx->stream;
     size_t total = 0;
     for (int i = 0; i < n; i++) total += (((size_t)Ks[i].dw + 3) & ~(size_t)3) + 3 * (((size_t)Ks[i].dh + 3) & ~(size_t)3) + 32;
+    bool make_tables = true;
     StxDevBlock tab;
-    STX_TRY(stx_dev_alloc(ctx, total * sizeof(float2), &tab));
-    float2* cursor = (float2*)tab.get();
+    float2* cursor = nullptr;
+    if (kept) {
+        std::vector<StxWarpTabRec> rec(n);
+        memset(rec.data(), 0, sizeof(StxWarpTabRec) * (size_t)n);
+        for (int i = 0; i < n; i++) {
+            const WarpK& K = Ks[i];
+            StxWarpTabRec& r = rec[i];
+            r.family = K.family; r.dw = K.dw; r.dh = K.dh; r.tlx = K.tlx; r.tly = K.tly; r.trig = K.trig;
+            r.scale = K.scale; r.t0 = K.t[0]; r.t1 = K.t[1]; r.kr1 = K.kr[1]; r.kr4 = K.kr[4]; r.kr7 = K.kr[7];
+        }
+        make_tables = !(kept->block && kept->type == TYPE && kept->floats2 == total && kept->rec.size() == (size_t)n &&
+                        memcmp(kept->rec.data(), rec.data(), sizeof(StxWarpTabRec) * (size_t)n) == 0);
+        if (make_tables) {
+            kept->type = -1;
+            if (kept->floats2 != total || !kept->block) {
+                if (kept->block) stx_dev_free(ctx, kept->block);
+                kept->block = nullptr; kept->floats2 = 0;
+                STX_TRY(stx_dev_alloc(ctx, total * sizeof(float2), &kept->block));
+                kept->floats2 = total;
+            }
+            kept->rec.swap(rec);
+        }
+        cursor = (float2*)kept->block;
+    } else {
+        STX_TRY(stx_dev_alloc(ctx, total * sizeof(float2), &tab));
+        cursor = (float2*)tab.get();
+    }
     for (int base = 0, m = 0; base < n; base += m) {
         const int rm = Ks[base].src ? Ks[base].remap : STX_REMAP_Q15;
         const bool gain = Ks[base].g_H != nullptr;
@@ -1023,9 +1050,10 @@
             tab_bytes += (double)K.dw * sizeof(float2) + (double)K.dh * 5 * sizeof(float);
             bytes += algo_bytes[base + i];
         }
-        {
+        if (make_tables) {
             StxProfScope prof(ctx, "warp_tables", tab_bytes);
             hipLaunchKernelGGL((warp_tables_kernel<TYPE>), dim3((max_tab + 255) / 256, m), dim3(256), 0, s, B);
+            ctx->warp_table_launches++;
         }
         if (fast) {
             StxProfScope prof(ctx, prof_name, bytes, nullptr, true);
@@ -1087,6 +1115,7 @@
     tab.reset();
     hipError_t e = hipGetLastError();
     if (e != hipSuccess) return stx_fail(STX_ERR_HIP, "warp kernel launch failed: %s", hipGetErrorString(e));
+    if (kept && make_tables) kept->type = TYPE;
     return STX_OK;
 }
 
@@ -1181,8 +1210,9 @@
 
 }
 
-int stx_launch_warp_batch(stx_ctx* ctx, const StxWarpLaunch* Ls, int n)
-{
+int stx_launch_warp_batch(stx_ctx* ctx, const StxWarpLaunch* Ls, int n, stx_warp_tables* kept)
+{
+    ctx->warp_table_launches = 0;
     if (n <= 0) return STX_OK;
     std::vector<WarpK> Ks(n);
     std::vector<double> bytes(n);
@@ -1191,11 +1221,11 @@
     const int dbg = Ls[0].debug_maps;
     const char* name = dbg ? "warp_debug_maps" : (img ? (mask ? "warp_img_mask" : "warp_img") : "warp_mask");
     switch (Ls[0].proj.family) {
-    case STX_F_PLANE: return launch_typed<STX_WARP_PLANE>(ctx, Ks.data(), n, img, mask, name, bytes.data(), dbg);
-    case STX_F_CYLINDRICAL: return launch_typed<STX_WARP_CYLINDRICAL>(ctx, Ks.data(), n, img, mask, name, bytes.data(), dbg);
+    case STX_F_PLANE: return launch_typed<STX_WARP_PLANE>(ctx, Ks.data(), n, img, mask, name, bytes.data(), dbg, kept);
+    case STX_F_CYLINDRICAL: return launch_typed<STX_WARP_CYLINDRICAL>(ctx, Ks.data(), n, img, mask, name, bytes.data(), dbg, kept);
     case STX_F_SPHERICAL:
     case STX_F_MERCATOR:
-        return launch_typed<STX_WARP_SPHERICAL>(ctx, Ks.data(), n, img, mask, name, bytes.data(), dbg);
+        return launch_typed<STX_WARP_SPHERICAL>(ctx, Ks.data(), n, img, mask, name, bytes.data(), dbg, kept);
     default: return launch_general(ctx, Ks.data(), n, img, mask, name, bytes.data(), dbg);
     }
 }
diff --git a/stitching_amd/csrc/stx_warp_host.cpp b/stitching_amd/csrc/stx_warp_host.cpp
--- a/stitching_amd/csrc/stx_warp_host.cpp
+++ b/stitching_amd/csrc/stx_warp_host.cpp
@@ -5,6 +5,7 @@
 #include <cstdlib>
 #include <cstring>
 #include <limits>
+#include <memory>
 
 #include "stx_internal.h"
 
@@ -311,7 +312,8 @@
 
 static int warp_batch_impl(stx_ctx* ctx, int type, float scale, int n, const float* K9s, const float* R9s,
                            const stx_buf* const* srcs, const int* rects, stx_buf** out_imgs, stx_buf** out_masks, int* out_xywh,
-                           const stx_buf* const* gains = nullptr, const int* gflags = nullptr, bool fresh_rois = false)
+                           const stx_buf* const* gains = nullptr, const int* gflags = nullptr, bool fresh_rois = false,
+                           stx_warp_tables* kept = nullptr)
 {
     if (!ctx || !K9s || !R9s || !srcs || n < 0) return stx_fail(STX_ERR_INVALID, "bad argument");
     if (!out_imgs && !out_masks) return stx_fail(STX_ERR_INVALID, "nothing requested");
@@ -411,7 +413,7 @@
             STX_TRY(stx_launch_gain_rows(ctx, n, wh.data(), gains, sub.data(), Hs.data(), yts.data()));
         }
     }
-    STX_TRY(stx_launch_warp_batch(ctx, Ls.data(), n));
+    STX_TRY(stx_launch_warp_batch(ctx, Ls.data(), n, kept));
     gscratch.reset();
     if (gains && !fused) STX_TRY(stx_block_gain_apply_batch(ctx, n, stx_buf_ptrs(bi).data(), gains, sub.data(), gflags));
     for (int i = 0; i < n; i++) {
@@ -443,6 +445,87 @@
     if (!gain_maps || !out_imgs) return stx_fail(STX_ERR_INVALID, "null argument");
     return warp_batch_impl(ctx, type, scale, n, K9s, R9s, srcs, rects_xywh_or_null, out_imgs, out_masks, rects_xywh_or_null ? nullptr : out_xywh_or_null,
                            gain_maps, gain_flags);
+}
+
+static int warp_kept_call(stx_ctx* ctx, stx_warp_tables** tables, int (*call)(stx_warp_tables*, void*), void* args)
+{
+    if (!ctx || !tables) return stx_fail(STX_ERR_INVALID, "null argument");
+    if (*tables && (*tables)->ctx != ctx)
+        return stx_fail(STX_ERR_INVALID, "warp tables: the handle belongs to another context (no cross-stream use)");
+    stx_warp_tables* t = *tables;
+    std::unique_ptr<stx_warp_tables> fresh;
+    if (!t) {
+        fresh.reset(new stx_warp_tables());
+        fresh->ctx = ctx;
+        t = fresh.get();
+    }
+    const int rc = call(t, args);
+    if (rc != STX_OK) {
+        if (fresh && fresh->block) { stx_set_device(ctx); stx_dev_free(ctx, fresh->block); }
+        return rc;
+    }
+    if (fresh) *tables = fresh.release();
+    return STX_OK;
+}
+
+STX_EXPORT int stx_warp_batch_rects_kept(stx_ctx* ctx, int type, float scale, int n, const float* K9s, const float* R9s,
+                                         const stx_buf* const* srcs, const int* rects_xywh, stx_buf** out_imgs, stx_buf** out_masks,
+                                         stx_warp_tables** tables)
+{
+    if (!rects_xywh) return stx_fail(STX_ERR_INVALID, "null argument");
+    struct A { stx_ctx* ctx; int type; float scale; int n; const float *K, *R; const stx_buf* const* srcs; const int* rects; stx_buf **oi, **om; };
+    A a{ctx, type, scale, n, K9s, R9s, srcs, rects_xywh, out_imgs, out_masks};
+    return warp_kept_call(ctx, tables, [](stx_warp_tables* t, void* p) {
+        const A& a = *static_cast<A*>(p);
+        return warp_batch_impl(a.ctx, a.type, a.scale, a.n, a.K, a.R, a.srcs, a.rects, a.oi, a.om, nullptr, nullptr, nullptr, false, t);
+    }, &a);
+}
+
+STX_EXPORT int stx_warp_batch_gain_kept(stx_ctx* ctx, int type, float scale, int n, const float* K9s, const float* R9s,
+                                        const stx_buf* const* srcs, const int* rects_xywh, const stx_buf* const* gain_maps, const int* gain_flags,
+                                        stx_buf** out_imgs, stx_buf** out_masks, stx_warp_tables** tables)
+{
+    if (!rects_xywh || !gain_maps || !out_imgs) return stx_fail(STX_ERR_INVALID, "null argument");
+    struct A { stx_ctx* ctx; int type; float scale; int n; const float *K, *R; const stx_buf* const* srcs; const int* rects;
+               const stx_buf* const* gains; const int* gflags; stx_buf **oi, **om; };
+    A a{ctx, type, scale, n, K9s, R9s, srcs, rects_xywh, gain_maps, gain_flags, out_imgs, out_masks};
+    return warp_kept_call(ctx, tables, [](stx_warp_tables* t, void* p) {
+        const A& a = *static_cast<A*>(p);
+        return warp_batch_impl(a.ctx, a.type, a.scale, a.n, a.K, a.R, a.srcs, a.rects, a.oi, a.om, nullptr, a.gains, a.gflags, false, t);
+    }, &a);
+}
+
+STX_EXPORT int stx_warp_batch_with_rois_kept(stx_ctx* ctx, int type, float scale, int n, const float* K9s, const float* R9s,
+                                             const stx_buf* const* srcs, const stx_buf* const* gain_maps_or_null, const int* gain_flags_or_null,
+                                             stx_buf** out_imgs, stx_buf** out_masks, int* out_xywh, stx_warp_tables** tables)
+{
+    if (!out_xywh) return stx_fail(STX_ERR_INVALID, "null argument");
+    if (gain_maps_or_null && !out_imgs) return stx_fail(STX_ERR_INVALID, "gains without images");
+    struct A { stx_ctx* ctx; int type; float scale; int n; const float *K, *R; const stx_buf* const* srcs;
+               const stx_buf* const* gains; const int* gflags; stx_buf **oi, **om; int* xywh; };
+    A a{ctx, type, scale, n, K9s, R9s, srcs, gain_maps_or_null, gain_flags_or_null, out_imgs, out_masks, out_xywh};
+    return warp_kept_call(ctx, tables, [](stx_warp_tables* t, void* p) {
+        const A& a = *static_cast<A*>(p);
+        return warp_batch_impl(a.ctx, a.type, a.scale, a.n, a.K, a.R, a.srcs, nullptr, a.oi, a.om, a.xywh, a.gains, a.gflags, true, t);
+    }, &a);
+}
+
+STX_EXPORT int stx_warp_tables_free(stx_warp_tables* t)
+{
+    if (!t) return STX_OK;
+    if (t->block) {
+        hipSetDevice(t->ctx->device);
+        stx_dev_free(t->ctx, t->block);
+    }
+    delete t;
+    return STX_OK;
+}
+
+STX_EXPORT int stx_debug_warp_table_launches(stx_ctx* ctx, int* out_launches)
+{
+    if (!ctx || !out_launches) return stx_fail(STX_ERR_INVALID, "null argument");
+    *out_launches = ctx->warp_table_launches;
+    return STX_OK;
 }
 
 STX_EXPORT int stx_warp_batch_with_rois(stx_ctx* ctx, int type, float scale, int n, const float* K9s, const float* R9s,
diff --git a/stitching_amd/pipeline.py b/stitching_amd/pipeline.py
--- a/stitching_amd/pipeline.py
+++ b/stitching_amd/pipeline.py
@@ -12,7 +12,7 @@
 from .seam_finder import DEVICE_SEAM_FINDERS, SeamFinder
 from .stitching_error import StitchingError
 from .synthetic import blend_strength_for_bands
-from .warper import Warper
+from .warper import Warper, WarpTables
 
 
 def mask_box(mask):
@@ -77,10 +77,11 @@
 class _RigGeometry:
 
     __slots__ = ("key", "rects", "prep_corners", "prep_sizes", "feed_corners", "feed_masks", "blend_strength", "crop", "gain_in_warp",
-                 "gain_corners", "gain_sub", "weights", "blender")
+                 "gain_corners", "gain_sub", "weights", "tables", "blender")
 
     def __init__(self):
         self.key = self.weights = self.crop = self.gain_corners = self.gain_sub = None
+        self.tables = WarpTables()
         self.blender = None
         self.gain_in_warp = True
 
@@ -168,6 +169,8 @@
         g, self._geometry = self._geometry, None
         if g is not None and g.weights is not None:
             g.weights.free()
+        if g is not None:
+            g.tables.free()
 
     def geometry_key(self):
         modes = (config.trig_mode(), config.remap_mode()) + tuple(config.pyrdown_mode())
@@ -192,7 +195,7 @@
             else:
                 imgs, _, _ = self.warper.warp_images_and_masks(self.frames, self.cameras, self.camera_aspect, rects=g.rects,
                                                                compensator=self.compensator if g.gain_in_warp else None,
-                                                               camera_arrays=self._cam_arrays, masks=False)
+                                                               camera_arrays=self._cam_arrays, masks=False, tables=g.tables)
                 if self.compensator is not None and not g.gain_in_warp:
                     imgs = self.compensator.apply_all(g.gain_corners, imgs, None, sub=g.gain_sub, ctx=self.ctx)
             self.last_crop = g.crop
@@ -222,7 +225,8 @@
         warped = None
         if self._mask_cols is None:
             warped = self.warper.warp_images_and_masks(self.frames, self.cameras, self.camera_aspect, compensator=self.compensator,
-                                                       with_rois=True, camera_arrays=self._cam_arrays)
+                                                       with_rois=True, camera_arrays=self._cam_arrays,
+                                                       tables=g.tables if self.reuse_geometry else None)
             self._adopt([r[0:2] for r in warped[2]], [r[2:4] for r in warped[2]])
         else:
             self.plan()
@@ -235,7 +239,8 @@
             box = [c if c is not None else (0, w, 0, h) for c, (w, h) in zip(crop, self.warped_sizes)]
             rects = [(cx + x0, cy + y0, x1 - x0, y1 - y0) for (x0, x1, y0, y1), (cx, cy) in zip(box, self.corners)]
             imgs, masks, rois = self.warper.warp_images_and_masks(self.frames, self.cameras, self.camera_aspect, rects=rects,
-                                                                  compensator=self.compensator, camera_arrays=self._cam_arrays)
+                                                                  compensator=self.compensator, camera_arrays=self._cam_arrays,
+                                                                  tables=g.tables if self.reuse_geometry else None)
             if self.feed_masks is not None:
                 masks = [m[y0:y1, x0:x1] for m, (x0, x1, y0, y1) in zip(self.feed_masks, box)]
             else:
diff --git a/stitching_amd/warper.py b/stitching_amd/warper.py
--- a/stitching_amd/warper.py
+++ b/stitching_amd/warper.py
@@ -19,6 +19,29 @@
 
 def _fp(a):
     return a.ctypes.data_as(C.POINTER(C.c_float))
+
+
+class WarpTables:
+
+    def __init__(self):
+        self.ctx, self._h = None, C.c_void_p()
+
+    def _ref(self, ctx):
+        if self.ctx is None:
+            self.ctx = ctx
+        return C.byref(self._h)
+
+    def free(self):
+        if self._h is not None and self._h.value:
+            if getattr(self.ctx, "handle", None):
+                self.ctx._lib.stx_warp_tables_free(self._h)
+            self._h = C.c_void_p()
+
+    def __del__(self):
+        try:
+            self.free()
+        except Exception:
+            pass
 
 
 class Warper:
@@ -133,7 +156,8 @@
                                                     src._h, C.byref(oi), C.byref(om), roi))
         return (self._result(DeviceImage(ctx, oi)), self._result(DeviceImage(ctx, om)), tuple(int(v) for v in roi))
 
-    def warp_images_and_masks(self, imgs, cameras, aspect=1, rects=None, compensator=None, with_rois=False, camera_arrays=None, masks=True):
+    def warp_images_and_masks(self, imgs, cameras, aspect=1, rects=None, compensator=None, with_rois=False, camera_arrays=None, masks=True,
+                              tables=None):
         ctx = self._ctx()
         srcs = [self._source(img, ctx) for img in imgs]
         cameras = list(cameras)
@@ -147,6 +171,8 @@
             if rects is None:
                 raise StitchingError("masks=False needs rects: the rectangles of the call that made the masks")
             h_mask = None
+        if tables is not None and rects is None and not with_rois:
+            raise StitchingError("tables= needs rects or with_rois: kept tables belong to given rectangles")
         rois = np.zeros((n, 4), np.int32)
         blocks = compensator is not None and compensator.compensator_type in ("gain_blocks", "channel_blocks")
         if blocks and compensator.gains is None:
@@ -157,8 +183,12 @@
                 gm = [compensator._gain_map(i, ctx) for i in range(n)]
                 ga, fl = (C.c_void_p * n)(*[g[0]._h for g in gm]), (C.c_int * n)(*[g[1] for g in gm])
                 compensator = None
-            _lib.check(ctx._lib.stx_warp_batch_with_rois(ctx.handle, self._type_id(), self._scale(aspect), n, _fp(Ks), _fp(Rs), h_src, ga, fl,
-                                                         h_img, h_mask, rois.ctypes.data_as(C.POINTER(C.c_int))))
+            if tables is not None:
+                _lib.check(ctx._lib.stx_warp_batch_with_rois_kept(ctx.handle, self._type_id(), self._scale(aspect), n, _fp(Ks), _fp(Rs), h_src, ga,
+                                                                  fl, h_img, h_mask, rois.ctypes.data_as(C.POINTER(C.c_int)), tables._ref(ctx)))
+            else:
+                _lib.check(ctx._lib.stx_warp_batch_with_rois(ctx.handle, self._type_id(), self._scale(aspect), n, _fp(Ks), _fp(Rs), h_src, ga, fl,
+                                                             h_img, h_mask, rois.ctypes.data_as(C.POINTER(C.c_int))))
         elif blocks:
             gm = [compensator._gain_map(i, ctx) for i in range(n)]
             ga, fl = (C.c_void_p * n)(*[g[0]._h for g in gm]), (C.c_int * n)(*[g[1] for g in gm])
@@ -166,13 +196,21 @@
             if rects is not None:
                 rois = np.ascontiguousarray(np.asarray(rects, np.int32).reshape(n, 4))
                 rp = rois.ctypes.data_as(C.POINTER(C.c_int))
-            _lib.check(ctx._lib.stx_warp_batch_gain(ctx.handle, self._type_id(), self._scale(aspect), n, _fp(Ks), _fp(Rs), h_src, rp, ga, fl,
-                                                    h_img, h_mask, None if rects is not None else rois.ctypes.data_as(C.POINTER(C.c_int))))
+            if tables is not None:
+                _lib.check(ctx._lib.stx_warp_batch_gain_kept(ctx.handle, self._type_id(), self._scale(aspect), n, _fp(Ks), _fp(Rs), h_src, rp, ga,
+                                                             fl, h_img, h_mask, tables._ref(ctx)))
+            else:
+                _lib.check(ctx._lib.stx_warp_batch_gain(ctx.handle, self._type_id(), self._scale(aspect), n, _fp(Ks), _fp(Rs), h_src, rp, ga, fl,
+                                                        h_img, h_mask, None if rects is not None else rois.ctypes.data_as(C.POINTER(C.c_int))))
             compensator = None
         elif rects is not None:
             rois = np.ascontiguousarray(np.asarray(rects, np.int32).reshape(n, 4))
-            _lib.check(ctx._lib.stx_warp_batch_rects(ctx.handle, self._type_id(), self._scale(aspect), n, _fp(Ks), _fp(Rs), h_src,
-                                                     rois.ctypes.data_as(C.POINTER(C.c_int)), h_img, h_mask))
+            if tables is not None:
+                _lib.check(ctx._lib.stx_warp_batch_rects_kept(ctx.handle, self._type_id(), self._scale(aspect), n, _fp(Ks), _fp(Rs), h_src,
+                                                              rois.ctypes.data_as(C.POINTER(C.c_int)), h_img, h_mask, tables._ref(ctx)))
+            else:
+                _lib.check(ctx._lib.stx_warp_batch_rects(ctx.handle, self._type_id(), self._scale(aspect), n, _fp(Ks), _fp(Rs), h_src,
+                                                         rois.ctypes.data_as(C.POINTER(C.c_int)), h_img, h_mask))
         else:
             _lib.check(ctx._lib.stx_warp_batch(ctx.handle, self._type_id(), self._scale(aspect), n, _fp(Ks), _fp(Rs), h_src,
                                                h_img, h_mask, rois.ctypes.data_as(C.POINTER(C.c_int))))
```

Result: faster. 210,300 Mpix/s (median of 6 runs) (+2.9%).
